# lan496/torch-m3gnet

Measured on AMD Instinct MI355X. Metric: atom-steps/sec (energy+forces) on 10k-atom PBC batch, 1/2/4/8 MI355X, higher is better.
Workload: dtype f32; 1 GPU; single 10000-atom fcc Cu PBC supercell per GPU (10x10x25 cells, a=3.61 A, jitter 0.025 A), r_cut 5 A / 3-body 4 A, default M3GNet (l_max=n_max=3, D=64, 3 blocks), energy+forces+stress; precision=fp32, atoms_per_gpu=10000, edges_per_gpu=420000, triplets_per_gpu=3060000

## Files before the change

### torch-m3gnet_amd/csrc/m3g_api.hip

```cpp
#include <climits>
#include <cmath>
#include <cstdarg>
#include <cstdio>
#include <cstdlib>
#include <cstring>
#include <utility>

#include "m3g_internal.h"

namespace m3g {

static thread_local char g_err[512] = "";
void set_error(const char* fmt, ...) {
  va_list ap;
  va_start(ap, fmt);
  vsnprintf(g_err, sizeof(g_err), fmt, ap);
  va_end(ap);
}

static void layout_mlp(MlpW& m, size_t& off) {
  auto take = [&](size_t n) { size_t r = off; off += (n + 63) / 64 * 64; return r; };
  m.w1a_t = take(kDP * 2 * kDP); m.w1b_t = take(kDP * 2 * kDP); m.w1c_t = take(kDP * 2 * kDP);
  m.b1 = take(2 * kDP);
  m.w2d_t = take(kDP * kDP); m.w2g_t = take(kDP * kDP);
// ... 75 lines not shown
    for (int k = 0; k < cols; ++k) blob[off + (size_t)k * ldo + col_off + o] = in[(size_t)o * ldi + k0 + k];
}
static void put_n(std::vector<float>& blob, size_t off, int ldo, const float* in, int rows, int ldi, int k0, int cols,
                  int row_off = 0) {
  for (int o = 0; o < rows; ++o)
    for (int k = 0; k < cols; ++k) blob[off + (size_t)(row_off + o) * ldo + k] = in[(size_t)o * ldi + k0 + k];
}

static void pack_mlp(std::vector<float>& blob, const MlpW& m, const m3g_plan& p, const std::string& pre,
                     const std::string& lin, int D, int R) {
  const float* wd1 = p.params.at(pre + ".dense.0.weight").data();
  const float* wg1 = p.params.at(pre + ".gate.0.weight").data();
  const size_t parts_t[3] = {m.w1a_t, m.w1b_t, m.w1c_t};
  const size_t parts_n[3] = {m.w1a, m.w1b, m.w1c};
  for (int part = 0; part < 3; ++part) {
    put_t(blob, parts_t[part], 2 * kDP, wd1, D, 3 * D, part * D, D, 0);
    put_t(blob, parts_t[part], 2 * kDP, wg1, D, 3 * D, part * D, D, kDP);
    put_n(blob, parts_n[part], kDP, wd1, D, 3 * D, part * D, D, 0);
    put_n(blob, parts_n[part], kDP, wg1, D, 3 * D, part * D, D, kDP);
  }
  const float* bd1 = p.params.at(pre + ".dense.0.bias").data();
  const float* bg1 = p.params.at(pre + ".gate.0.bias").data();
  for (int o = 0; o < D; ++o) { blob[m.b1 + o] = bd1[o]; blob[m.b1 + kDP + o] = bg1[o]; }
  const float* wd2 = p.params.at(pre + ".dense.2.weight").data();
  const float* wg2 = p.params.at(pre + ".gate.2.weight").data();
  put_t(blob, m.w2d_t, kDP, wd2, D, D, 0, D); put_t(blob, m.w2g_t, kDP, wg2, D, D, 0, D);
  put_n(blob, m.w2d, kDP, wd2, D, D, 0, D); put_n(blob, m.w2g, kDP, wg2, D, D, 0, D);
  const float* bd2 = p.params.at(pre + ".dense.2.bias").data();
  const float* bg2 = p.params.at(pre + ".gate.2.bias").data();
  for (int o = 0; o < D; ++o) { blob[m.b2d + o] = bd2[o]; blob[m.b2g + o] = bg2[o]; }
  const float* wl = p.params.at(lin).data();
  put_t(blob, m.wl_t, kDP, wl, D, R, 0, R);
  put_n(blob, m.wl, kRP, wl, D, R, 0, R);
}

Work work_carve(int B, const StepPath& path, int64_t N, int64_t E, int64_t S, void* base) {
  Work w{};
  Carve c{(char*)base};
  auto take = [&](size_t n_floats) { return (float*)c.take(n_floats * sizeof(float)); };
  size_t e = (size_t)E, n = (size_t)N;
  w.u = take(e * 3); w.d = take(e); w.h = take(e * kRP); w.hp = take(e * kRP);
  w.q = take(e * kCP); w.qp = take(e * kCP); w.fc3 = take(e); w.fc3p = take(e);
  for (int b = 0; b <= B; ++b) w.x[b] = take(n * kDP);
  for (int b = 0; b < B; ++b) w.v[b] = take(n * kCP);
  for (int b = 0; b < B; ++b) w.m[b] = take(e * kCP);
  w.dx = take(n * kDP); w.dx2 = take(n * kDP);
  w.dm = take(e * kCP); w.g = take(e * kCP); w.dg = take(e * kCP);
  w.dh = take(e * kRP); w.dd = take(e); w.du = take(e * 3); w.dp1 = take(e * 4 * kDP); w.dr = take(e * 3);
  const size_t tiles16 = (e + 15) / 16;
  if (path.pipeline == kPipeMfma) {
    for (int b = 0; b <= B; ++b) w.e_blk[b] = take(tiles16 * 1024);
    if (path.saved_acts >= 1) for (int b = 0; b < B; ++b) w.p1_blk[b] = take(tiles16 * 2 * 2048);
    if (path.saved_acts >= 2) for (int b = 0; b < B; ++b) w.p2_blk[b] = take(tiles16 * 2 * 2048);
    for (int b = 0; b < B; ++b) { w.TAb[b] = take(n * 4 * kDP); w.TBb[b] = take(n * 4 * kDP); }
    w.de_soa = take(tiles16 * 1024);
    w.dcn = take(tiles16 * 1024);
    w.dh_parts = take((size_t)(2 * B + 1) * e * kRP);
    w.seg_head = take((tiles16 + 1) * 4 * kDP);
    w.seg_first = take((n + 1) * 4 * kDP);
  } else {
    w.TA = take(n * 4 * kDP); w.TB = take(n * 4 * kDP);
    w.e = take(e * kDP);
    w.de = take(e * kDP);
    for (int b = 0; b < B; ++b) w.act[b] = take(e * 8 * kDP);
  }
  static_assert(kSyncWords <= 64, "the tail scratch reserves 64 words");
  w.tail = take(n + (size_t)S * 2 + 64);
  w.sync = w.tail ? (int32_t*)(w.tail + n + (size_t)S * 2) : nullptr;
  w.total_bytes = c.off;
  return w;
}

}

using namespace m3g;

static void drop_graphs(const m3g_plan* plan);

enum StageId { ST_GEOM = 0, ST_EMBED, ST_NODE_PRE, ST_THREEBODY, ST_EDGE_FWD, ST_NODE_SUM, ST_READOUT, ST_OUTPUTS, ST_EDGE_REV_NODE,
               ST_EDGE_REV, ST_THREEBODY_REV, ST_NODE_REV, ST_EMBED_REV, ST_GEOM_REV, ST_EDGE_REV_FUSED, ST_COUNT };
static const char* kStageNames[ST_COUNT] = {"geometry_basis", "embed", "node_pre", "threebody_fwd", "edge_block_fwd", "node_sum",
                                            "readout", "optional_outputs", "edge_rev_node_mlp", "edge_rev_edge_mlp", "threebody_rev",
                                            "node_rev", "embed_rev", "geometry_rev_forces", "edge_rev_fused"};
struct StageTimer {
  const m3g_plan* p;
  hipStream_t s;
  size_t pair = (size_t)-1;
  StageTimer(const m3g_plan* plan, bool profile, int stage, hipStream_t stream) : p(plan), s(stream) {
    if (!profile) return;
    if (p->ev_used * 2 + 2 > p->ev_pool.size()) {
      hipEvent_t a, b;
      if (hipEventCreate(&a) != hipSuccess || hipEventCreate(&b) != hipSuccess) return;
      p->ev_pool.push_back(a);
      p->ev_pool.push_back(b);
      p->ev_stage.push_back(stage);
    }
    pair = p->ev_used++;
    p->ev_stage[pair] = stage;
    (void)hipEventRecord(p->ev_pool[2 * pair], s);
  }
  ~StageTimer() {
    if (pair != (size_t)-1) (void)hipEventRecord(p->ev_pool[2 * pair + 1], s);
  }
};
#define M3G_STAGE(id) StageTimer _st_##id(plan, mode.profile, id, s)

extern "C" int m3g_profile_enable(m3g_plan* plan, int32_t enable) {
// ... 92 lines not shown
extern "C" int m3g_plan_set_param(m3g_plan* plan, const char* key, const float* host_data, int64_t numel) {
  if (!plan || !key || !host_data) { set_error("m3g_plan_set_param: null argument"); return M3G_ERR_VALUE; }
  auto exp = expected_params(plan->cfg);
  auto it = exp.find(key);
  if (it == exp.end()) { set_error("unknown parameter key '%s'", key); return M3G_ERR_VALUE; }
  if (it->second != numel) { set_error("parameter '%s': expected %lld values, got %lld", key, (long long)it->second, (long long)numel); return M3G_ERR_VALUE; }
  plan->params[key].assign(host_data, host_data + numel);
  plan->committed = false;
  return M3G_OK;
}

extern "C" int m3g_plan_set_const(m3g_plan* plan, const char* name, const float* host_data, int64_t numel) {
  if (!plan || !name || !host_data) { set_error("m3g_plan_set_const: null argument"); return M3G_ERR_VALUE; }
  auto exp = expected_consts(plan->cfg);
  auto it = exp.find(name);
  if (it == exp.end()) { set_error("unknown constant '%s'", name); return M3G_ERR_VALUE; }
  if (it->second != numel) { set_error("constant '%s': expected %lld values, got %lld", name, (long long)it->second, (long long)numel); return M3G_ERR_VALUE; }
  plan->cvals[name].assign(host_data, host_data + numel);
  plan->committed = false;
  return M3G_OK;
}

static int hook_stamps(m3g_plan* plan, int32_t* value) {
  if (*value && !plan->d_stamps) {
    M3G_HIP_CHECK(hipMalloc((void**)&plan->d_stamps, 256 * 16 * 12 * sizeof(unsigned long long)));
    M3G_HIP_CHECK(hipMemset(plan->d_stamps, 0, 256 * 16 * 12 * sizeof(unsigned long long)));
  } else if (!*value && plan->d_stamps) {
    (void)hipFree(plan->d_stamps);
    plan->d_stamps = nullptr;
  }
  *value = *value == 0 ? 0 : *value == 3 ? 3 : *value == 2 ? 2 : 1;
  return M3G_OK;
}
struct OptionRow {
  const char* name;
  int Options::*member;
  int lo, hi;
  const char* error;
  int (*hook)(m3g_plan*, int32_t* value);
};
#define M3G_HOOK(...) [](m3g_plan* plan, int32_t* value) -> int { __VA_ARGS__; return M3G_OK; }
static const OptionRow kOptions[] = {
    {"edge_kernel", &Options::edge_kernel, 0, 2, "edge_kernel must be 0 (VALU baseline), 1 (MFMA) or 2 (any-size path)",
     M3G_HOOK(if (plan->generic && *value != 2) { set_error("this model size only runs on the any-size path (edge_kernel = 2)"); return M3G_ERR_UNSUPPORTED; })},
    {"precision", &Options::precision, 0, 2,
     "precision must be 0 (fp32: exact fp32 MFMA products), 1 (bf16x3 split products) or 2 (f16x3: scaled fp16 split products)", nullptr},
    {"save_p1", &Options::save_p1, 0, 1, nullptr, nullptr},
    {"save_p2", &Options::save_p2, 0, 1, nullptr, nullptr},
    {"rev_kernel", &Options::rev_kernel, 0, 1, "rev_kernel must be 0 (node-MLP + edge-MLP kernel pair) or 1 (fused)", nullptr},
    {"small_tiles", &Options::small_tiles, 0, INT_MAX, "small_tiles must be >= 0", M3G_HOOK(plan->opt.small_tiles_fwd = *value)},
    {"small_tiles_fwd", &Options::small_tiles_fwd, 0, INT_MAX, "small_tiles_fwd must be >= 0", nullptr},
    {"dp1_by_dst", &Options::dp1_by_dst, 0, 1, nullptr, nullptr},
    {"split_node_tiles", &Options::split_node_tiles, 0, INT_MAX, "split_node_tiles must be >= 0", nullptr},
    {"species_tables", &Options::species_tables, 0, 1, nullptr, nullptr},
    {"fuse_node_tb", &Options::fuse_node_tb, 0, 1, nullptr, nullptr},
    {"debug_node_tb_polls", &Options::debug_node_tb_polls, INT_MIN, INT_MAX, nullptr, nullptr},
    {"split_tail", &Options::split_tail, 0, 2, "split_tail must be 0 (never), 1 (a single left-over tile) or 2 (one or two)", nullptr},
    {"small_launches", &Options::small_launches, 0, 1, nullptr, nullptr},
    {"graph_replay", &Options::graph_replay, 0, 1, nullptr, M3G_HOOK(if (!*value) drop_graphs(plan))},
    {"overlap", &Options::overlap, 0, 1, nullptr, nullptr},
    {"threebody_moments", &Options::tb_moments, 0, 1, nullptr, nullptr},
    {"legendre_backward", &Options::legendre_ref, 0, 1, "legendre_backward: 0 (exact derivative) or 1 (the reference's backward)", nullptr},
    {"readout_f16", &Options::readout_f16, 0, 1, nullptr, nullptr},
    {"stress_mode", &Options::stress_mode, 0, 1, "stress_mode must be 0 (reference: sum pos (x) F / V) or 1 (pair virial)", nullptr},
    {"debug_force_move", nullptr, INT_MIN, INT_MAX, nullptr, M3G_HOOK(plan->debug_force_move = *value != 0; plan->committed = false)},
    {"stamps", &Options::stamp_target, INT_MIN, INT_MAX, nullptr, hook_stamps},
};
#undef M3G_HOOK

extern "C" int m3g_plan_set_option(m3g_plan* plan, const char* name, int32_t value) {
  if (!plan || !name) { set_error("m3g_plan_set_option: null argument"); return M3G_ERR_VALUE; }
  for (const OptionRow& row : kOptions) {
    if (strcmp(name, row.name) != 0) continue;
    if (value < row.lo || value > row.hi) {
      if (row.error) { set_error("%s", row.error); return M3G_ERR_VALUE; }
      value = 1;
    }
    if (row.hook) { int rc = row.hook(plan, &value); if (rc) return rc; }
    if (row.member) plan->opt.*row.member = value;
    return M3G_OK;
  }
  set_error("unknown option '%s'", name);
  return M3G_ERR_VALUE;
}

extern "C" int m3g_debug_read_stamps(m3g_plan* plan, uint64_t* host_out ) {
  if (!plan || !host_out || !plan->d_stamps) { set_error("stamps not enabled"); return M3G_ERR_STATE; }
  M3G_HIP_CHECK(hipMemcpy(host_out, plan->d_stamps, 256 * 16 * 12 * sizeof(unsigned long long), hipMemcpyDeviceToHost));
  return M3G_OK;
}

extern "C" int m3g_plan_commit(m3g_plan* plan) {
  if (!plan) { set_error("m3g_plan_commit: null plan"); return M3G_ERR_VALUE; }
  drop_graphs(plan);
  const m3g_config& cfg = plan->cfg;
  for (auto& kv : expected_params(cfg))
    if (!plan->params.count(kv.first)) { set_error("parameter '%s' was never set", kv.first.c_str()); return M3G_ERR_STATE; }
  for (auto& kv : expected_consts(cfg))
    if (!plan->cvals.count(kv.first)) { set_error("constant '%s' was never set", kv.first.c_str()); return M3G_ERR_STATE; }
  const int D = cfg.embedding_dim, R = cfg.n_max, L = cfg.l_max, C = L * R, B = cfg.num_blocks;
  {
    int dev = 0;
    M3G_HIP_CHECK(hipGetDevice(&dev));
    if (plan->device >= 0 && (plan->device != dev || plan->debug_force_move)) {
      M3G_HIP_CHECK(hipSetDevice(plan->device));
      M3G_HIP_CHECK(hipDeviceSynchronize());
// ... 23 lines not shown
  c.inv_len = 1.f / c.length_scale;
  const double rc = cfg.cutoff / cfg.length_scale, rc3 = cfg.threebody_cutoff / cfg.length_scale;
  fill_radial_consts(c, R, rc, plan->cvals.at("coeff").data(), plan->cvals.at("em").data(), plan->cvals.at("dm").data());
  fill_angular_consts(c, L, R, rc, rc3, plan->cvals.at("bessel_zeros").data(), plan->cvals.at("factors").data());

  const WeightLayout& wl = plan->wl;
  std::vector<float> blob(wl.total, 0.f);
  put_t(blob, wl.emb, kDP, plan->params.at("model.3.linear.weight").data(), D, cfg.num_types, 0, cfg.num_types);
  put_t(blob, wl.adj_t, kDP, plan->params.at("model.5.linear.weight").data(), D, R, 0, R);
  put_n(blob, wl.adj, kRP, plan->params.at("model.5.linear.weight").data(), D, R, 0, R);
  for (int t = 0; t < cfg.num_types; ++t) blob[wl.elemental + t] = plan->cvals.at("elemental_energies")[t];
  char buf[128];
  for (int b = 0; b < B; ++b) {
    const BlockW& bw = wl.blk[b];
    std::string tb = "model." + std::to_string(6 + 2 * b), cv = "model." + std::to_string(7 + 2 * b);
    const float* w1 = plan->params.at(tb + ".linear_sigmoid1.weight").data();
    put_t(blob, bw.tb_w1_t, kCP, w1, C, D, 0, D);
    put_n(blob, bw.tb_w1, kDP, w1, C, D, 0, D);
    for (int cc = 0; cc < C; ++cc) blob[bw.tb_b1 + cc] = plan->params.at(tb + ".linear_sigmoid1.bias")[cc];
    const float* wd = plan->params.at(tb + ".gated_mlp.dense.0.weight").data();
    const float* wg = plan->params.at(tb + ".gated_mlp.gate.0.weight").data();
    put_t(blob, bw.tb_wd_t, kDP, wd, D, C, 0, C); put_t(blob, bw.tb_wg_t, kDP, wg, D, C, 0, C);
    put_n(blob, bw.tb_wd, kCP, wd, D, C, 0, C); put_n(blob, bw.tb_wg, kCP, wg, D, C, 0, C);
    pack_mlp(blob, bw.e, *plan, cv + ".concat_edge_update", cv + ".edge_linear.weight", D, R);
    pack_mlp(blob, bw.n, *plan, cv + ".concat_node_update", cv + ".node_linear.weight", D, R);
  }
  {
    const ReadoutW& r = wl.ro;
    snprintf(buf, sizeof buf, "model.%d.gated", 6 + 2 * B);
    std::string ro = buf;
    const float* wd0 = plan->params.at(ro + ".dense.0.weight").data();
    const float* wg0 = plan->params.at(ro + ".gate.0.weight").data();
    const float* wd2 = plan->params.at(ro + ".dense.2.weight").data();
    const float* wg2 = plan->params.at(ro + ".gate.2.weight").data();
    put_t(blob, r.w1d_t, kDP, wd0, D, D, 0, D); put_t(blob, r.w1g_t, kDP, wg0, D, D, 0, D);
    put_t(blob, r.w2d_t, kDP, wd2, D, D, 0, D); put_t(blob, r.w2g_t, kDP, wg2, D, D, 0, D);
    put_n(blob, r.w1d, kDP, wd0, D, D, 0, D); put_n(blob, r.w1g, kDP, wg0, D, D, 0, D);
    put_n(blob, r.w2d, kDP, wd2, D, D, 0, D); put_n(blob, r.w2g, kDP, wg2, D, D, 0, D);
    for (int o = 0; o < D; ++o) {
      blob[r.b1d + o] = plan->params.at(ro + ".dense.0.bias")[o];
      blob[r.b1g + o] = plan->params.at(ro + ".gate.0.bias")[o];
      blob[r.b2d + o] = plan->params.at(ro + ".dense.2.bias")[o];
      blob[r.b2g + o] = plan->params.at(ro + ".gate.2.bias")[o];
      blob[r.w3d + o] = plan->params.at(ro + ".dense.4.weight")[o];
      blob[r.w3g + o] = plan->params.at(ro + ".gate.4.weight")[o];
    }
    blob[r.b3] = plan->params.at(ro + ".dense.4.bias")[0];
    blob[r.b3 + 1] = plan->params.at(ro + ".gate.4.bias")[0];
  }
  if (!plan->d_weights) M3G_HIP_CHECK(hipMalloc((void**)&plan->d_weights, wl.total * sizeof(float)));
  M3G_HIP_CHECK(hipMemcpy(plan->d_weights, blob.data(), wl.total * sizeof(float), hipMemcpyHostToDevice));
  { int rc = pack_mfma_images(plan); if (rc) return rc; }
  { int rc = build_species_tables(plan); if (rc) return rc; }
  plan->committed = true;
  return M3G_OK;
}

static StepPath plan_step_path(const m3g_plan* plan, int64_t N, int64_t E, int64_t T, int64_t S, int topo_hints, bool forces, bool stresses, bool profile) {
  const m3g_config& cfg = plan->cfg;
  return resolve_step_path(plan->opt, ModelDims{cfg.l_max, cfg.n_max, cfg.l_max * cfg.n_max, cfg.num_blocks}, N, E, T, S, topo_hints, forces, stresses, profile);
}

extern "C" int m3g_workspace_bytes(const m3g_plan* plan, int64_t N, int64_t E, int64_t T, int64_t S, size_t* bytes) {
  if (!plan || !bytes || N < 0 || E < 0 || T < 0 || S < 0) { set_error("m3g_workspace_bytes: bad argument"); return M3G_ERR_VALUE; }
  const StepPath p = plan_step_path(plan, N, E, T, S, 0, true, true, false);
  *bytes = p.pipeline == kPipeAnySize ? generic_workspace_bytes(plan, N, E, T, S) : work_carve(plan->cfg.num_blocks, p, N, E, S, nullptr).total_bytes;
  return M3G_OK;
}

static bool ensure_side_stream(const m3g_plan* plan) {
  if (plan->side_stream) return true;
  if (hipStreamCreateWithFlags(&plan->side_stream, hipStreamNonBlocking) != hipSuccess) { plan->side_stream = nullptr; return false; }
  if (hipEventCreateWithFlags(&plan->ev_fork, hipEventDisableTiming) != hipSuccess ||
      hipEventCreateWithFlags(&plan->ev_join, hipEventDisableTiming) != hipSuccess)
    return false;
  return true;
}

static void drop_graphs(const m3g_plan* plan) {
  for (auto& g : plan->graphs) {
    if (g.exec) (void)hipGraphExecDestroy(g.exec);
    if (g.graph) (void)hipGraphDestroy(g.graph);
  }
  plan->graphs.clear();
}

struct RunMode { bool profile; };

struct Step {
  const m3g_plan* plan;
  const m3g_io* io;
  const StepPath p;
  const bool mfma;
  const Consts& c;
  const WeightLayout& wl;
  const float* W;
  hipStream_t s;
  RunMode mode;
  Topo t;
  Work w;
  float *ea, *st;
  int enqueue_forward() const, enqueue_optional_outputs() const, enqueue_reverse() const;
};

static int check_call(const m3g_plan* plan, const m3g_io* io) {
  if (!plan || !io) { set_error("m3g_energy_forces: null argument"); return M3G_ERR_VALUE; }
  if (!plan->committed) { set_error("m3g_energy_forces: plan parameters not committed"); return M3G_ERR_STATE; }
  int dev = -1;
  M3G_HIP_CHECK(hipGetDevice(&dev));
  if (dev == plan->device) return M3G_OK;
  set_error("m3g_energy_forces: the plan was committed on device %d but the current device is %d (commit again on this device)", plan->device, dev);
  return M3G_ERR_STATE;
}

int Step::enqueue_forward() const {
  const bool want_f = io->forces != nullptr;
  {
    M3G_STAGE(ST_GEOM);
    if (p.block0 == kBlock0ExpandBesideGeom) launch_geometry_species(plan, c, t, w, io->pos, io->lattice, io->edge_cell_shift, io->atom_types, s);
    else if (p.block0 == kBlock0Kernel && p.geom_with_node_pre) launch_geometry_node_pre(plan, c, t, w, io->pos, io->lattice, io->edge_cell_shift, io->atom_types, W + wl.emb, s);
    else launch_geometry(c, t, io->pos, io->lattice, io->edge_cell_shift, w, s);
  }
  {
    M3G_STAGE(ST_EMBED);
    if (mfma) {
      if (c.B == 0) launch_embed_nodes_only(c, W, wl, t, io->atom_types, w, s);
      if (!p.fused_rev || c.B == 0) launch_embed_edges_soa(c, W + wl.adj_t, w.h, w.e_blk[0], t.E, s);
    } else {
      launch_embed(c, W, wl, t, io->atom_types, w, s);
    }
  }
  for (int b = 0; b < c.B; ++b) {
    {
      M3G_STAGE(ST_NODE_PRE);
      if (mfma && b == 0 && p.block0 == kBlock0ExpandBesideGeom) {  }
      else if (mfma && b == 0 && p.block0 == kBlock0ExpandAlone) launch_species_expand(plan, c, t, w, io->atom_types, s);
      else if (mfma && b == 0 && p.geom_with_node_pre) {  }
      else if (mfma) launch_node_pre_mfma(plan, p.node_split, c, t, w, b, b > 0 ? w.x[b - 1] : nullptr, w.x[b], w.v[b], w.TAb[b], w.TBb[b],
                                          b == 0 ? io->atom_types : nullptr, W + wl.emb, s);
      else launch_node_pre(c, W, wl.blk[b], t, w, nullptr, w.x[b], w.v[b], w.TA, w.TB, s);
    }
    { M3G_STAGE(ST_THREEBODY); launch_threebody(p, c, t, w, w.v[b], w.m[b], s); }
    M3G_STAGE(ST_EDGE_FWD);
    if (mfma) {
      if (p.fwd_split) launch_edge_fwd_split(plan, p, c, t, w, b, s);
      else launch_edge_block_mfma(plan, p, c, t, w, b, s, b + 1 < c.B || io->edge_attr != nullptr);
      (void)ST_NODE_SUM;
    } else {
      launch_edge_block(c, W, wl.blk[b], t, w, b, w.x[b], w.x[b + 1], s);
    }
  }
  M3G_STAGE(ST_READOUT);
  if (mfma) launch_readout_mfma(plan, p, c, wl, t, io->atom_types, c.B > 0 ? w.x[c.B - 1] : nullptr, w.x[c.B], w, ea, st, io->total_energy, want_f, s);
  else launch_readout(c, W, wl, t, io->atom_types, nullptr, w.x[c.B], w, ea, st, io->total_energy, want_f, s);
  return M3G_OK;
}

int Step::enqueue_optional_outputs() const {
  M3G_STAGE(ST_OUTPUTS);
  if (io->node_features) launch_copy_strided(w.x[c.B], kDP, io->node_features, c.D, c.D, t.N, s);
  if (io->edge_attr) {
    if (mfma) launch_soa_to_rows(w.e_blk[c.B], io->edge_attr, c.D, c.D, t.E, s);
    else launch_copy_strided(w.e, kDP, io->edge_attr, c.D, c.D, t.E, s);
  }
  if (io->edge_distances && t.E > 0) M3G_HIP_CHECK(hipMemcpyAsync(io->edge_distances, w.d, sizeof(float) * t.E, hipMemcpyDeviceToDevice, s));
  if (io->edge_weights) launch_copy_strided(w.h, kRP, io->edge_weights, c.R, c.R, t.E, s);
  if (io->triplet_angles) launch_triplet_angles(t, io->triplet_edge_index, w.u, io->triplet_angles, s);
  if (io->mid_edge_features)
    for (int b = 0; b < c.B; ++b)
      launch_copy_expand_rows(t.act_id, w.m[b], kCP, io->mid_edge_features + (size_t)b * t.E * c.C, c.C, c.C, t.E, s);
  return M3G_OK;
}

int Step::enqueue_reverse() const {
  float *dx_cur = w.dx, *dx_alt = w.dx2;
  bool dr_done = false;
  if (!mfma && c.B > 0 && t.E > 0) {
    M3G_HIP_CHECK(hipMemsetAsync(w.de, 0, sizeof(float) * t.E * kDP, s));
    M3G_HIP_CHECK(hipMemsetAsync(w.dh, 0, sizeof(float) * t.E * kRP, s));
  }
  for (int b = c.B - 1; b >= 0; --b) {
    const bool first = b == c.B - 1;
    switch (p.rev_edge) {
      case kRevSplit: { M3G_STAGE(ST_EDGE_REV_FUSED); launch_edge_rev_split(plan, p, c, t, w, b, dx_cur, first, s); } break;
      case kRevF32: { M3G_STAGE(ST_EDGE_REV_FUSED); launch_edge_rev_f32(plan, p, c, t, w, b, dx_cur, first, s); } break;
      case kRevFused: { M3G_STAGE(ST_EDGE_REV_FUSED); launch_edge_rev_fused(plan, c, t, w, b, dx_cur, first, s); } break;
      case kRevPair: {
        { M3G_STAGE(ST_EDGE_REV_NODE); launch_edge_rev_node_mlp(plan, p, c, t, w, b, dx_cur, s); }
        M3G_STAGE(ST_EDGE_REV);
        launch_edge_rev_edge_mlp(plan, p, c, t, w, b, dx_cur, first, s);
      } break;
      default: { M3G_STAGE(ST_EDGE_REV); launch_edge_block_reverse(c, W, wl.blk[b], t, w, b, dx_cur, s); }
    }
    bool node_done = false;
    if (p.tail[b] == kTailOverlap) {
      if (!ensure_side_stream(plan)) { set_error("overlap: could not create the internal stream"); return M3G_ERR_HIP; }
      M3G_HIP_CHECK(hipEventRecord(plan->ev_fork, s));
      M3G_HIP_CHECK(hipStreamWaitEvent(plan->side_stream, plan->ev_fork, 0));
      launch_threebody_reverse(p, c, t, w, w.v[b], first, plan->side_stream, plan->opt.legendre_ref);
      M3G_HIP_CHECK(hipEventRecord(plan->ev_join, plan->side_stream));
      launch_node_reverse(c, W, wl.blk[b], t, w, w.v[b], dx_cur, dx_alt, true, p.dp1, false, s);
      M3G_HIP_CHECK(hipStreamWaitEvent(s, plan->ev_join, 0));
      launch_node_reverse_v_term(c, W, wl.blk[b], t, w, w.v[b], dx_alt, s);
      node_done = true;
    } else if (p.tail[b] == kTailNodeTb) {
      node_done = launch_node_tb_reverse(c, W, wl.blk[b], t, w, w.v[b], first, dx_cur, dx_alt, p.dp1, b, s, p.tb_hints, plan->opt.debug_node_tb_polls);
    } else if (p.tail[b] == kTailFinalTb) {
      launch_threebody_reverse_final(c, t, w, w.v[b], first, w.dh_parts, c.B, s, p.tb_hints);
      dr_done = true;
    }
    if (!node_done && p.tail[b] != kTailFinalTb) {
      { M3G_STAGE(ST_THREEBODY_REV); launch_threebody_reverse(p, c, t, w, w.v[b], first, s, plan->opt.legendre_ref); }
      if (b > 0) {
        M3G_STAGE(ST_NODE_REV);
        launch_node_reverse(c, W, wl.blk[b], t, w, w.v[b], dx_cur, dx_alt, p.fused_rev, p.dp1, true, s, p.node_rev_small);
        node_done = true;
      }
    }
    if (node_done) std::swap(dx_cur, dx_alt);
  }
  {
    M3G_STAGE(ST_EMBED_REV);
    if (p.fused_rev) {  }
    else if (mfma) launch_embed_edges_reverse_soa(W + wl.adj, w.h, w.de_soa, w.dh_parts + (size_t)2 * c.B * t.E * kRP, t.E, s);
    else launch_embed_reverse(c, W, wl, t, w, s);
  }
  M3G_STAGE(ST_GEOM_REV);
  if (mfma) launch_geometry_reverse(c, t, w, w.dh_parts, p.fused_rev ? c.B : 2 * c.B + 1, io->forces, io->stresses, s, p.gather_virial, io->pos, io->lattice, dr_done);
  else launch_geometry_reverse(c, t, w, w.dh, 1, io->forces, io->stresses, s);
  if (p.stress == kStressPair) launch_stress_pair(t, w, io->lattice, io->stresses, s);
  else if (p.stress == kStressRef) launch_stress(c, t, io->pos, io->lattice, io->forces, io->stresses, s, p.energy_deferred ? ea : nullptr, st, io->total_energy);
  return M3G_OK;
}

static int enqueue_step(const m3g_plan* plan, const m3g_io* io, void* workspace, size_t workspace_bytes, hipStream_t s, RunMode mode) {
  const int64_t N = io->n_atoms, E = io->n_edges, T = io->n_triplets, S = io->n_structs;
  if (N < 0 || E < 0 || T < 0 || S < 0) { set_error("negative size"); return M3G_ERR_VALUE; }
  if (!io->total_energy || !io->topo || (N > 0 && (!io->pos || !io->atom_types)) || (S > 0 && !io->lattice) || (E > 0 && !io->edge_cell_shift)) {
    set_error("m3g_energy_forces: missing required pointer");
// ... 150 lines not shown
```

### torch-m3gnet_amd/csrc/m3g_edge_common.h

```cpp
#pragma once
#include <utility>

#include "m3g_device.h"
#include "m3g_internal.h"
#include "m3g_dual_chain.h"
#include "m3g_dual_f32.h"
#include "m3g_mfma_common.h"

namespace m3g {

constexpr int kFwdLdsFloats = 8 * kTbSteps * 64 + 2 * (8 * 4 * 4 * 64 + 2 * (4 * 4 * 4 * 64) + 2 * 4 * 64 + 4 * 64) + 4 * 64;
constexpr int kRevMlpFloats = 8 * 4 * 4 * 64 + 4 * (4 * 4 * 4 * 64) + 2 * 4 * 64 + 4 * 8 * 4 * 64 + 64 * 4;
constexpr int kRevEdgeFloats = kRevMlpFloats + 8 * kTbSteps * 64 + 8 * 4 * 64;
constexpr int kWaves = 16;
constexpr int kWavesFwdH = 12;
constexpr int kWavesFwdBf = 12;
template <int PREC>
constexpr int fwd_waves() { return PREC == kPrecF16x3 ? kWavesFwdH : PREC == kPrecBf16x3 ? kWavesFwdBf : kWaves; }
constexpr int kWavesRevFused = 8;
constexpr int kWavesRev = 12;
constexpr int kTileEdges = 16;
constexpr int kTileFloats = 4 * 64 * 4;
constexpr int kP1TileFloats = 8 * 64 * 4;

// ... 178 lines not shown
  for (int base = 0; base < n_vec; base += nt * kBatch) {
    f32x4 t[kBatch];
    static_for<kBatch>([&]<int j>() {
      const int i = base + j * nt + (int)threadIdx.x;
      t[j] = i < n_vec ? *(const f32x4*)(src + 4 * i) : zero4();
    });
    static_for<kBatch>([&]<int j>() {
      const int i = base + j * nt + (int)threadIdx.x;
      if (i < n_vec) *(f32x4*)(lds + 4 * i) = t[j];
    });
  }
  if (threadIdx.x == 0) *lds_head = 0;
  __syncthreads();
}

__device__ __forceinline__ unsigned long long stamp_now() {
  unsigned long long t;
  __builtin_amdgcn_sched_barrier(0);
  asm volatile("s_memtime %0\n\ts_waitcnt lgkmcnt(0)" : "=s"(t)::"memory");
  __builtin_amdgcn_sched_barrier(0);
  return t;
}
template <bool ON>
struct Stamps {
  unsigned long long last = 0, sum[12] = {0, 0, 0, 0, 0, 0, 0, 0, 0, 0, 0, 0};
  __device__ __forceinline__ void start() { if (ON) last = stamp_now(); }
  template <int I>
  __device__ __forceinline__ void mark() {
    if (ON) { unsigned long long t = stamp_now(); sum[I] += t - last; last = t; }
  }
  template <bool ACCUMULATE>
  __device__ __forceinline__ void store(unsigned long long* stamps, int lane) const {
    if (ON && lane == 0) {
      const int wave = threadIdx.x >> 6;
      unsigned long long* dst = stamps + ((size_t)blockIdx.x * 16 + wave) * 12;
      for (int i = 0; i < 12; ++i) dst[i] = ACCUMULATE ? dst[i] + sum[i] : sum[i];
    }
  }
};

struct FwdArgs {
  int64_t E, tiles;
  const float* img;
  const int32_t *src, *dst;
  const float *h, *m, *TA, *TB;
  const int32_t* act_id;
  const float* e_in;
  float* e_out;
  float *seg_head, *seg_first;
  unsigned long long* stamps;
  float* p1_out;
  float* p2_out;
  float w_inv;
};

template <int TBS>
__device__ __forceinline__ void tb_preact(const float* tbimg, const float (&mb)[TBS], f32x4 (&p)[8], int lane) {
  zero(p);
  static_for<TBS>([&]<int s>() {
    const float b = mb[s];
    static_for<8>([&]<int ob>() { p[ob] = mfma16(tbimg[(ob * kTbSteps + s) * 64 + lane], b, p[ob]); });
  });
}

template <int PREC, int TBS>
struct TbIn { float mb[TBS]; };
template <int TBS>
struct TbIn<kPrecF16x3, TBS> { f16x8 hi, lo; float inv; };

template <int PREC, int TBS>
__device__ __forceinline__ TbIn<PREC, TBS> tb_load(const float* __restrict__ m, int arow, int q, float w_inv) {
  TbIn<PREC, TBS> r;
  if constexpr (PREC == kPrecF16x3) {
    f32x4 v[2] = {zero4(), zero4()};
    if (arow >= 0 && q < 2) {
      const float* row = m + (int64_t)arow * kCP + 8 * q;
      v[0] = *(const f32x4*)row;
      v[1] = *(const f32x4*)(row + 4);
    }
    const EdgeScale sc = edge_scale<2>(v);
    split8h(v[0], v[1], sc.s, r.hi, r.lo);
    r.inv = sc.inv * w_inv;
  } else {
    static_for<TBS>([&]<int s>() { r.mb[s] = arow >= 0 ? m[(int64_t)arow * kCP + 4 * s + q] : 0.f; });
  }
  return r;
}
template <int PREC, int TBS>
__device__ __forceinline__ void tb_preact_p(const float* tbimg, const TbIn<PREC, TBS>& in, f32x4 (&p)[8], int lane) {
  if constexpr (PREC == kPrecF16x3) {
    const f16x8* hi = reinterpret_cast<const f16x8*>(tbimg) + (lane & 31);
    const f16x8* lo = hi + 8 * 32;
    f16x8 ah = hi[0], al = lo[0];
    static_for<8>([&]<int ob>() {
      f16x8 nh = ah, nl = al;
      if constexpr (ob + 1 < 8) { nh = hi[(ob + 1) * 32]; nl = lo[(ob + 1) * 32]; }
      sched_fence();
      f32x4 t = zero4();
      t = mfma_f16(ah, in.hi, t);
      t = mfma_f16(ah, in.lo, t);
      t = mfma_f16(al, in.hi, t);
      p[ob] = t * in.inv;
      sched_fence();
      ah = nh; al = nl;
    });
  } else {
    tb_preact<TBS>(tbimg, in.mb, p, lane);
  }
}

__device__ __forceinline__ void gather_tables(const float* __restrict__ TA, const float* __restrict__ TB, int mlp, int64_t ci,
                                              int64_t cj, int qd, f32x4 (&p1)[8]) {
  const float* ta = TA + ci * (4 * kDP) + mlp * (2 * kDP) + 4 * qd;
  const float* tb = TB + cj * (4 * kDP) + mlp * (2 * kDP) + 4 * qd;
  static_for<8>([&]<int ob>() { p1[ob] = *(const f32x4*)(ta + ob * 16) + *(const f32x4*)(tb + ob * 16); });
}

__device__ __forceinline__ void gated_out_reverse(f32x4& d2d, f32x4& d2g, const f32x4& d_upd, const f32x4& sl, const float* wl4, f32x4& dhv) {
  static_for<2>([&]<int k>() {
    const f32x2 p2d = {d2d[2 * k], d2d[2 * k + 1]}, p2g = {d2g[2 * k], d2g[2 * k + 1]};
    const f32x2 du = {d_upd[2 * k], d_upd[2 * k + 1]}, s_lin = {sl[2 * k], sl[2 * k + 1]};
    f32x2 sd, dsd;
    silu_pair(p2d, sd, dsd);
    const f32x2 sg = sigmoid_pair(p2g);
    const f32x2 a_g = du * sg;
    const f32x2 d_s = a_g * sd;
    const f32x2 d_o = a_g * s_lin;
    const f32x2 dd = d_o * dsd;
    const f32x2 dgt = (d_s * s_lin) * (1.f - sg);
    const f32x4 w0 = *(const f32x4*)(wl4 + (2 * k) * 4), w1 = *(const f32x4*)(wl4 + (2 * k + 1) * 4);
    f32x2 h01 = {dhv[0], dhv[1]}, h23 = {dhv[2], dhv[3]};
    h01 += f32x2{w0[0], w0[1]} * d_s[0]; h23 += f32x2{w0[2], w0[3]} * d_s[0];
    h01 += f32x2{w1[0], w1[1]} * d_s[1]; h23 += f32x2{w1[2], w1[3]} * d_s[1];
    dhv[0] = h01[0]; dhv[1] = h01[1]; dhv[2] = h23[0]; dhv[3] = h23[1];
    d2d[2 * k] = dd[0]; d2d[2 * k + 1] = dd[1];
    d2g[2 * k] = dgt[0]; d2g[2 * k + 1] = dgt[1];
  });
}

__device__ __forceinline__ void load_dmsg(const float* __restrict__ dx_new, int64_t ci, int qd, f32x4 (&dmsg)[4]) {
  const float* xrow = dx_new + ci * kDP + 4 * qd;
  static_for<4>([&]<int blk>() { dmsg[blk] = *(const f32x4*)(xrow + blk * 16); });
}
__device__ __forceinline__ void de2_from(bool de_is_zero, const float* de_tile, const f32x4 (&contrib)[4], f32x4 (&de)[4]) {
  if (de_is_zero) {
    static_for<4>([&]<int blk>() { de[blk] = contrib[blk]; });
  } else {
    static_for<4>([&]<int blk>() { de[blk] = load_tile4(de_tile + blk * 256) + contrib[blk]; });
  }
}
template <bool STORE>
__device__ __forceinline__ void de1_from(float* de_tile, const f32x4 (&contrib)[4], f32x4 (&de)[4]) {
  static_for<4>([&]<int blk>() {
    de[blk] += contrib[blk];
    if (STORE) *(f32x4*)(de_tile + blk * 256) = de[blk];
  });
}

struct RevArgs {
  int64_t E, tiles;
  const float* img;
  const int32_t *src, *dst;
  const float *h, *m, *dx_new;
  const int32_t* act_id;
  const float *TA, *TB;
  const float* e_tile;
  const float* e2_tile;
  float* de_soa;
  float* dcn;
  int de_is_zero;
  float* dm;
  float* dh;
  float* dp1;
  unsigned long long* stamps;
  float *seg_head, *seg_first;
  const float* p1;
  const float* p2;
  float w_inv;
  float* dp1_scale;
  const int32_t* in_pos;
  int split_tail;
};

__device__ __forceinline__ float sum_lane_quarters(float x) {
  const unsigned u = __builtin_bit_cast(unsigned, x);
  auto r16 = __builtin_amdgcn_permlane16_swap(u, u, false, false);
  const float y = __builtin_bit_cast(float, (unsigned)r16[0]) + __builtin_bit_cast(float, (unsigned)r16[1]);
  const unsigned v = __builtin_bit_cast(unsigned, y);
  auto r32 = __builtin_amdgcn_permlane32_swap(v, v, false, false);
  return __builtin_bit_cast(float, (unsigned)r32[0]) + __builtin_bit_cast(float, (unsigned)r32[1]);
}

__device__ __forceinline__ void store_dh(float* dh, int64_t edge, int64_t E, f32x4 dhv, int qd) {
  static_for<4>([&]<int rr>() { dhv[rr] = sum_lane_quarters(dhv[rr]); });
  if (qd == 0 && edge < E) *(f32x4*)(dh + edge * kRP) = dhv;
}

inline int grid_for_tiles(int64_t tiles, int  = kWaves) {
  int64_t wgs = tiles;
  wgs = (wgs + 7) / 8 * 8;
  if (wgs < 8) wgs = 8;
  if (wgs > 256) wgs = 256;
  return (int)wgs;
}

inline int tb_steps_for(int C) { return (C + 3) / 4; }
inline int64_t tiles_for(int64_t E) { return (E + kTileEdges - 1) / kTileEdges; }

inline FwdArgs fwd_args(const Topo& t, const Work& w, int b, const float* img) {
  FwdArgs a{};
  a.E = t.E; a.tiles = tiles_for(t.E); a.img = img;
  a.src = t.src; a.dst = t.dst; a.h = w.h; a.m = w.m[b]; a.TA = w.TAb[b]; a.TB = w.TBb[b]; a.act_id = t.act_id;
  a.e_in = w.e_blk[b]; a.e_out = w.e_blk[b + 1]; a.seg_head = w.seg_head; a.seg_first = w.seg_first; a.w_inv = 1.f;
  return a;
}
inline RevArgs rev_args(const Topo& t, const Work& w, int b, const float* img, const float* dx_new, bool de_is_zero, int dh_slice) {
  RevArgs a{};
  a.E = t.E; a.tiles = tiles_for(t.E); a.img = img;
  a.src = t.src; a.dst = t.dst; a.h = w.h; a.m = w.m[b]; a.dx_new = dx_new; a.act_id = t.act_id;
  a.de_soa = w.de_soa; a.de_is_zero = de_is_zero ? 1 : 0; a.dm = w.dm; a.dh = w.dh_parts + (size_t)dh_slice * t.E * kRP; a.dp1 = w.dp1;
  a.w_inv = 1.f;
  return a;
}

#define M3G_TBS_SWITCH(C_, CALL)                     \
  switch (tb_steps_for(C_)) {                        \
    case 1: { constexpr int TBS = 1; CALL; } break;  \
    case 2: { constexpr int TBS = 2; CALL; } break;  \
    case 3: { constexpr int TBS = 3; CALL; } break;  \
    default: { constexpr int TBS = 4; CALL; } break; \
  }

#define M3G_PREC_SWITCH(P_, CALL)                                            \
  if ((P_) == kPrecF32) { constexpr int PREC = kPrecF32; CALL; }             \
  else if ((P_) == kPrecF16x3) { constexpr int PREC = kPrecF16x3; CALL; }    \
  else { constexpr int PREC = kPrecBf16x3; CALL; }

}
```

### torch-m3gnet_amd/csrc/m3g_edge_mfma.hip

```cpp
#include "m3g_edge_common.h"

namespace m3g {

__device__ __forceinline__ void save_store(float* ptr, const f32x4& val) { __builtin_nontemporal_store(val, (f32x4*)ptr); }
template <bool KEEP_P1, int PREC, int SAVE = 0>
__device__ __forceinline__ void mlp_preacts(const float* lds, int w1c, int w2d, int w2g, int b2, const f32x4 (&x)[4], f32x4 (&p1)[8],
                                            f32x4 (&p2)[8], int lane, float* p1_out = nullptr, float* p2_out = nullptr, float w_inv = 1.f) {
  chain_p<PREC, 8, 2>(lds + w1c, x, p1, lane, w_inv);
  if constexpr (SAVE == 1) static_for<8>([&]<int ob>() { *(f32x4*)(p1_out + ob * 256) = p1[ob]; });
  bias_step<4, 0>(lds + b2, p2, lane);
  bias_step<4, 4>(lds + b2 + 4 * 64, p2, lane);
  if constexpr (!KEEP_P1 && SAVE == 2) {
    static_for<8>([&]<int ob>() {
      f32x4 ds;
      static_for<2>([&]<int k>() {
        f32x2 act, der;
        silu_pair(f32x2{p1[ob][2 * k], p1[ob][2 * k + 1]}, act, der);
        p1[ob][2 * k] = act[0]; p1[ob][2 * k + 1] = act[1];
        ds[2 * k] = der[0]; ds[2 * k + 1] = der[1];
      });
      save_store(p1_out + ob * 256, ds);
    });
    chain_p<PREC, 4, 2, 0, 0>(lds + w2d, p1, p2, lane, w_inv);
    chain_p<PREC, 4, 2, 4, 4>(lds + w2g, p1, p2, lane, w_inv);
    static_for<8>([&]<int ob>() { save_store(p2_out + ob * 256, p2[ob]); });
    return;
  }
  if (KEEP_P1) {
    f32x4 hid[8];
    static_for<8>([&]<int ob>() { silu_keep_derivative(p1[ob], hid[ob]); });
    chain_p<PREC, 4, 2, 0, 0>(lds + w2d, hid, p2, lane, w_inv);
    chain_p<PREC, 4, 2, 4, 4>(lds + w2g, hid, p2, lane, w_inv);
  } else {
    if constexpr (PREC == kPrecF16x3) {
      static_for<8>([&]<int ob>() {
        static_for<2>([&]<int k>() {
          const f32x2 v = silu_pair(f32x2{p1[ob][2 * k], p1[ob][2 * k + 1]});
          p1[ob][2 * k] = v[0]; p1[ob][2 * k + 1] = v[1];
        });
      });
    } else {
      static_for<8>([&]<int ob>() { static_for<4>([&]<int r>() { p1[ob][r] = fsilu(p1[ob][r]); }); });
    }
    chain_p<PREC, 4, 2, 0, 0>(lds + w2d, p1, p2, lane, w_inv);
    chain_p<PREC, 4, 2, 4, 4>(lds + w2g, p1, p2, lane, w_inv);
  }
}

template <bool ST, int S0, int PREC, int SAVE>
__device__ __forceinline__ void mlp_forward_mfma(const float* lds, const MfmaMlpFwd& L, int mlp, const FwdArgs& a, int64_t ci,
                                                 int64_t cj, float hb, const f32x4 (&x)[4], f32x4 (&out)[4], int lane,
                                                 Stamps<ST>& st, float* p1_out, float* p2_out) {
  f32x4 p1[8], p2[8];
  gather_tables(a.TA, a.TB, mlp, ci, cj, lane >> 4, p1);
  st.template mark<S0>();
  mlp_preacts<false, PREC, SAVE>(lds, L.w1c, L.w2d, L.w2g, L.b2, x, p1, p2, lane, p1_out, p2_out, a.w_inv);
  st.template mark<S0 + 1>();
  static_for<4>([&]<int ob>() {
    out[ob] = mfma16(lds[L.wl + ob * 64 + lane], hb, zero4());
    mul_gated<PREC == kPrecF16x3 || PREC == kPrecF32>(out[ob], p2[ob], p2[4 + ob]);
  });
  st.template mark<S0 + 3>();
}

template <int TBS, bool ST = false, bool FIRST = false, int PREC = kPrecBf16x3, int SAVE = 0, bool STORE_E = true>
__global__ void __launch_bounds__(64 * fwd_waves<PREC>()) k_edge_block_mfma(FwdArgs a, MfmaFwdLayout L) {
  __shared__ __attribute__((aligned(16))) float lds[kFwdLdsFloats + 4];
  int* q_head = reinterpret_cast<int*>(lds + kFwdLdsFloats);
  load_image(lds, a.img, kFwdLdsFloats, q_head);
  const int lane = threadIdx.x & 63, qd = lane >> 4;
  TileQueue queue(a.tiles, q_head);
  Stamps<ST> st;
  int ticket = queue.fetch(lane);
  if (ticket >= queue.count) return;
  int ci_i, cj_i;
  load_ends(a.src, a.dst, queue.base + ticket, a.E, lane, ci_i, cj_i);
  int arow_i = load_arow(a.act_id, queue.base + ticket, a.E, lane);
  for (;;) {
    const int64_t tile = queue.base + ticket;
    ticket = queue.fetch(lane);
    const bool has_next = ticket < queue.count;
    int nci = 0, ncj = 0, narow = -1;
    if (has_next) {
      load_ends(a.src, a.dst, queue.base + ticket, a.E, lane, nci, ncj);
      narow = load_arow(a.act_id, queue.base + ticket, a.E, lane);
    }
    int lv = lane;
    asm volatile("" : "+v"(lv));
    st.start();
    const int64_t edge = tile * kTileEdges + (lane & 15);
    const int64_t ec = edge < a.E ? edge : a.E - 1;
    const int64_t ci = ci_i, cj = cj_i;
    const int qv = lv >> 4;
    const int tl_out = FIRST ? lv : lane;
    const float* e_tile = a.e_in + tile * kTileFloats + lane * 4;
    float* e_otile = a.e_out + tile * kTileFloats + tl_out * 4;
    f32x4 x[4];
    if (!FIRST) static_for<4>([&]<int blk>() { x[blk] = load_tile4(e_tile + blk * 256); });
    const int arow = arow_i;
    const TbIn<PREC, TBS> tbin = tb_load<PREC, TBS>(a.m, arow, qv, a.w_inv);
    const float hb = a.h[ec * kRP + qv];
    if (FIRST) {
      static_for<4>([&]<int blk>() {
        x[blk] = mfma16(lds[L.adj + blk * 64 + lv], hb, zero4());
        static_for<4>([&]<int r>() { x[blk][r] = fsilu(x[blk][r]); });
      });
    }
    st.template mark<0>();
    {
      f32x4 p[8];
      tb_preact_p<PREC, TBS>(lds + L.tb, tbin, p, lv);
      static_for<4>([&]<int blk>() { add_gated<PREC == kPrecF16x3 || PREC == kPrecF32>(x[blk], p[blk], p[4 + blk]); });
    }
    st.template mark<1>();
    f32x4 out[4];
    float* p1_tile = SAVE >= 1 ? a.p1_out + tile * (2 * kP1TileFloats) + lane * 4 : nullptr;
    float* p2_tile = SAVE >= 2 ? a.p2_out + tile * (2 * kP1TileFloats) + lane * 4 : nullptr;
    mlp_forward_mfma<ST, 2, PREC, SAVE>(lds, L.mlp[0], 0, a, ci, cj, hb, x, out, lv, st, p1_tile, p2_tile);
    static_for<4>([&]<int blk>() {
      x[blk] += out[blk];
      if constexpr (STORE_E) *(f32x4*)(e_otile + blk * 256) = x[blk];
    });
    st.template mark<6>();
    mlp_forward_mfma<ST, 7, PREC, SAVE>(lds, L.mlp[1], 1, a, ci, cj, hb, x, out, lv, st, SAVE >= 1 ? p1_tile + kP1TileFloats : nullptr,
                                        SAVE >= 2 ? p2_tile + kP1TileFloats : nullptr);
    {
      if (edge >= a.E) static_for<4>([&]<int blk>() { out[blk] = zero4(); });
      const SegMasks sk = seg_masks((int)ci, lane);
      seg_scan(out, sk);
      seg_store(out, sk, a.seg_head, a.seg_first, tile, ci, qd, 0);
    }
    st.template mark<11>();
    if (!has_next) break;
    ci_i = nci;
    cj_i = ncj;
    arow_i = narow;
  }
  st.template store<false>(a.stamps, lane);
}

template <bool ST, int PREC, bool SAVED>
__device__ __forceinline__ void mlp_reverse_mfma(const float* lds, const MfmaMlpRev& L, int mlp, const RevArgs& a, int64_t edge, int64_t tile,
                                                 int64_t ci, int64_t cj, const f32x4& hv, const f32x4 (&x)[4],
                                                 const f32x4 (&d_upd)[4], f32x4 (&contrib)[4], f32x4& dhv, int lane,
                                                 Stamps<ST>& st) {
  const int qd = lane >> 4;
  f32x4 p1[8], d2[8];
  if constexpr (SAVED) {
    const float* src = a.p1 + tile * (2 * kP1TileFloats) + mlp * kP1TileFloats + (threadIdx.x & 63) * 4;
    static_for<8>([&]<int ob>() { p1[ob] = load_tile4(src + ob * 256); });
    st.template mark<2>();
    bias_step<4, 0>(lds + L.b2, d2, lane);
    bias_step<4, 4>(lds + L.b2 + 4 * 64, d2, lane);
    f32x4 hid[8];
    static_for<8>([&]<int ob>() { silu_keep_derivative(p1[ob], hid[ob]); });
    chain_p<PREC, 4, 2, 0, 0>(lds + L.w2d, hid, d2, lane, a.w_inv);
    chain_p<PREC, 4, 2, 4, 4>(lds + L.w2g, hid, d2, lane, a.w_inv);
  } else {
    gather_tables(a.TA, a.TB, mlp, ci, cj, qd, p1);
    st.template mark<2>();
    mlp_preacts<true, PREC>(lds, L.w1c, L.w2d, L.w2g, L.b2, x, p1, d2, lane, nullptr, nullptr, a.w_inv);
  }
  st.template mark<3>();
  static_for<4>([&]<int ob>() {
    static_for<4>([&]<int r>() {
      const float p2d = d2[ob][r], p2g = d2[4 + ob][r];
      const f32x4 w = *(const f32x4*)(lds + L.wl + (ob * 16 + 4 * qd + r) * 4);
      const float s_lin = w[0] * hv[0] + w[1] * hv[1] + w[2] * hv[2] + w[3] * hv[3];
      const float sg = fsigmoid(p2g), sgd = fsigmoid(p2d), sd = p2d * sgd;
      const float du = d_upd[ob][r];
      const float d_out = du * s_lin, d_s = du * sd * sg;
      dhv[0] += d_s * w[0]; dhv[1] += d_s * w[1]; dhv[2] += d_s * w[2]; dhv[3] += d_s * w[3];
      d2[ob][r] = d_out * sg * (sgd * (1.f + p2d * (1.f - sgd)));
      d2[4 + ob][r] = d_out * sd * sg * (1.f - sg);
    });
    asm volatile("" : "+v"(dhv[0]), "+v"(dhv[1]), "+v"(dhv[2]), "+v"(dhv[3]));
  });
  st.template mark<4>();
  f32x4 dp1[8];
  zero(dp1);
  chain_p<PREC, 4, 2, 0, 0>(lds + L.w2dT, d2, dp1, lane, a.w_inv);
  chain_p<PREC, 4, 2, 4, 4>(lds + L.w2gT, d2, dp1, lane, a.w_inv);
  static_for<8>([&]<int ob>() { dp1[ob] *= p1[ob]; });
  st.template mark<5>();
  if (edge < a.E) {
    float* row = a.dp1 + edge * (4 * kDP) + mlp * (2 * kDP) + 4 * qd;
    static_for<8>([&]<int ob>() { *(f32x4*)(row + ob * 16) = dp1[ob]; });
  }
  zero(contrib);
  chain_p<PREC, 4, 4>(lds + L.w1cT, dp1, contrib, lane, a.w_inv);
  st.template mark<6>();
}

template <int PREC, bool SAVED = false>
__global__ void __launch_bounds__(64 * kWavesRev) k_edge_rev_node_mlp(RevArgs a, MfmaRevLayout L) {
  __shared__ __attribute__((aligned(16))) float lds[kRevMlpFloats + 4];
  int* q_head = reinterpret_cast<int*>(lds + kRevMlpFloats);
  load_image(lds, a.img, kRevMlpFloats, q_head);
  const int lane = threadIdx.x & 63, qd = lane >> 4;
  TileQueue queue(a.tiles, q_head);
  int ticket = queue.fetch(lane);
  if (ticket >= queue.count) return;
  int ci_i, cj_i;
  load_ends(a.src, a.dst, queue.base + ticket, a.E, lane, ci_i, cj_i);
  for (;;) {
    const int64_t tile = queue.base + ticket;
    ticket = queue.fetch(lane);
    const bool has_next = ticket < queue.count;
    int nci = 0, ncj = 0;
    if (has_next) load_ends(a.src, a.dst, queue.base + ticket, a.E, lane, nci, ncj);
    int lv = lane;
    asm volatile("" : "+v"(lv));
    const int64_t edge = tile * kTileEdges + (lane & 15);
    const int64_t ec = edge < a.E ? edge : a.E - 1;
    const int64_t ci = ci_i, cj = cj_i;
    float* dcn_tile = a.dcn + tile * kTileFloats + lane * 4;
    const float* e_tile = a.e_tile + tile * kTileFloats + lane * 4;
    const f32x4 hv = *(const f32x4*)(a.h + ec * kRP);
    f32x4 dhv = zero4();
    f32x4 contrib[4];
    {
      f32x4 dmsg[4], x[4];
      load_dmsg(a.dx_new, ci, qd, dmsg);
      if (!SAVED) static_for<4>([&]<int blk>() { x[blk] = *(const f32x4*)(e_tile + blk * 256); });
      Stamps<false> st0;
      mlp_reverse_mfma<false, PREC, SAVED>(lds, L.mlp, 1, a, edge, tile, ci, cj, hv, x, dmsg, contrib, dhv, lv, st0);
    }
    static_for<4>([&]<int blk>() { *(f32x4*)(dcn_tile + blk * 256) = contrib[blk]; });
    store_dh(a.dh, edge, a.E, dhv, qd);
    if (!has_next) break;
    ci_i = nci;
    cj_i = ncj;
  }
}

template <int TBS, bool ST = false, int PREC = kPrecBf16x3, bool SAVED = false>
__global__ void __launch_bounds__(64 * kWavesRev) k_edge_rev_edge_mlp(RevArgs a, MfmaRevLayout L) {
  Stamps<ST> st;
  __shared__ __attribute__((aligned(16))) float lds[kRevEdgeFloats + 4];
  int* q_head = reinterpret_cast<int*>(lds + kRevEdgeFloats);
  load_image(lds, a.img, kRevEdgeFloats, q_head);
  const int lane = threadIdx.x & 63, qd = lane >> 4;
  TileQueue queue(a.tiles, q_head);
  int ticket = queue.fetch(lane);
  if (ticket >= queue.count) return;
  int ci_i, cj_i;
  load_ends(a.src, a.dst, queue.base + ticket, a.E, lane, ci_i, cj_i);
  for (;;) {
    const int64_t tile = queue.base + ticket;
    ticket = queue.fetch(lane);
    const bool has_next = ticket < queue.count;
    int nci = 0, ncj = 0;
    if (has_next) load_ends(a.src, a.dst, queue.base + ticket, a.E, lane, nci, ncj);
    int lv = lane;
    asm volatile("" : "+v"(lv));
    st.start();
    const int64_t edge = tile * kTileEdges + (lane & 15);
    const int64_t ec = edge < a.E ? edge : a.E - 1;
    const int64_t ci = ci_i, cj = cj_i;
    float* de_tile = a.de_soa + tile * kTileFloats + lane * 4;
    const float* e_tile = a.e_tile + tile * kTileFloats + lane * 4;
    const f32x4 hv = *(const f32x4*)(a.h + ec * kRP);
    f32x4 dhv = zero4();
    float mb[TBS];
    const int arow = a.act_id[ec];
    static_for<TBS>([&]<int s>() { mb[s] = arow >= 0 ? a.m[(int64_t)arow * kCP + 4 * s + qd] : 0.f; });
    f32x4 de[4], contrib[4];
    {
      f32x4 x[4];
      if constexpr (!SAVED) {
        f32x4 p[8];
        static_for<4>([&]<int blk>() { x[blk] = *(const f32x4*)(e_tile + blk * 256); });
        tb_preact<TBS>(lds + L.tb, mb, p, lv);
        static_for<4>([&]<int blk>() { add_gated<false>(x[blk], p[blk], p[4 + blk]); });
      }
      st.template mark<1>();
      const float* dcn_tile = a.dcn + tile * kTileFloats + lane * 4;
      if (a.de_is_zero) {
        static_for<4>([&]<int blk>() { de[blk] = *(const f32x4*)(dcn_tile + blk * 256); });
      } else {
        static_for<4>([&]<int blk>() { de[blk] = *(const f32x4*)(de_tile + blk * 256) + *(const f32x4*)(dcn_tile + blk * 256); });
      }
      mlp_reverse_mfma<ST, PREC, SAVED>(lds, L.mlp, 0, a, edge, tile, ci, cj, hv, x, de, contrib, dhv, lv, st);
    }
    static_for<4>([&]<int blk>() {
      de[blk] += contrib[blk];
      *(f32x4*)(de_tile + blk * 256) = de[blk];
    });
    f32x4 d8[8];
    tb_preact<TBS>(lds + L.tb, mb, d8, lv);
    static_for<4>([&]<int blk>() {
      static_for<4>([&]<int r>() {
        const float p = d8[blk][r], sgd = fsigmoid(p), sg = fsigmoid(d8[4 + blk][r]);
        d8[blk][r] = de[blk][r] * sg * (sgd * (1.f + p * (1.f - sgd)));
        d8[4 + blk][r] = de[blk][r] * (p * sgd) * sg * (1.f - sg);
      });
    });
    f32x4 dmv[1];
    zero(dmv);
    chain_p<PREC, 1, 4>(lds + L.tbT, d8, dmv, lv, a.w_inv);
    store_dh(a.dh, edge, a.E, dhv, qd);
    if (edge < a.E && arow >= 0) *(f32x4*)(a.dm + (int64_t)arow * kCP + 4 * qd) = dmv[0];
    st.template mark<7>();
    if (!has_next) break;
    ci_i = nci;
    cj_i = ncj;
  }
  st.template store<false>(a.stamps, lane);
}

constexpr int kRevFusedFloats = 8 * kTbSteps * 64 + 8 * 4 * 64 + 2 * (128 * 64 + 2 * 64 * 64 + 2 * 4 * 64 + 64 * 4 + 4 * 64) + 4 * 64 + 64 * 4;

template <int PREC, int OB, int KS, int ROWS, int XOFF = 0, int AOFF = 0, int RB0 = 0, int NX, int NA>
__device__ __forceinline__ void cdual(const float* img, const f32x4 (&x)[NX], f32x4 (&acc)[NA], int lane, float w_inv) {
  if constexpr (PREC == kPrecF16x3) chain_dual_h<OB, KS, ROWS, XOFF, AOFF, RB0>(img, x, acc, lane, w_inv);
  else chain_dual<OB, KS, ROWS, XOFF, AOFF, RB0>(img, x, acc, lane);
}
template <int PREC, int OB, int KS, int ROWS, int DOFF = 0, int AOFF = 0, int KB0 = 0, int ND, int NA>
__device__ __forceinline__ void cdual_t(const float* img, const f32x4 (&d)[ND], f32x4 (&acc)[NA], int lane, float w_inv) {
  if constexpr (PREC == kPrecF16x3) chain_dual_t_h<OB, KS, ROWS, DOFF, AOFF, KB0>(img, d, acc, lane, w_inv);
  else chain_dual_t<OB, KS, ROWS, DOFF, AOFF, KB0>(img, d, acc, lane);
}

template <bool KEEP_P1>
__device__ __forceinline__ void mlp_preacts_dual(const float* lds, const MfmaMlpFused& L, const f32x4 (&x)[4], f32x4 (&p1)[8],
                                                 f32x4 (&p2)[8], int lane) {
  chain_dual<8, 2, 128>(lds + L.w1c, x, p1, lane);
  bias_step<4, 0>(lds + L.b2, p2, lane);
  bias_step<4, 4>(lds + L.b2 + 4 * 64, p2, lane);
  if (KEEP_P1) {
    f32x4 hid[8];
    static_for<8>([&]<int ob>() { silu_keep_derivative(p1[ob], hid[ob]); });
    chain_dual<4, 2, 64, 0, 0>(lds + L.w2d, hid, p2, lane);
    chain_dual<4, 2, 64, 4, 4>(lds + L.w2g, hid, p2, lane);
  } else {
    static_for<8>([&]<int ob>() { static_for<4>([&]<int r>() { p1[ob][r] = fsilu(p1[ob][r]); }); });
    chain_dual<4, 2, 64, 0, 0>(lds + L.w2d, p1, p2, lane);
    chain_dual<4, 2, 64, 4, 4>(lds + L.w2g, p1, p2, lane);
  }
}


template <bool NEED_DP1, int MLP, int PREC, bool ST = false, int S0 = 0>
__device__ __forceinline__ void mlp_reverse_dual(const float* lds, const MfmaMlpFused& L, const RevArgs& a, int64_t edge, int64_t tile,
                                                 int64_t ci, int64_t cj, const SegMasks& sk, const f32x4& hv, const f32x4 (&x)[4],
                                                 const f32x4 (&d_upd)[4], f32x4 (&contrib)[4], f32x4& dhv, int lane, Stamps<ST>& st,
                                                 f32x4& dp1_inv) {
  constexpr int mlp = MLP;
  const int qd = lane >> 4;
  f32x4 p1[8], d2[8];
  gather_tables(a.TA, a.TB, mlp, ci, cj, qd, p1);
  cdual<PREC, 8, 2, 128>(lds + L.w1c, x, p1, lane, a.w_inv);
  sched_fence();
  st.template mark<S0>();
  bias_step<4, 0>(lds + L.b2, d2, lane);
  bias_step<4, 4>(lds + L.b2 + 4 * 64, d2, lane);
  static_for<2>([&]<int half>() {
    f32x4 hid[4];
    static_for<4>([&]<int ob>() {
      static_for<2>([&]<int k>() {
        f32x4& pv = p1[4 * half + ob];
        f32x2 act, der;
        silu_pair(f32x2{pv[2 * k], pv[2 * k + 1]}, act, der);
        hid[ob][2 * k] = act[0]; hid[ob][2 * k + 1] = act[1];
        pv[2 * k] = der[0]; pv[2 * k + 1] = der[1];
      });
    });
    cdual<PREC, 4, 2, 64, 0, 4 * half>(lds + (half == 0 ? L.w2d : L.w2g), hid, d2, lane, a.w_inv);
    sched_fence();
  });
  st.template mark<S0 + 1>();
  const float hb_sel = qd == 0 ? hv[0] : qd == 1 ? hv[1] : qd == 2 ? hv[2] : hv[3];
  static_for<4>([&]<int ob>() {
    const f32x4 sl = mfma16(lds[L.wld + ob * 64 + lane], hb_sel, zero4());
    gated_out_reverse(d2[ob], d2[4 + ob], d_upd[ob], sl, lds + L.wl + (ob * 16 + 4 * qd) * 4, dhv);
    asm volatile("" : "+v"(dhv[0]), "+v"(dhv[1]), "+v"(dhv[2]), "+v"(dhv[3]));
  });
  zero(contrib);
  sched_fence();
  st.template mark<S0 + 2>();
  static_for<2>([&]<int half>() {
    f32x4 dp1[4];
    zero(dp1);
    cdual_t<PREC, 4, 2, 64, 4 * half, 0>(lds + (half == 0 ? L.w2d : L.w2g), d2, dp1, lane, a.w_inv);
    static_for<4>([&]<int ob>() { dp1[ob] *= p1[4 * half + ob]; });
    if (NEED_DP1 && edge < a.E) {
      if constexpr (PREC == kPrecBf16x3) {
        unsigned* row = reinterpret_cast<unsigned*>(a.dp1) + edge * kDp1PackedDwords + 3 * (mlp * 32 + half * 16 + qd);
        static_for<4>([&]<int ob>() { *(u32x3_a4*)(row + 12 * ob) = pack24(dp1[ob]); });
      }
    }
    if constexpr (PREC == kPrecF16x3) {
      EdgeScale scd;
      chain_dual_t_h<4, 2, 128, 0, 0, 4 * half>(lds + L.w1c, dp1, contrib, lane, a.w_inv, &scd);
      if (NEED_DP1 && edge < a.E) {
        unsigned* row = reinterpret_cast<unsigned*>(a.dp1) + edge * kDp1PackedDwords + 3 * (mlp * 32 + half * 16 + qd);
        const float s9 = scd.s * 512.f;
        static_for<4>([&]<int ob>() { *(u32x3_a4*)(row + 12 * ob) = pack24_fixed(dp1[ob], s9); });
      }
      dp1_inv[mlp * 2 + half] = scd.inv * (1.f / 512.f);
    } else {
      cdual_t<PREC, 4, 2, 128, 0, 0, 4 * half>(lds + L.w1c, dp1, contrib, lane, a.w_inv);
    }
    if (NEED_DP1) {
      if (edge >= a.E) zero(dp1);
      seg_scan(dp1, sk);
      seg_store(dp1, sk, a.seg_head, a.seg_first, tile, ci, qd, MLP * 8 + 4 * half);
    }
    sched_fence();
    st.template mark<S0 + 3 + half>();
  });
}

template <int TBS, bool NEED_DP1, int WAVES, int PREC = kPrecBf16x3, bool ST = false>
__global__ void __launch_bounds__(64 * WAVES) k_edge_rev_fused(RevArgs a, MfmaRevFusedLayout L) {
  Stamps<ST> st;
  __shared__ __attribute__((aligned(16))) float lds[kRevFusedFloats + 4];
  int* q_head = reinterpret_cast<int*>(lds + kRevFusedFloats);
  load_image(lds, a.img, kRevFusedFloats, q_head);
  const int lane = threadIdx.x & 63, qd = lane >> 4;
  TileQueue queue(a.tiles, q_head);
  int ticket = queue.fetch(lane);
  if (ticket >= queue.count) return;
  int ci_i, cj_i;
  load_ends(a.src, a.dst, queue.base + ticket, a.E, lane, ci_i, cj_i);
  int arow_i = load_arow(a.act_id, queue.base + ticket, a.E, lane);
  for (;;) {
    const int64_t tile = queue.base + ticket;
    ticket = queue.fetch(lane);
    const bool has_next = ticket < queue.count;
    int nci = 0, ncj = 0, narow = -1;
    if (has_next) {
      load_ends(a.src, a.dst, queue.base + ticket, a.E, lane, nci, ncj);
      narow = load_arow(a.act_id, queue.base + ticket, a.E, lane);
    }
    int lv = lane;
    asm volatile("" : "+v"(lv));
    st.start();
    const int64_t edge = tile * kTileEdges + (lane & 15);
    const int64_t ec = edge < a.E ? edge : a.E - 1;
    const int64_t ci = ci_i, cj = cj_i;
    const SegMasks sk = seg_masks((int)ci, lane);
    float* de_tile = a.de_soa + tile * kTileFloats + lane * 4;
    const float* e_tile = a.e_tile + tile * kTileFloats + lane * 4;
    const f32x4 hv = *(const f32x4*)(a.h + ec * kRP);
    f32x4 dhv = zero4(), dp1_inv = zero4();
    const int arow = arow_i;
    const TbIn<PREC, TBS> tbin = tb_load<PREC, TBS>(a.m, arow, qd, a.w_inv);
    f32x4 x[4], de[4], contrib[4];
    constexpr bool FIRST = !NEED_DP1;
    {
      f32x4 x2[4];
      const float* e2_tile = a.e2_tile + tile * kTileFloats + lane * 4;
      static_for<4>([&]<int blk>() { x2[blk] = load_tile4(e2_tile + blk * 256); });
      f32x4 dmsg[4];
      load_dmsg(a.dx_new, ci, qd, dmsg);
      mlp_reverse_dual<NEED_DP1, 1, PREC, ST, 0>(lds, L.mlp[1], a, edge, tile, ci, cj, sk, hv, x2, dmsg, contrib, dhv, lv, st, dp1_inv);
    }
    de2_from(a.de_is_zero, de_tile, contrib, de);
    asm volatile("" : "+v"(lv));
    sched_fence();
    if (FIRST) {
      const float hb = a.h[ec * kRP + qd];
      static_for<4>([&]<int blk>() {
        x[blk] = mfma16(lds[L.adj + blk * 64 + lv], hb, zero4());
        static_for<4>([&]<int r>() { x[blk][r] = fsilu(x[blk][r]); });
      });
    } else {
      static_for<4>([&]<int blk>() { x[blk] = load_tile4(e_tile + blk * 256); });
    }
    {
      f32x4 p[8];
      tb_preact_p<PREC, TBS>(lds + L.tb, tbin, p, lv);
      static_for<4>([&]<int blk>() { add_gated<true>(x[blk], p[blk], p[4 + blk]); });
    }
    st.template mark<5>();
    mlp_reverse_dual<NEED_DP1, 0, PREC, ST, 6>(lds, L.mlp[0], a, edge, tile, ci, cj, sk, hv, x, de, contrib, dhv, lv, st, dp1_inv);
    if (NEED_DP1 && PREC == kPrecF16x3 && qd == 0 && edge < a.E) *(f32x4*)(a.dp1_scale + edge * 4) = dp1_inv;
    de1_from<!FIRST>(de_tile, contrib, de);
    if (FIRST) {
      const float hb = a.h[ec * kRP + qd];
      static_for<4>([&]<int blk>() {
        const f32x4 pe = mfma16(lds[L.adj + blk * 64 + lv], hb, zero4());
        static_for<4>([&]<int r>() {
          const f32x4 w = *(const f32x4*)(lds + L.adjp + (blk * 16 + 4 * qd + r) * 4);
          const float t = de[blk][r] * fdsilu(pe[r]);
          dhv[0] += t * w[0]; dhv[1] += t * w[1]; dhv[2] += t * w[2]; dhv[3] += t * w[3];
        });
        asm volatile("" : "+v"(dhv[0]), "+v"(dhv[1]), "+v"(dhv[2]), "+v"(dhv[3]));
      });
    }
    f32x4 d8[8];
    tb_preact_p<PREC, TBS>(lds + L.tb, tbin, d8, lv);
    static_for<4>([&]<int blk>() { gated_reverse(d8[blk], d8[4 + blk], de[blk]); });
    f32x4 dmv[1];
    zero(dmv);
    chain_p<PREC, 1, 4>(lds + L.tbT, d8, dmv, lv, a.w_inv);
    store_dh(a.dh, edge, a.E, dhv, qd);
    if (edge < a.E && arow >= 0) *(f32x4*)(a.dm + (int64_t)arow * kCP + 4 * qd) = dmv[0];
    st.template mark<11>();
    if (!has_next) break;
    ci_i = nci;
    cj_i = ncj;
    arow_i = narow;
  }
  st.template store<true>(a.stamps, lane);
}

__device__ __forceinline__ int64_t soa_index(int64_t edge, int o) {
  return (edge >> 4) * kTileFloats + (o >> 4) * 256 + (((o >> 2) & 3) * 16 + (int)(edge & 15)) * 4 + (o & 3);
}

__global__ void __launch_bounds__(256) k_soa_to_rows(int64_t E, int width, int row_stride, const float* __restrict__ soa,
                                                     float* __restrict__ rows) {
  int64_t idx = blockIdx.x * (int64_t)blockDim.x + threadIdx.x;
  if (idx >= E * kDP) return;
  int64_t edge = idx >> 6;
  int o = (int)(idx & 63);
  if (o < width) rows[edge * row_stride + o] = soa[soa_index(edge, o)];
}
__global__ void __launch_bounds__(256) k_rows_to_soa(int64_t E, int64_t tiles, const float* __restrict__ rows, float* __restrict__ soa) {
  int64_t idx = blockIdx.x * (int64_t)blockDim.x + threadIdx.x;
  if (idx >= tiles * kTileFloats) return;
  int64_t tile = idx / kTileFloats;
  int rem = (int)(idx % kTileFloats), blk = rem >> 8, lane = (rem >> 2) & 63, reg = rem & 3;
  int64_t edge = tile * kTileEdges + (lane & 15);
  int o = blk * 16 + 4 * (lane >> 4) + reg;
  soa[idx] = edge < E ? rows[edge * kDP + o] : 0.f;
}

// ... 25 lines not shown
  int64_t ec = edge < E ? edge : E - 1;
  const f32x4 hv = *(const f32x4*)(h + ec * kRP);
  const float* src = de_soa + tile * kTileFloats + lane * 4;
  float d0 = 0.f, d1 = 0.f, d2 = 0.f, d3 = 0.f;
#pragma unroll
  for (int blk = 0; blk < 4; ++blk) {
    const f32x4 dv = *(const f32x4*)(src + blk * 256);
#pragma unroll
    for (int reg = 0; reg < 4; ++reg) {
      int o = blk * 16 + 4 * qd + reg;
      const f32x4 w = *(const f32x4*)(adj + o * kRP);
      float pe = w[0] * hv[0] + w[1] * hv[1] + w[2] * hv[2] + w[3] * hv[3];
      float t = dv[reg] * dsilu_f(pe);
      d0 += t * w[0]; d1 += t * w[1]; d2 += t * w[2]; d3 += t * w[3];
    }
  }
  d0 += __shfl_xor(d0, 16); d1 += __shfl_xor(d1, 16); d2 += __shfl_xor(d2, 16); d3 += __shfl_xor(d3, 16);
  d0 += __shfl_xor(d0, 32); d1 += __shfl_xor(d1, 32); d2 += __shfl_xor(d2, 32); d3 += __shfl_xor(d3, 32);
  if (qd == 0 && edge < E) *(f32x4*)(dh + edge * kRP) = f32x4{d0, d1, d2, d3};
}

void launch_rows_to_soa(const float* rows, float* soa, int64_t E, hipStream_t s) {
  int64_t tiles = tiles_for(E);
  if (tiles > 0)
    hipLaunchKernelGGL(k_rows_to_soa, dim3((unsigned)((tiles * kTileFloats + 255) / 256)), dim3(256), 0, s, E, tiles, rows, soa);
}
void launch_soa_to_rows(const float* soa, float* rows, int row_stride, int width, int64_t E, hipStream_t s) {
  if (E > 0) hipLaunchKernelGGL(k_soa_to_rows, dim3((unsigned)((E * kDP + 255) / 256)), dim3(256), 0, s, E, width, row_stride, soa, rows);
}
void launch_embed_edges_soa(const Consts& c, const float* adj_t, const float* h, float* soa, int64_t E, hipStream_t s) {
  int64_t tiles = tiles_for(E);
  if (tiles > 0)
    hipLaunchKernelGGL(k_embed_edges_soa, dim3((unsigned)((tiles * kTileFloats + 255) / 256)), dim3(256), 0, s, c.R, E, tiles, adj_t, h, soa);
}
void launch_embed_edges_reverse_soa(const float* adj, const float* h, const float* de_soa, float* dh, int64_t E, hipStream_t s) {
  int64_t tiles = tiles_for(E);
  if (tiles > 0)
    hipLaunchKernelGGL(k_embed_edges_reverse_soa, dim3((unsigned)((tiles * 64 + 255) / 256)), dim3(256), 0, s, E, tiles, adj, h, de_soa, dh);
}

void launch_edge_block_mfma(const m3g_plan* plan, const StepPath& p, const Consts& c, const Topo& t, const Work& w, int b, hipStream_t s,
                            bool e_out_read) {
  const int64_t tiles = tiles_for(t.E);
  const MfmaFwdLayout L = mfma_fwd_layout();
  const int prec = plan->opt.precision;
  if (tiles > 0) {
    FwdArgs a = fwd_args(t, w, b, plan->d_mfma_fwd[prec] + (size_t)b * L.total);
    a.stamps = plan->d_stamps;
    if (p.saved_acts >= 1) a.p1_out = w.p1_blk[b];
    if (p.saved_acts == 2) a.p2_out = w.p2_blk[b];
    if (prec == kPrecF16x3) a.w_inv = plan->w_scale_inv;
    dim3 grid(grid_for_tiles(tiles));
    const bool first = b == 0 && p.fused_rev;
    const int save = p.fwd_save;
#define M3G_FWD_LAUNCH(ST_, FIRST_, PREC_, SAVE_) hipLaunchKernelGGL((k_edge_block_mfma<TBS, ST_, FIRST_, PREC_, SAVE_>), grid, dim3(64 * fwd_waves<PREC_>()), 0, s, a, L)
#define M3G_FWD_BY_MODE(ST_, FIRST_)                                                               \
  if (prec == kPrecBf16x3) { M3G_FWD_LAUNCH(ST_, FIRST_, kPrecBf16x3, 0); }                        \
  else if (prec == kPrecF16x3) { M3G_FWD_LAUNCH(ST_, FIRST_, kPrecF16x3, 0); }                     \
  else if (save == 2 && !ST_ && !e_out_read) { hipLaunchKernelGGL((k_edge_block_mfma<TBS, false, FIRST_, kPrecF32, 2, false>), grid, dim3(64 * fwd_waves<kPrecF32>()), 0, s, a, L); } \
  else if (save == 2) { M3G_FWD_LAUNCH(ST_, FIRST_, kPrecF32, 2); }                                \
  else if (save == 1) { M3G_FWD_LAUNCH(ST_, FIRST_, kPrecF32, 1); }                                \
  else { M3G_FWD_LAUNCH(ST_, FIRST_, kPrecF32, 0); }
    if (plan->d_stamps && plan->opt.stamp_target == 1 && tb_steps_for(c.C) == 3) {
      constexpr int TBS = 3;
      if (first) { M3G_FWD_BY_MODE(true, true); } else { M3G_FWD_BY_MODE(true, false); }
    } else if (first) {
      M3G_TBS_SWITCH(c.C, M3G_FWD_BY_MODE(false, true));
    } else {
      M3G_TBS_SWITCH(c.C, M3G_FWD_BY_MODE(false, false));
    }
#undef M3G_FWD_BY_MODE
#undef M3G_FWD_LAUNCH
  }
}

void launch_edge_rev_node_mlp(const m3g_plan* plan, const StepPath& p, const Consts& c, const Topo& t, const Work& w, int b, const float* dx_new,
                              hipStream_t s) {
  (void)c;
  const int64_t tiles = tiles_for(t.E);
  if (tiles == 0) return;
  const MfmaRevLayout L = mfma_rev_layout();
  const int prec = plan->opt.precision;
  const float* img_n = plan->d_mfma_rev[prec] + (size_t)b * L.per_block + L.total_e;
  const bool saved = p.saved_acts >= 1;
  RevArgs an = rev_args(t, w, b, img_n, dx_new, false, 2 * b + 1);
  an.TA = w.TAb[b]; an.TB = w.TBb[b]; an.e_tile = w.e_blk[b + 1]; an.dcn = w.dcn;
  if (saved) an.p1 = w.p1_blk[b];
  if (prec == kPrecF16x3) an.w_inv = plan->w_scale_inv;
  if (saved) { M3G_PREC_SWITCH(prec, hipLaunchKernelGGL((k_edge_rev_node_mlp<PREC, true>), dim3(grid_for_tiles(tiles)), dim3(64 * kWavesRev), 0, s, an, L)); }
  else { M3G_PREC_SWITCH(prec, hipLaunchKernelGGL((k_edge_rev_node_mlp<PREC, false>), dim3(grid_for_tiles(tiles)), dim3(64 * kWavesRev), 0, s, an, L)); }
}

void launch_edge_rev_edge_mlp(const m3g_plan* plan, const StepPath& p, const Consts& c, const Topo& t, const Work& w, int b, const float* dx_new,
                              bool de_is_zero, hipStream_t s) {
  const int64_t tiles = tiles_for(t.E);
  if (tiles == 0) return;
  const MfmaRevLayout L = mfma_rev_layout();
  const int prec = plan->opt.precision;
  const bool saved = p.saved_acts >= 1;
  const float* img_e = plan->d_mfma_rev[prec] + (size_t)b * L.per_block;
  RevArgs ae = rev_args(t, w, b, img_e, dx_new, de_is_zero, 2 * b);
  ae.TA = w.TAb[b]; ae.TB = w.TBb[b]; ae.e_tile = w.e_blk[b]; ae.dcn = w.dcn; ae.stamps = plan->d_stamps;
  if (saved) ae.p1 = w.p1_blk[b];
  if (prec == kPrecF16x3) ae.w_inv = plan->w_scale_inv;
  dim3 grid(grid_for_tiles(tiles)), block(64 * kWavesRev);
  if (plan->d_stamps && plan->opt.stamp_target == 2 && tb_steps_for(c.C) == 3 && prec == kPrecBf16x3) {
    hipLaunchKernelGGL((k_edge_rev_edge_mlp<3, true>), grid, block, 0, s, ae, L);
    return;
  }
  if (saved) { M3G_PREC_SWITCH(prec, M3G_TBS_SWITCH(c.C, hipLaunchKernelGGL((k_edge_rev_edge_mlp<TBS, false, PREC, true>), grid, block, 0, s, ae, L))); }
  else { M3G_PREC_SWITCH(prec, M3G_TBS_SWITCH(c.C, hipLaunchKernelGGL((k_edge_rev_edge_mlp<TBS, false, PREC, false>), grid, block, 0, s, ae, L))); }
}

void launch_edge_rev_fused(const m3g_plan* plan, const Consts& c, const Topo& t, const Work& w, int b, const float* dx_new,
                           bool de_is_zero, hipStream_t s) {
  const int64_t tiles = tiles_for(t.E);
  if (tiles == 0) return;
  const MfmaRevFusedLayout L = mfma_rev_fused_layout();
  const bool f16 = plan->opt.precision == kPrecF16x3;
  const float* img = (f16 ? plan->d_mfma_revf_h : plan->d_mfma_revf) + (size_t)b * L.total;
  RevArgs ar = rev_args(t, w, b, img, dx_new, de_is_zero, b);
  ar.TA = w.TAb[b]; ar.TB = w.TBb[b]; ar.e_tile = w.e_blk[b]; ar.e2_tile = w.e_blk[b + 1]; ar.stamps = plan->d_stamps;
  ar.seg_head = w.seg_head; ar.seg_first = w.seg_first; ar.dp1_scale = dp1_scale_of(w.dp1, t.E);
  if (f16) ar.w_inv = plan->w_scale_inv;
  constexpr int WV = kWavesRevFused;
  dim3 grid(grid_for_tiles(tiles)), block(64 * WV);
  if (plan->d_stamps && plan->opt.stamp_target == 3 && f16 && tb_steps_for(c.C) == 3) {
    if (b > 0) hipLaunchKernelGGL((k_edge_rev_fused<3, true, WV, kPrecF16x3, true>), grid, block, 0, s, ar, L);
    else hipLaunchKernelGGL((k_edge_rev_fused<3, false, WV, kPrecF16x3, true>), grid, block, 0, s, ar, L);
    return;
  }
#define M3G_REVF_LAUNCH(NEED_) \
  if (f16) { M3G_TBS_SWITCH(c.C, hipLaunchKernelGGL((k_edge_rev_fused<TBS, NEED_, WV, kPrecF16x3>), grid, block, 0, s, ar, L)); } \
  else { M3G_TBS_SWITCH(c.C, hipLaunchKernelGGL((k_edge_rev_fused<TBS, NEED_, WV, kPrecBf16x3>), grid, block, 0, s, ar, L)); }
  if (b > 0) { M3G_REVF_LAUNCH(true); }
  else { M3G_REVF_LAUNCH(false); }
#undef M3G_REVF_LAUNCH
}

}
```

### torch-m3gnet_amd/csrc/m3g_edge_small.hip

```cpp
#include "m3g_edge_common.h"
#include "m3g_edge_split_rev.h"

namespace m3g {

namespace {

inline int grid_for_split(int64_t tiles) {
  int64_t wgs = tiles < 512 ? tiles : 512;
  return (int)(wgs < 1 ? 1 : wgs);
}

struct FwdMlpA {
  float w1[2][16], w2[2][16];
  f32x4 b2[2];
  float wl;
};
__device__ __forceinline__ void load_fwd_mlp(const float* __restrict__ img, const MfmaMlpFwd& L, int w, int lane, FwdMlpA& A) {
  static_for<2>([&]<int hf>() {
    static_for<16>([&]<int k>() {
      A.w1[hf][k] = img[L.w1c + ((hf * 4 + w) * 16 + k) * 64 + lane];
      A.w2[hf][k] = img[(hf == 0 ? L.w2d : L.w2g) + (w * 16 + k) * 64 + lane];
    });
    A.b2[hf] = *(const f32x4*)(img + L.b2 + hf * 4 * 64 + w * 64 + 4 * (lane >> 4));
  });
  A.wl = img[L.wl + w * 64 + lane];
}

template <int SAVE>
__device__ __forceinline__ f32x4 mlp_forward_split(const FwdMlpA& A, const f32x4 (&t1)[2], const f32x4 (&x)[4], float hb, float* hs, int w,
                                                   int lane, float* p1_out, float* p2_out) {
  f32x4 p1d = t1[0], p1g = t1[1];
  __builtin_amdgcn_s_setprio(1);
  static_for<4>([&]<int blk>() {
    static_for<4>([&]<int r>() {
      const float b = x[blk][r];
      p1d = mfma16(A.w1[0][blk * 4 + r], b, p1d);
      p1g = mfma16(A.w1[1][blk * 4 + r], b, p1g);
    });
  });
  __builtin_amdgcn_s_setprio(0);
  if constexpr (SAVE == 2) {
    f32x4 dsd, dsg;
    static_for<2>([&]<int k>() {
      f32x2 act, der;
      silu_pair(f32x2{p1d[2 * k], p1d[2 * k + 1]}, act, der);
      p1d[2 * k] = act[0]; p1d[2 * k + 1] = act[1];
      dsd[2 * k] = der[0]; dsd[2 * k + 1] = der[1];
      silu_pair(f32x2{p1g[2 * k], p1g[2 * k + 1]}, act, der);
      p1g[2 * k] = act[0]; p1g[2 * k + 1] = act[1];
      dsg[2 * k] = der[0]; dsg[2 * k + 1] = der[1];
    });
    __builtin_nontemporal_store(dsd, (f32x4*)(p1_out + w * 256));
    __builtin_nontemporal_store(dsg, (f32x4*)(p1_out + (4 + w) * 256));
  } else {
    static_for<4>([&]<int r>() { p1d[r] = fsilu(p1d[r]); p1g[r] = fsilu(p1g[r]); });
  }
  split_publish(hs, w, lane, p1d, p1g);
  f32x4 hid[8];
  split_collect(hs, lane, hid);
  f32x4 p2d = A.b2[0], p2g = A.b2[1];
  __builtin_amdgcn_s_setprio(1);
  chain_reg16<0>(A.w2[0], hid, p2d);
  chain_reg16<4>(A.w2[1], hid, p2g);
  __builtin_amdgcn_s_setprio(0);
  if constexpr (SAVE == 2) {
    __builtin_nontemporal_store(p2d, (f32x4*)(p2_out + w * 256));
    __builtin_nontemporal_store(p2g, (f32x4*)(p2_out + (4 + w) * 256));
  }
  f32x4 out = mfma16(A.wl, hb, zero4());
  mul_gated<true>(out, p2d, p2g);
  return out;
}

template <int TBS, bool FIRST, int SAVE>
__global__ void __launch_bounds__(64 * kSplitWaves) k_edge_fwd_split(FwdArgs a, MfmaFwdLayout L) {
  __shared__ __attribute__((aligned(16))) float xs[4 * 256];
  __shared__ __attribute__((aligned(16))) float hs[8 * 256];
  const int lane = threadIdx.x & 63, qd = lane >> 4;
  const int w = __builtin_amdgcn_readfirstlane((int)(threadIdx.x >> 6));
  if ((int64_t)blockIdx.x >= a.tiles) return;
  float a_tb[2][TBS];
  static_for<2>([&]<int hf>() { static_for<TBS>([&]<int s>() { a_tb[hf][s] = a.img[L.tb + ((hf * 4 + w) * kTbSteps + s) * 64 + lane]; }); });
  FwdMlpA A0, A1;
  load_fwd_mlp(a.img, L.mlp[0], w, lane, A0);
  load_fwd_mlp(a.img, L.mlp[1], w, lane, A1);
  float a_adj = 0.f;
  if (FIRST) a_adj = a.img[L.adj + w * 64 + lane];
  for (int64_t tile = blockIdx.x; tile < a.tiles; tile += gridDim.x) {
    const int64_t edge = tile * kTileEdges + (lane & 15);
    const int64_t ec = edge < a.E ? edge : a.E - 1;
    const int64_t ci = a.src[ec], cj = a.dst[ec];
    const int arow = a.act_id[ec];
    const float hb = a.h[ec * kRP + qd];
    float mb[TBS];
    static_for<TBS>([&]<int s>() { mb[s] = arow >= 0 ? a.m[(int64_t)arow * kCP + 4 * s + qd] : 0.f; });
    f32x4 t1[2][2];
    static_for<2>([&]<int mlp>() {
      static_for<2>([&]<int hf>() {
        const int off = mlp * (2 * kDP) + 4 * qd + (hf * 4 + w) * 16;
        t1[mlp][hf] = *(const f32x4*)(a.TA + ci * (4 * kDP) + off) + *(const f32x4*)(a.TB + cj * (4 * kDP) + off);
      });
    });
    f32x4 xw;
    if (FIRST) {
      xw = mfma16(a_adj, hb, zero4());
      static_for<4>([&]<int r>() { xw[r] = fsilu(xw[r]); });
    } else {
      xw = load_tile4(a.e_in + tile * kTileFloats + w * 256 + lane * 4);
    }
    {
      f32x4 pd = zero4(), pg = zero4();
      static_for<TBS>([&]<int s>() {
        pd = mfma16(a_tb[0][s], mb[s], pd);
        pg = mfma16(a_tb[1][s], mb[s], pg);
      });
      add_gated<true>(xw, pd, pg);
    }
    f32x4 x[4];
    *(f32x4*)(xs + w * 256 + lane * 4) = xw;
    __syncthreads();
    static_for<4>([&]<int blk>() { x[blk] = *(const f32x4*)(xs + blk * 256 + lane * 4); });
    float* p1_tile = SAVE == 2 ? a.p1_out + tile * (2 * kP1TileFloats) + lane * 4 : nullptr;
    float* p2_tile = SAVE == 2 ? a.p2_out + tile * (2 * kP1TileFloats) + lane * 4 : nullptr;
    f32x4 out = mlp_forward_split<SAVE>(A0, t1[0], x, hb, hs, w, lane, p1_tile, p2_tile);
    xw += out;
    *(f32x4*)(a.e_out + tile * kTileFloats + w * 256 + lane * 4) = xw;
    *(f32x4*)(xs + w * 256 + lane * 4) = xw;
    __syncthreads();
    static_for<4>([&]<int blk>() { x[blk] = *(const f32x4*)(xs + blk * 256 + lane * 4); });
    out = mlp_forward_split<SAVE>(A1, t1[1], x, hb, hs, w, lane, SAVE == 2 ? p1_tile + kP1TileFloats : nullptr,
                                  SAVE == 2 ? p2_tile + kP1TileFloats : nullptr);
    f32x4 msg[1] = {edge < a.E ? out : zero4()};
    const SegMasks sk = seg_masks((int)ci, lane);
    seg_scan(msg, sk);
    seg_store(msg, sk, a.seg_head, a.seg_first, tile, ci, qd, w);
  }
}

template <int TBS, bool NEED_DP1>
__global__ void __launch_bounds__(64 * kSplitWaves) __attribute__((amdgpu_waves_per_eu(2, 2))) k_edge_rev_split(RevArgs a, MfmaRevF32Layout L) {
  __shared__ __attribute__((aligned(16))) float scratch[kRevSplitGroupFloats + kRevSplitTabFloats];
  if ((int64_t)blockIdx.x >= a.tiles) return;
  const int lane = threadIdx.x & 63;
  const int w = __builtin_amdgcn_readfirstlane((int)(threadIdx.x >> 6));
  rev_split_run<TBS, NEED_DP1>(a, L, a.img, scratch, 1, 0, w, lane, (int64_t)blockIdx.x, a.tiles, (int64_t)gridDim.x);
}

}

void launch_edge_fwd_split(const m3g_plan* plan, const StepPath& p, const Consts& c, const Topo& t, const Work& w, int b, hipStream_t s) {
  const int64_t tiles = tiles_for(t.E);
  if (tiles == 0) return;
  const int save = p.fwd_save;
  const MfmaFwdLayout L = mfma_fwd_layout();
  FwdArgs a = fwd_args(t, w, b, plan->d_mfma_fwd[kPrecF32] + (size_t)b * L.total);
  if (save == 2) { a.p1_out = w.p1_blk[b]; a.p2_out = w.p2_blk[b]; }
  const dim3 grid(grid_for_split(tiles)), block(64 * kSplitWaves);
  const bool first = b == 0 && p.fused_rev;
#define M3G_FWDS(FIRST_) \
  if (save == 2) { M3G_TBS_SWITCH(c.C, hipLaunchKernelGGL((k_edge_fwd_split<TBS, FIRST_, 2>), grid, block, 0, s, a, L)); } \
  else { M3G_TBS_SWITCH(c.C, hipLaunchKernelGGL((k_edge_fwd_split<TBS, FIRST_, 0>), grid, block, 0, s, a, L)); }
  if (first) { M3G_FWDS(true); } else { M3G_FWDS(false); }
#undef M3G_FWDS
}

void launch_edge_rev_split(const m3g_plan* plan, const StepPath& p, const Consts& c, const Topo& t, const Work& w, int b, const float* dx_new, bool de_is_zero,
                           hipStream_t s) {
  const int64_t tiles = tiles_for(t.E);
  if (tiles == 0) return;
  const MfmaRevF32Layout L = mfma_rev_f32_layout();
  RevArgs ar = rev_args(t, w, b, plan->d_mfma_revf32 + (size_t)b * L.total, dx_new, de_is_zero, b);
  ar.seg_head = w.seg_head; ar.seg_first = w.seg_first; ar.p1 = w.p1_blk[b]; ar.p2 = w.p2_blk[b];
  if (p.dp1_by_dst) ar.in_pos = t.in_pos;
  const dim3 grid(grid_for_split(tiles)), block(64 * kSplitWaves);
  if (b > 0) { M3G_TBS_SWITCH(c.C, hipLaunchKernelGGL((k_edge_rev_split<TBS, true>), grid, block, 0, s, ar, L)); }
  else { M3G_TBS_SWITCH(c.C, hipLaunchKernelGGL((k_edge_rev_split<TBS, false>), grid, block, 0, s, ar, L)); }
}

}
```

### torch-m3gnet_amd/csrc/m3g_geometry.hip

```cpp
#include "m3g_internal.h"
#include "m3g_struct_sum.h"
#include "m3g_geometry_body.h"

namespace m3g {

template <bool FULL, int L, int R>
__global__ void __launch_bounds__(256) k_geometry(Consts c, GeomArgs a) {
  geometry_body<FULL, L, R>(c, a, blockIdx.x);
}

__global__ void __launch_bounds__(256) k_geometry_reverse(GeomRev a, float* __restrict__ dr) {
  int64_t e = blockIdx.x * (int64_t)blockDim.x + threadIdx.x;
  if (e >= a.E) return;
  float rx, ry, rz;
  edge_dr(a, e, rx, ry, rz);
  dr[e * 3 + 0] = rx;
  dr[e * 3 + 1] = ry;
  dr[e * 3 + 2] = rz;
}

__device__ __forceinline__ float inv_volume(const float* __restrict__ L) {
  const float cx = L[4] * L[8] - L[5] * L[7], cy = L[5] * L[6] - L[3] * L[8], cz = L[3] * L[7] - L[4] * L[6];
  return 1.f / fabsf(L[0] * cx + L[1] * cy + L[2] * cz);
}
// ... 82 lines not shown
                                                            const float* __restrict__ dr, float* __restrict__ stresses) {
  __shared__ float part[kStructThreads * 6];
  float tot[6];
  struct_reduce<6, kStructThreads>(blockIdx.x, struct_ptr, flags, n_atoms, batch, tot, part, [&](int a, int s, float* v) {
    const float inv = -inv_volume(lattice + (int64_t)s * 9);
#pragma unroll
    for (int k = 0; k < 6; ++k) v[k] = 0.f;
    for (int e = row_ptr[a]; e < row_ptr[a + 1]; ++e) {
      const float d = dist[e];
      const float rx = d * u[e * 3], ry = d * u[e * 3 + 1], rz = d * u[e * 3 + 2];
      const float gx = dr[e * 3], gy = dr[e * 3 + 1], gz = dr[e * 3 + 2];
      v[0] += rx * gx; v[1] += ry * gy; v[2] += rz * gz;
      v[3] += 0.5f * (ry * gz + rz * gy); v[4] += 0.5f * (rz * gx + rx * gz); v[5] += 0.5f * (rx * gy + ry * gx);
    }
#pragma unroll
    for (int k = 0; k < 6; ++k) v[k] *= inv;
  });
  if (threadIdx.x < 6) stresses[(int64_t)blockIdx.x * 6 + threadIdx.x] = tot[threadIdx.x];
}

__global__ void __launch_bounds__(kStructThreads) k_struct_energy(const int32_t* __restrict__ struct_ptr, const int32_t* __restrict__ flags,
                                                       int64_t n_atoms, const int32_t* __restrict__ batch, const float* __restrict__ ea,
                                                       float energy_scale, float* __restrict__ scaled_total, float* __restrict__ total) {
  __shared__ float part[kStructThreads];
  struct_energy<kStructThreads>(blockIdx.x, struct_ptr, flags, n_atoms, batch, ea, energy_scale, scaled_total, total, part);
}
void launch_energy_sums(const Consts& c, const Topo& t, const float* ea, float* scaled_total, float* total, hipStream_t s) {
  if (t.S > 0)
    hipLaunchKernelGGL(k_struct_energy, dim3((unsigned)t.S), dim3(kStructThreads), 0, s, t.struct_ptr, t.flags, t.N, t.batch, ea, c.energy_scale,
                       scaled_total, total);
}


__global__ void __launch_bounds__(256) k_triplet_angles(int64_t T, const int64_t* __restrict__ tei, const float* __restrict__ u,
                                                        float* __restrict__ out) {
  int64_t t = blockIdx.x * (int64_t)blockDim.x + threadIdx.x;
  if (t >= T) return;
  int64_t e1 = tei[t], e2 = tei[T + t];
  float c = u[e1 * 3] * u[e2 * 3] + u[e1 * 3 + 1] * u[e2 * 3 + 1] + u[e1 * 3 + 2] * u[e2 * 3 + 2];
  c = fminf(1.f, fmaxf(-1.f, c));
  if (fabsf(c) > 1.f - 2.4e-7f) c = copysignf(1.f, c);
  out[t] = c;
}

__global__ void __launch_bounds__(256) k_edge_featurizer(Consts c, int64_t E, const float* __restrict__ d, float* __restrict__ out,
                                                         int out_stride) {
  int64_t e = blockIdx.x * (int64_t)blockDim.x + threadIdx.x;
  if (e >= E) return;
  float h[kRCap], hp[kRCap];
  radial_basis(c, d[e], h, hp);
  for (int m = 0; m < c.R; ++m) out[e * out_stride + m] = h[m];
}

void launch_geometry(const Consts& c, const Topo& t, const float* pos, const float* lattice, const int32_t* shift,
                     const Work& w, hipStream_t s) {
  if (t.E == 0) {
    if (w.sync) (void)hipMemsetAsync(w.sync, 0, sizeof(int32_t) * kSyncWords, s);
    return;
  }
  const GeomArgs a = geometry_args(t, pos, lattice, shift, w);
  M3G_DISPATCH_LR(c.L, c.R, hipLaunchKernelGGL((k_geometry<true, L, R>), grid_for(t.E), dim3(256), 0, s, c, a));
}

void launch_distance_only(float length_scale, const Topo& t, const float* pos, const float* lattice, const int32_t* shift,
                          float* u, float* d, hipStream_t s) {
  if (t.E == 0) return;
  Consts c{};
  c.length_scale = length_scale;
  const GeomArgs a{t.E, t.src, t.dst, t.batch, pos, lattice, shift, u, d, nullptr, nullptr, nullptr, nullptr, nullptr, nullptr, nullptr, nullptr};
  hipLaunchKernelGGL((k_geometry<false, 1, 1>), grid_for(t.E), dim3(256), 0, s, c, a);
}

void launch_geometry_reverse(const Consts& c, const Topo& t, const Work& w, const float* dh, int dh_parts, float* forces,
                             float* stresses, hipStream_t s, bool gather_virial, const float* pos, const float* lattice, bool dr_done) {
  const GeomRev g{t.E, w.u, w.d, w.hp, dh, dh_parts, w.dd, w.du, (t.T > 0 && c.B > 0) ? t.act_id : nullptr};
  if (t.E > 0 && !dr_done) hipLaunchKernelGGL(k_geometry_reverse, grid_for(t.E), dim3(256), 0, s, g, w.dr);
  if (t.N > 0) {
    StressTail st{t.S, t.struct_ptr, t.flags, t.batch, pos, lattice, stresses, gather_virial ? w.sync + kSyncForceTail : nullptr};
    hipLaunchKernelGGL(k_force_gather, grid_for(t.N * 16), dim3(256), 0, s, c.length_scale, t.N, t.row_ptr, t.in_ptr, t.in_edge,
                       w.dr, forces, stresses, (stresses && !gather_virial) ? 6 * t.S : 0, st);
  } else if (stresses) {
    (void)hipMemsetAsync(stresses, 0, sizeof(float) * 6 * t.S, s);
  }
}

void launch_force_gather(float length_scale, const Topo& t, const float* dr, float* forces, float* stresses, hipStream_t s) {
  if (t.N > 0)
    hipLaunchKernelGGL(k_force_gather, grid_for(t.N * 16), dim3(256), 0, s, length_scale, t.N, t.row_ptr, t.in_ptr, t.in_edge, dr, forces,
                       stresses, stresses ? 6 * t.S : 0, StressTail{});
  else if (stresses)
    (void)hipMemsetAsync(stresses, 0, sizeof(float) * 6 * t.S, s);
}

void launch_stress(const Consts& c, const Topo& t, const float* pos, const float* lattice, const float* forces,
                   float* stresses, hipStream_t s, const float* ea, float* scaled_total, float* total) {
  if (t.S > 0)
    hipLaunchKernelGGL(k_struct_stress, dim3((unsigned)t.S), dim3(kStructThreads), 0, s, t.struct_ptr, t.flags, t.N, t.batch, pos, lattice, forces,
                       stresses, ea, c.energy_scale, scaled_total, total);
}

void launch_stress_pair(const Topo& t, const Work& w, const float* lattice, float* stresses, hipStream_t s) {
  if (t.S > 0)
    hipLaunchKernelGGL(k_struct_stress_pair, dim3((unsigned)t.S), dim3(kStructThreads), 0, s, t.struct_ptr, t.flags, t.N, t.batch, t.row_ptr, lattice,
                       w.u, w.d, w.dr, stresses);
}

void launch_triplet_angles(const Topo& t, const int64_t* tei, const float* u, float* out, hipStream_t s) {
  if (t.T > 0) hipLaunchKernelGGL(k_triplet_angles, grid_for(t.T), dim3(256), 0, s, t.T, tei, u, out);
}

void launch_edge_featurizer(const Consts& c, int64_t E, const float* d, float* out, int out_stride, hipStream_t s) {
  if (E > 0) hipLaunchKernelGGL(k_edge_featurizer, grid_for(E), dim3(256), 0, s, c, E, d, out, out_stride);
}

}
```

### torch-m3gnet_amd/csrc/m3g_geometry_body.h

```cpp
#pragma once
#include "m3g_internal.h"
#include "m3g_basis.h"

namespace m3g {

__device__ __forceinline__ void radial_basis(const Consts& c, float d, float* h, float* hp) {
  float f = 0.f, df = 0.f;
#pragma unroll
  for (int m = 0; m < kRCap; ++m) {
    if (m < c.R) {
      if (m > 0) { f = h[m - 1]; df = hp[m - 1]; }
      radial_term(c, m, d, f, df);
      h[m] = f;
      hp[m] = df;
    } else {
      h[m] = 0.f;
      hp[m] = 0.f;
    }
  }
}

struct GeomArgs {
  int64_t E;
  const int32_t *src, *dst, *batch;
  const float *pos, *lattice;
  const int32_t* shift;
  float *u, *dist, *h, *hp, *q, *qp, *fc3, *fc3p;
  const int32_t* act_id;
  int32_t* sync;
};
template <bool FULL, int L, int R>
__device__ __forceinline__ void geometry_body(const Consts& c, const GeomArgs& a, int64_t vblock) {
  const int64_t E = a.E;
  const int32_t* __restrict__ src = a.src;
  const int32_t* __restrict__ dst = a.dst;
  const int32_t* __restrict__ batch = a.batch;
  const float* __restrict__ pos = a.pos;
  const float* __restrict__ lattice = a.lattice;
  const int32_t* __restrict__ shift = a.shift;
  float* __restrict__ u = a.u;
  float* __restrict__ dist = a.dist;
  float* __restrict__ h = a.h;
  float* __restrict__ hp = a.hp;
  float* __restrict__ q = a.q;
  float* __restrict__ qp = a.qp;
  float* __restrict__ fc3 = a.fc3;
  float* __restrict__ fc3p = a.fc3p;
  const int32_t* __restrict__ act_id = a.act_id;
  int32_t* __restrict__ sync = a.sync;
  int64_t e = vblock * (int64_t)blockDim.x + threadIdx.x;
  if (sync && vblock == 0 && threadIdx.x < kSyncWords) sync[threadIdx.x] = 0;
  if (e >= E) return;
  int i = src[e], j = dst[e], s = batch[i];
  float ls = c.length_scale;
  float r[3];
  float sh0 = (float)shift[e * 3 + 0], sh1 = (float)shift[e * 3 + 1], sh2 = (float)shift[e * 3 + 2];
#pragma unroll
  for (int a = 0; a < 3; ++a) {
    float l0 = lattice[s * 9 + 0 + a] / ls, l1 = lattice[s * 9 + 3 + a] / ls, l2 = lattice[s * 9 + 6 + a] / ls;
    float sv = (sh0 * l0 + sh1 * l1) + sh2 * l2;
    r[a] = (pos[(int64_t)j * 3 + a] / ls + sv) - pos[(int64_t)i * 3 + a] / ls;
  }
  float d = sqrtf(r[0] * r[0] + r[1] * r[1] + r[2] * r[2]);
  dist[e] = d;
  u[e * 3 + 0] = r[0] / d;
  u[e * 3 + 1] = r[1] / d;
  u[e * 3 + 2] = r[2] / d;
  if (!FULL) return;
  float hh[kRCap], hd[kRCap];
  radial_basis(c, d, hh, hd);
  *(float4*)(h + e * kRP) = float4{hh[0], hh[1], hh[2], hh[3]};
  *(float4*)(hp + e * kRP) = float4{hd[0], hd[1], hd[2], hd[3]};
  const Envelope env = envelope(d, c.rc3);
  const float f = env.f, fp = env.fp;
  fc3[e] = f;
  fc3p[e] = fp;
  const int ar = act_id[e];
  if (ar < 0) return;
  float qr[kCP], qpr[kCP];
#pragma unroll
  for (int cc = 0; cc < kCP; ++cc) { qr[cc] = 0.f; qpr[cc] = 0.f; }
#pragma unroll
  for (int n = 0; n < R; ++n) {
#pragma unroll
    for (int l = 0; l < L; ++l) {
      float jl[kLCap], djl[kLCap];
      float x = c.zeros[l][n] * d / c.rc;
      sph_bessel<kLCap, true>(kLCap, x, jl, djl);
      float chi = jl[l] / c.factors[l][n];
      float dchi = djl[l] * (c.zeros[l][n] / c.rc) / c.factors[l][n];
      qr[l * R + n] = chi * f;
      qpr[l * R + n] = dchi * f + chi * fp;
    }
  }
#pragma unroll
  for (int cc = 0; cc < kCP; cc += 4) {
    *(float4*)(q + (int64_t)ar * kCP + cc) = float4{qr[cc], qr[cc + 1], qr[cc + 2], qr[cc + 3]};
    *(float4*)(qp + (int64_t)ar * kCP + cc) = float4{qpr[cc], qpr[cc + 1], qpr[cc + 2], qpr[cc + 3]};
  }
}


struct GeomRev {
  int64_t E;
  const float *u, *dist, *hp, *dh;
  int dh_parts;
  const float *dd, *du;
  const int32_t* act_id;
};
__device__ __forceinline__ void edge_dr(const GeomRev& a, int64_t e, float& rx, float& ry, float& rz) {
#pragma clang fp contract(off)
  const int ar = a.act_id ? a.act_id[e] : -1;
  float g = ar >= 0 ? a.dd[ar] : 0.f;
  float dhs[kRP] = {0.f, 0.f, 0.f, 0.f};
  for (int p = 0; p < a.dh_parts; ++p) {
    const float4 t = *(const float4*)(a.dh + ((int64_t)p * a.E + e) * kRP);
    dhs[0] += t.x; dhs[1] += t.y; dhs[2] += t.z; dhs[3] += t.w;
  }
  {
    const float4 t = *(const float4*)(a.hp + e * kRP);
    float dot = dhs[1] * t.y;
    dot = __builtin_fmaf(dhs[0], t.x, dot);
    dot = __builtin_fmaf(dhs[2], t.z, dot);
    dot = __builtin_fmaf(dhs[3], t.w, dot);
    g = g + dot;
  }
  const float ux = a.u[e * 3], uy = a.u[e * 3 + 1], uz = a.u[e * 3 + 2];
  float ax = 0.f, ay = 0.f, az = 0.f;
  if (ar >= 0) { ax = a.du[(int64_t)ar * 3]; ay = a.du[(int64_t)ar * 3 + 1]; az = a.du[(int64_t)ar * 3 + 2]; }
  const float proj = __builtin_fmaf(ax, ux, ay * uy) + az * uz;
  const float inv = 1.f / a.dist[e];
  rx = __builtin_fmaf(g, ux, __builtin_fmaf(-proj, ux, ax) * inv);
  ry = __builtin_fmaf(g, uy, __builtin_fmaf(-proj, uy, ay) * inv);
  rz = __builtin_fmaf(g, uz, __builtin_fmaf(-proj, uz, az) * inv);
}

inline GeomArgs geometry_args(const Topo& t, const float* pos, const float* lattice, const int32_t* shift, const Work& w) {
  return GeomArgs{t.E, t.src, t.dst, t.batch, pos, lattice, shift, w.u, w.d, w.h, w.hp, w.q, w.qp, w.fc3, w.fc3p, t.act_id, w.sync};
}

}
```

### torch-m3gnet_amd/csrc/m3g_internal.h

```cpp
#pragma once
#include <hip/hip_runtime.h>

#include <cmath>
#include <cstddef>
#include <cstdint>
#include <map>
#include <string>
#include <vector>

#include "../../include/m3gnet_hip.h"
#include "m3g_step_path.h"

namespace m3g {

constexpr int kDP = 64;
constexpr int kLCap = 4;
constexpr int kRCap = 4;
constexpr int kRAnyCap = 10;
constexpr int kCP = 16;
constexpr int kRP = 4;

void set_error(const char* fmt, ...);
#define M3G_HIP_CHECK(expr)                                                               \
  do {                                                                                    \
// ... 70 lines not shown
  int w1c;
  int w2d, w2g, b2;
  int w2dT;
  int w2gT;
  int w1cT;
  int wl;
  int total;
};
struct MfmaRevLayout {
  MfmaMlpRev mlp;
  int tb;
  int tbT;
  int total_n;
  int total_e;
  int per_block;
};
struct MfmaMlpFused {
  int w1c;
  int w2d, w2g;
  int b2;
  int wl;
  int wld;
};
struct MfmaRevFusedLayout {
  int tb;
  int tbT;
  MfmaMlpFused mlp[2];
  int adj;
  int adjp;
  int total;
};
struct MfmaMlpRevF32 {
  int w2d, w2g;
  int w1cT;
  int b2;
  int wl;
  int wld;
};
struct MfmaRevF32Layout {
  int tb;
  int tbT;
  MfmaMlpRevF32 mlp[2];
  int adj;
  int adjp;
  int total;
};
MfmaRevF32Layout mfma_rev_f32_layout();
constexpr int kNodeRowBlocks = 33;
constexpr int kNodeImgFloats = kNodeRowBlocks * 16 * 64 + kNodeRowBlocks * 16;
constexpr int kSpeciesRowFloats = kDP + kCP + 2 * 4 * kDP;
constexpr size_t species_tab_v(int num_types) { return (size_t)num_types * kDP; }
constexpr size_t species_tab_ta(int num_types) { return (size_t)num_types * (kDP + kCP); }
constexpr size_t species_tab_tb(int num_types) { return (size_t)num_types * (kDP + kCP + 4 * kDP); }
struct ReadoutImg {
  static constexpr int w1 = 0;
  static constexpr int w2d = w1 + 8 * 2 * 512;
  static constexpr int w2g = w2d + 4 * 2 * 512;
  static constexpr int w2dT = w2g + 4 * 2 * 512;
  static constexpr int w2gT = w2dT + 4 * 2 * 512;
  static constexpr int w1T = w2gT + 4 * 2 * 512;
  static constexpr int b1 = w1T + 4 * 4 * 512;
  static constexpr int b2 = b1 + 128;
  static constexpr int w3 = b2 + 128;
  static constexpr int b3 = w3 + 128;
  static constexpr int total = b3 + 4;
};
MfmaFwdLayout mfma_fwd_layout();
MfmaRevLayout mfma_rev_layout();
MfmaRevFusedLayout mfma_rev_fused_layout();

}

struct m3g_plan {
  m3g_config cfg;
  m3g::Consts consts;
  m3g::WeightLayout wl;
  std::map<std::string, std::vector<float>> params;
  std::map<std::string, std::vector<float>> cvals;
  float* d_weights = nullptr;
  float* d_mfma_fwd[m3g::kNumPrec] = {nullptr, nullptr, nullptr};
  float* d_mfma_rev[m3g::kNumPrec] = {nullptr, nullptr, nullptr};
  float* d_mfma_revf = nullptr;
  float* d_mfma_revf_h = nullptr;
  float* d_mfma_revf32 = nullptr;
  float* d_node_img[m3g::kNumPrec] = {nullptr, nullptr, nullptr};
  float* d_species_tab[m3g::kNumPrec] = {nullptr, nullptr, nullptr};
  m3g::Options opt;
  float w_scale_inv = 1.f;
  int device = -1;
  bool generic = false;
  float* d_generic = nullptr;
  std::map<std::string, size_t> generic_off;
  float* d_readout_img = nullptr;
  float* d_readout_img_h = nullptr;
  float ro_w_scale_inv = 1.f;
  unsigned long long* d_stamps = nullptr;
  bool committed = false;
  bool debug_force_move = false;
  mutable hipStream_t side_stream = nullptr;
  mutable hipEvent_t ev_fork = nullptr, ev_join = nullptr;
  struct GraphEntry { std::vector<unsigned char> key; hipGraph_t graph = nullptr; hipGraphExec_t exec = nullptr; };
  mutable std::vector<GraphEntry> graphs;
  bool profile = false;
  mutable std::vector<hipEvent_t> ev_pool;
  mutable std::vector<int> ev_stage;
  mutable size_t ev_used = 0;
};

namespace m3g {

inline size_t align_up(size_t x, size_t a = 256) { return (x + a - 1) / a * a; }
inline dim3 grid_for(int64_t n, int per = 256) { return dim3((unsigned)((n + per - 1) / per)); }
struct Carve {
  uintptr_t base;
  size_t off = 0;
  explicit Carve(const void* b) : base((uintptr_t)b) {}
  template <class T> T* take(size_t count) { T* r = (T*)(base + off); off += align_up(sizeof(T) * count); return r; }
  void* take(size_t bytes) { return take<char>(bytes); }
};
inline size_t carve_offset(const void* p) { return (size_t)(uintptr_t)p; }

template <class C>
inline void fill_radial_consts(C& c, int R, double rc, const float* coeff, const float* em, const float* dm) {
  const float pi_f = (float)M_PI;
  for (int m = 0; m < R; ++m) {
    c.a1[m] = ((float)(m + 1) * pi_f) / (float)rc;
    c.a2[m] = ((float)(m + 2) * pi_f) / (float)rc;
    c.coeff[m] = coeff[m];
    c.rec_mul[m] = m > 0 ? sqrtf(em[m] / dm[m - 1]) : 0.f;
    c.rec_div[m] = sqrtf(dm[m]);
  }
}
template <class C>
inline void fill_angular_consts(C& c, int L, int R, double rc, double rc3, const float* zeros, const float* factors) {
  c.rc = (float)rc;
  c.rc3 = (float)rc3;
  for (int l = 0; l < L; ++l) {
    c.ynorm[l] = (float)std::sqrt((2 * l + 1) / (4.0 * M_PI));
    for (int n = 0; n < R; ++n) {
// ... 41 lines not shown
  int32_t* in_edge;
  int32_t* in_pos;
  int32_t* in_pair;
  int32_t* t1_ptr;
  int32_t* t1_e2;
  int32_t* t2_ptr;
  int32_t* t2_e1;
  int32_t* act_list;
  int32_t* act_scan;
  int32_t* act_id;
  int32_t* arow_ptr;
  int32_t* t1_e2c;
  int32_t* t2_e1c;
  uint8_t* t1_b;
  uint8_t* t2_b;
  int32_t* act_dst;
  int32_t* tb_win;
  int32_t* tb_fast;
  int32_t* n_act;
  int32_t* batch;
  int32_t* struct_ptr;
  int32_t* flags;
  void* sort_tmp;
  size_t sort_tmp_bytes;
  size_t total_bytes;
};
Topo topo_carve(int64_t N, int64_t E, int64_t T, int64_t S, void* base);
size_t topo_sort_tmp_bytes(int64_t E, int64_t T);

inline float* dp1_scale_of(float* dp1, int64_t E) { return dp1 ? dp1 + (size_t)E * 192 : nullptr; }
struct Work {
  float *u, *d, *h, *hp, *q, *qp, *fc3, *fc3p;
  float* x[kMaxBlocks + 1];
  float* v[kMaxBlocks];
  float *TA, *TB;
  float* e;
  float* m[kMaxBlocks];
  float* act[kMaxBlocks];
  float *dx, *dx2;
  float* de;
  float* dm;
  float* g;
  float* dg;
  float* dh;
  float* dd;
  float* du;
  float* dp1;
  float* dr;
  float* e_blk[kMaxBlocks + 1];
  float* p2_blk[kMaxBlocks];
  float* p1_blk[kMaxBlocks];
  float* TAb[kMaxBlocks];
  float* TBb[kMaxBlocks];
  float* de_soa;
  float* dcn;
  float* dh_parts;
  float* seg_head;
  float* seg_first;
  float* tail;
  int32_t* sync;
  size_t total_bytes;
};
Work work_carve(int B, const StepPath& path , int64_t N, int64_t E, int64_t S, void* base);

void launch_geometry(const Consts& c, const Topo& t, const float* pos, const float* lattice, const int32_t* shift,
                     const Work& w, hipStream_t s);
void launch_geometry_reverse(const Consts& c, const Topo& t, const Work& w, const float* dh, int dh_parts, float* forces,
                             float* stresses, hipStream_t s, bool gather_virial = false, const float* pos = nullptr, const float* lattice = nullptr,
                             bool dr_done = false);
void launch_stress(const Consts& c, const Topo& t, const float* pos, const float* lattice, const float* forces,
                   float* stresses, hipStream_t s, const float* ea = nullptr, float* scaled_total = nullptr, float* total = nullptr);
void launch_stress_pair(const Topo& t, const Work& w, const float* lattice, float* stresses, hipStream_t s);
void launch_force_gather(float length_scale, const Topo& t, const float* dr, float* forces, float* stresses, hipStream_t s);
size_t generic_workspace_bytes(const m3g_plan* plan, int64_t N, int64_t E, int64_t T, int64_t S);
int generic_commit(m3g_plan* plan);
void generic_free(m3g_plan* plan);
int generic_energy_forces(const m3g_plan* plan, const m3g_io* io, void* workspace, size_t workspace_bytes, hipStream_t s);
void generic_edge_featurizer(int n_max, double rc, const float* coeff, const float* em, const float* dm, int64_t E, const float* d, float* out,
                             hipStream_t s);
void launch_triplet_angles(const Topo& t, const int64_t* tei, const float* u, float* out, hipStream_t s);
void launch_distance_only(float length_scale, const Topo& t, const float* pos, const float* lattice,
                          const int32_t* shift, float* u, float* d, hipStream_t s);
void launch_edge_featurizer(const Consts& c, int64_t E, const float* d, float* out, int out_stride, hipStream_t s);
void launch_embed(const Consts& c, const float* W, const WeightLayout& wl, const Topo& t, const int64_t* types,
                  const Work& w, hipStream_t s);
void launch_embed_reverse(const Consts& c, const float* W, const WeightLayout& wl, const Topo& t, const Work& w,
                          hipStream_t s);
void launch_node_pre(const Consts& c, const float* W, const BlockW& bw, const Topo& t, const Work& w, const float* x_prev, float* x,
                     float* v, float* TA, float* TB, hipStream_t s);
void launch_node_pre_mfma(const m3g_plan* plan, bool split, const Consts& c, const Topo& t, const Work& w, int b, const float* x_prev, float* x,
                          float* v, float* TA, float* TB, const int64_t* types, const float* emb, hipStream_t s);
void launch_geometry_node_pre(const m3g_plan* plan, const Consts& c, const Topo& t, const Work& w, const float* pos, const float* lattice,
                              const int32_t* shift, const int64_t* types, const float* emb, hipStream_t s);
void launch_species_expand(const m3g_plan* plan, const Consts& c, const Topo& t, const Work& w, const int64_t* types, hipStream_t s);
void launch_geometry_species(const m3g_plan* plan, const Consts& c, const Topo& t, const Work& w, const float* pos, const float* lattice,
                             const int32_t* shift, const int64_t* types, hipStream_t s);
int build_species_tables(m3g_plan* plan);
void launch_energy_sums(const Consts& c, const Topo& t, const float* scaled_atomic, float* scaled_total, float* total, hipStream_t s);
void launch_readout_mfma(const m3g_plan* plan, const StepPath& p, const Consts& c, const WeightLayout& wl, const Topo& t, const int64_t* types,
                         const float* x_prev, float* x, const Work& w, float* scaled_atomic, float* scaled_total, float* total,
                         bool want_grad, hipStream_t s);
void launch_node_reverse(const Consts& c, const float* W, const BlockW& bw, const Topo& t, const Work& w,
                         const float* v, const float* dx_new, float* dx_out, bool row_sums_in_seg, int dp1_packed, bool with_v_term,
                         hipStream_t s, bool small = false);
void launch_node_reverse_v_term(const Consts& c, const float* W, const BlockW& bw, const Topo& t, const Work& w, const float* v,
                                float* dx_out, hipStream_t s);
void launch_readout(const Consts& c, const float* W, const WeightLayout& wl, const Topo& t, const int64_t* types,
                    const float* x_prev, float* x, const Work& w, float* scaled_atomic, float* scaled_total, float* total,
                    bool want_grad, hipStream_t s);
void launch_gather_rows(const float* table, int64_t n, int width, int table_stride, int table_rows, bool transposed,
                        const int64_t* idx, float* out, hipStream_t s);
void launch_copy_expand_rows(const int32_t* row_id, const float* in, int in_stride, float* out, int out_stride, int width, int64_t n,
                             hipStream_t s);
void launch_copy_strided(const float* in, int in_stride, float* out, int out_stride, int width, int64_t rows,
                         hipStream_t s);
void launch_threebody(const StepPath& p, const Consts& c, const Topo& t, const Work& w, const float* v, float* m, hipStream_t s);
void launch_threebody_reverse(const StepPath& p, const Consts& c, const Topo& t, const Work& w, const float* v, bool first, hipStream_t s,
                              bool ref_legendre = false);
void launch_threebody_reverse_final(const Consts& c, const Topo& t, const Work& w, const float* v, bool first, const float* dh, int dh_parts,
                                    hipStream_t s, int topo_hints);
bool launch_node_tb_reverse(const Consts& c, const float* W, const BlockW& bw, const Topo& t, const Work& w, const float* v, bool first,
                            const float* dx_new, float* dx_out, int dp1_packed, int block, hipStream_t s, int topo_hints, int debug_polls = 0);
int pack_mfma_images(m3g_plan* plan);
void free_mfma_images(m3g_plan* plan);
void launch_edge_block_mfma(const m3g_plan* plan, const StepPath& p, const Consts& c, const Topo& t, const Work& w, int b, hipStream_t s,
                            bool e_out_read = true);
void launch_edge_rev_node_mlp(const m3g_plan* plan, const StepPath& p, const Consts& c, const Topo& t, const Work& w, int b, const float* dx_new,
                              hipStream_t s);
void launch_edge_rev_edge_mlp(const m3g_plan* plan, const StepPath& p, const Consts& c, const Topo& t, const Work& w, int b, const float* dx_new,
                              bool de_is_zero, hipStream_t s);
void launch_edge_rev_fused(const m3g_plan* plan, const Consts& c, const Topo& t, const Work& w, int b, const float* dx_new,
                           bool de_is_zero, hipStream_t s);
void launch_edge_rev_f32(const m3g_plan* plan, const StepPath& p, const Consts& c, const Topo& t, const Work& w, int b, const float* dx_new,
                         bool de_is_zero, hipStream_t s);
void launch_edge_fwd_split(const m3g_plan* plan, const StepPath& p, const Consts& c, const Topo& t, const Work& w, int b, hipStream_t s);
void launch_edge_rev_split(const m3g_plan* plan, const StepPath& p, const Consts& c, const Topo& t, const Work& w, int b, const float* dx_new, bool de_is_zero,
                           hipStream_t s);
void launch_embed_edges_soa(const Consts& c, const float* adj_t, const float* h, float* soa, int64_t E, hipStream_t s);
void launch_embed_edges_reverse_soa(const float* adj, const float* h, const float* de_soa, float* dh_slice, int64_t E, hipStream_t s);
void launch_embed_nodes_only(const Consts& c, const float* W, const WeightLayout& wl, const Topo& t, const int64_t* types,
                             const Work& w, hipStream_t s);
void launch_rows_to_soa(const float* rows, float* soa, int64_t E, hipStream_t s);
void launch_soa_to_rows(const float* soa, float* rows, int row_stride, int width, int64_t E, hipStream_t s);
void launch_edge_block(const Consts& c, const float* W, const BlockW& bw, const Topo& t, const Work& w, int b,
                       const float* x_old, float* x_new, hipStream_t s);
void launch_edge_block_reverse(const Consts& c, const float* W, const BlockW& bw, const Topo& t, const Work& w, int b,
                               const float* dx_new, hipStream_t s);

}
```

### torch-m3gnet_amd/csrc/m3g_node_mfma.hip

```cpp
#include "m3g_edge_common.h"
#include "m3g_struct_sum.h"
#include "m3g_geometry_body.h"

namespace m3g {


constexpr int kNodeXPitch = 68;
__device__ __forceinline__ void add_message_sums(f32x4 (&xr)[4], int64_t atom, int q, const float* __restrict__ seg_head,
                                                 const float* __restrict__ seg_first, const int32_t* __restrict__ row_ptr) {
  const int r0 = row_ptr[atom], r1 = row_ptr[atom + 1];
  if (r1 > r0) {
    if (r0 & 15) static_for<4>([&]<int j>() { xr[j] += *(const f32x4*)(seg_first + atom * (4 * kDP) + 16 * q + 4 * j); });
    for (int t = (r0 + 15) >> 4; t <= (r1 - 1) >> 4; ++t)
      static_for<4>([&]<int j>() { xr[j] += *(const f32x4*)(seg_head + (int64_t)t * (4 * kDP) + 16 * q + 4 * j); });
  }
}
__device__ __forceinline__ void store_x_row(float* __restrict__ x, int64_t atom, int q, const f32x4 (&xr)[4]) {
  static_for<4>([&]<int j>() { *(f32x4*)(x + atom * kDP + 16 * q + 4 * j) = xr[j]; });
}
__device__ __forceinline__ void x_rows_to_blocks(float* xs, int m, int q, const f32x4 (&xr)[4], f32x4 (&xb)[4]) {
  static_for<4>([&]<int j>() { *(f32x4*)(xs + m * kNodeXPitch + 16 * q + 4 * j) = xr[j]; });
  static_for<4>([&]<int blk>() { xb[blk] = *(const f32x4*)(xs + m * kNodeXPitch + blk * 16 + 4 * q); });
}
__device__ __forceinline__ void store_node_block(int ob, const f32x4& acc, int64_t atom, int q, int C, float* __restrict__ TA, float* __restrict__ TB,
// ... 106 lines not shown
    const int j = w + 4 * jj;
    const int ob = 11 * g + (j < 11 ? j : 0);
    static_for<16>([&]<int k>() { a[jj][k] = img[(ob * 16 + k) * 64 + lane]; });
    acc[jj] = *(const f32x4*)(img + kNodeRowBlocks * 16 * 64 + ob * 16 + 4 * q);
  });
  const int64_t atom = tile * 16 + m;
  const bool live = atom < N;
  f32x4 xr[4];
  static_for<4>([&]<int j>() { xr[j] = zero4(); });
  if (live) {
    const float* src = (x_prev ? x_prev : x) + atom * kDP + 16 * q;
    if (types) {
      int64_t ty = types[atom];
      ty = ty < 0 ? 0 : (ty >= num_types ? num_types - 1 : ty);
      src = emb + ty * kDP + 16 * q;
    }
    static_for<4>([&]<int j>() { xr[j] = *(const f32x4*)(src + 4 * j); });
    if (types && g == 0 && w == 0) store_x_row(x, atom, q, xr);
    if (x_prev) {
      add_message_sums(xr, atom, q, seg_head, seg_first, row_ptr);
      if (g == 0 && w == 0) store_x_row(x, atom, q, xr);
    }
  }
  f32x4 xb[4];
  x_rows_to_blocks(xs, m, q, xr, xb);
  static_for<4>([&]<int blk>() {
    static_for<4>([&]<int r>() {
      const float b = xb[blk][r];
      static_for<3>([&]<int jj>() { acc[jj] = mfma16(a[jj][blk * 4 + r], b, acc[jj]); });
    });
  });
  if (!live) return;
  static_for<3>([&]<int jj>() {
    const int j = w + 4 * jj;
    if (j >= 11) return;
    store_node_block(11 * g + j, acc[jj], atom, q, C, TA, TB, v);
  });
}

__global__ void __launch_bounds__(256) k_node_pre_split(NodePreArgs a) { node_pre_split_body(a, blockIdx.x); }
template <int L, int R>
__global__ void __launch_bounds__(256) k_geometry_node_pre(Consts c, GeomArgs ga, int n_geo, NodePreArgs na) {
  if ((int)blockIdx.x < n_geo) geometry_body<true, L, R>(c, ga, blockIdx.x);
  else node_pre_split_body(na, (int64_t)blockIdx.x - n_geo);
}

struct SpeciesArgs {
  int64_t N;
  const int64_t* types;
  int num_types;
  const float* tab;
  float *x, *v, *TA, *TB;
};
constexpr int kSpeciesRowVecs = kSpeciesRowFloats / 4, kSpeciesVecsPerThread = 4;
__device__ __forceinline__ void species_expand_body(const SpeciesArgs& a, int64_t vblock) {
  const int64_t total = a.N * kSpeciesRowVecs;
  const int64_t first = vblock * (256 * kSpeciesVecsPerThread) + threadIdx.x;
  const float* __restrict__ tab = a.tab;
  const int64_t* __restrict__ types = a.types;
  const int nt = a.num_types;
  f32x4 t[kSpeciesVecsPerThread];
  float* dst[kSpeciesVecsPerThread];
  static_for<kSpeciesVecsPerThread>([&]<int j>() {
    const int64_t i = first + j * 256;
    dst[j] = nullptr;
    if (i >= total) return;
    const int64_t atom = i / kSpeciesRowVecs;
    const int piece = (int)(i - atom * kSpeciesRowVecs);
    bool bad;
    const int64_t ty = species_index(types[atom], nt, bad);
    const float* src;
    if (piece < 16) {
      src = tab + ty * kDP + 4 * piece;
      dst[j] = a.x + atom * kDP + 4 * piece;
    } else if (piece < 20) {
      src = tab + species_tab_v(nt) + ty * kCP + 4 * (piece - 16);
      dst[j] = a.v + atom * kCP + 4 * (piece - 16);
    } else if (piece < 84) {
      src = tab + species_tab_ta(nt) + ty * (4 * kDP) + 4 * (piece - 20);
      dst[j] = a.TA + atom * (4 * kDP) + 4 * (piece - 20);
    } else {
      src = tab + species_tab_tb(nt) + ty * (4 * kDP) + 4 * (piece - 84);
      dst[j] = a.TB + atom * (4 * kDP) + 4 * (piece - 84);
    }
    t[j] = *(const f32x4*)src;
  });
  static_for<kSpeciesVecsPerThread>([&]<int j>() {
    if (dst[j]) *(f32x4*)dst[j] = t[j];
  });
}
static_assert(kSpeciesRowVecs == 16 + 4 + 64 + 64, "species_expand_body: the pieces of a row");

__global__ void __launch_bounds__(256) k_species_expand(SpeciesArgs a) { species_expand_body(a, blockIdx.x); }
template <int L, int R>
__global__ void __launch_bounds__(256) k_geometry_species(Consts c, GeomArgs ga, int n_geo, SpeciesArgs sa) {
  if ((int)blockIdx.x < n_geo) geometry_body<true, L, R>(c, ga, blockIdx.x);
  else species_expand_body(sa, (int64_t)blockIdx.x - n_geo);
}

struct ReadoutSums {
  const int32_t *struct_ptr, *flags, *batch;
  float* total;
  int32_t* counter;
};
template <int PREC>
__global__ void __launch_bounds__(256) k_readout_mfma(Consts c, int64_t N, const float* __restrict__ img, float w_inv, const float* __restrict__ elemental,
                                                      const int64_t* __restrict__ types, const float* __restrict__ x_prev,
                                                      const float* __restrict__ seg_head, const float* __restrict__ seg_first,
                                                      const int32_t* __restrict__ row_ptr, float* __restrict__ x,
                                                      float* scaled_atomic, float* __restrict__ dx,
                                                      float* __restrict__ scaled_total, int64_t S, ReadoutSums rs) {
  __shared__ __attribute__((aligned(16))) float lds[ReadoutImg::total + 4 * 16 * kNodeXPitch];
  if (blockIdx.x == 0) for (int64_t i = threadIdx.x; i < S; i += blockDim.x) scaled_total[i] = 0.f;
  {
    constexpr int kVec = ReadoutImg::total / 4, kBatch = 16;
    for (int base = 0; base < kVec; base += 256 * kBatch) {
      f32x4 t[kBatch];
      static_for<kBatch>([&]<int j>() {
        const int i = base + j * 256 + (int)threadIdx.x;
        t[j] = i < kVec ? *(const f32x4*)(img + 4 * i) : zero4();
      });
      static_for<kBatch>([&]<int j>() {
        const int i = base + j * 256 + (int)threadIdx.x;
        if (i < kVec) *(f32x4*)(lds + 4 * i) = t[j];
      });
    }
  }
  __syncthreads();
  const int lane = threadIdx.x & 63, wave = threadIdx.x >> 6, m = lane & 15, q = lane >> 4;
  float* xs = lds + ReadoutImg::total + wave * 16 * kNodeXPitch;
  const int64_t tiles = (N + 15) / 16;
  for (int64_t tile = (int64_t)blockIdx.x * 4 + wave; tile < tiles; tile += (int64_t)gridDim.x * 4) {
    const int64_t atom = tile * 16 + m;
    const bool live = atom < N;
    f32x4 xr[4];
    static_for<4>([&]<int j>() { xr[j] = zero4(); });
    if (live) {
      const float* src = (x_prev ? x_prev : x) + atom * kDP + 16 * q;
      static_for<4>([&]<int j>() { xr[j] = *(const f32x4*)(src + 4 * j); });
      if (x_prev) {
        add_message_sums(xr, atom, q, seg_head, seg_first, row_ptr);
        static_for<4>([&]<int j>() { *(f32x4*)(x + atom * kDP + 16 * q + 4 * j) = xr[j]; });
      }
    }
    f32x4 xb[4];
    x_rows_to_blocks(xs, m, q, xr, xb);
    int lv = lane;
    asm volatile("" : "+v"(lv));
    f32x4 p1[8], hid[8];
    static_for<8>([&]<int ob>() { p1[ob] = *(const f32x4*)(lds + ReadoutImg::b1 + ob * 16 + 4 * q); });
// ... 176 lines not shown
  if (!rs.counter) return;
  if (!last_workgroup(rs.counter)) return;
  for (int sidx = 0; sidx < (int)S; ++sidx)
    struct_energy<256>(sidx, rs.struct_ptr, rs.flags, N, rs.batch, scaled_atomic, c.energy_scale, scaled_total, rs.total, xs);
}

void launch_readout_mfma(const m3g_plan* plan, const StepPath& p, const Consts& c, const WeightLayout& wl, const Topo& t, const int64_t* types,
                         const float* x_prev, float* x, const Work& w, float* scaled_atomic, float* scaled_total, float* total,
                         bool want_grad, hipStream_t s) {
  if (t.N == 0) (void)hipMemsetAsync(scaled_total, 0, sizeof(float) * t.S, s);
  if (t.N > 0) {
    const int64_t tiles = (t.N + 15) / 16;
    const int wgs = (int)std::min<int64_t>((tiles + 3) / 4, 256);
    const ReadoutSums rs{t.struct_ptr, t.flags, t.batch, total, p.readout_sums ? w.sync + kSyncReadout : nullptr};
    auto launch = [&](auto kernel, unsigned grid, const float* img, auto... w_inv) {
      hipLaunchKernelGGL(kernel, dim3(grid), dim3(256), 0, s, c, t.N, img, w_inv..., plan->d_weights + wl.elemental, types, x_prev, w.seg_head,
                         w.seg_first, t.row_ptr, x, scaled_atomic, want_grad ? w.dx : nullptr, scaled_total, t.S, rs);
    };
    if (p.readout == kReadoutSplit) {
      if (want_grad) launch(k_readout_split<true>, (unsigned)tiles, plan->d_readout_img);
      else launch(k_readout_split<false>, (unsigned)tiles, plan->d_readout_img);
    } else if (p.readout == kReadoutF16) {
      launch(k_readout_mfma<kPrecF16x3>, (unsigned)wgs, plan->d_readout_img_h, plan->ro_w_scale_inv);
    } else {
      launch(k_readout_mfma<kPrecF32>, (unsigned)wgs, plan->d_readout_img, 1.f);
    }
  }
  if (!p.readout_sums && !p.energy_deferred) launch_energy_sums(c, t, scaled_atomic, scaled_total, total, s);
}

void launch_node_pre_mfma(const m3g_plan* plan, bool split, const Consts& c, const Topo& t, const Work& w, int b, const float* x_prev, float* x,
                          float* v, float* TA, float* TB, const int64_t* types, const float* emb, hipStream_t s) {
  if (t.N == 0) return;
  const int64_t tiles = (t.N + 15) / 16;
  const int prec = plan->opt.precision;
  if (split) {
    const NodePreArgs a{c.C, t.N, plan->d_node_img[kPrecF32] + (size_t)b * kNodeImgFloats, x_prev, w.seg_head, w.seg_first, t.row_ptr, x, v, TA, TB,
                        types, emb, c.num_types};
    hipLaunchKernelGGL(k_node_pre_split, dim3((unsigned)(3 * tiles)), dim3(256), 0, s, a);
    return;
  }
  const int wgs = 3 * (int)std::min<int64_t>((tiles + 3) / 4, 256);
  M3G_PREC_SWITCH(prec,
                  hipLaunchKernelGGL((k_node_pre_mfma<PREC>), dim3(wgs), dim3(256), 0, s, c.C, t.N,
                                     plan->d_node_img[prec] + (size_t)b * kNodeImgFloats, x_prev, w.seg_head, w.seg_first,
                                     t.row_ptr, x, v, TA, TB, types, emb, c.num_types,
                                     prec == kPrecF16x3 ? plan->w_scale_inv : 1.f));
}

void launch_geometry_node_pre(const m3g_plan* plan, const Consts& c, const Topo& t, const Work& w, const float* pos, const float* lattice,
                              const int32_t* shift, const int64_t* types, const float* emb, hipStream_t s) {
  const int64_t tiles = (t.N + 15) / 16;
  const int n_geo = (int)((t.E + 255) / 256);
  const GeomArgs ga = geometry_args(t, pos, lattice, shift, w);
  const NodePreArgs na{c.C, t.N, plan->d_node_img[kPrecF32], nullptr, w.seg_head, w.seg_first, t.row_ptr, w.x[0], w.v[0], w.TAb[0], w.TBb[0], types, emb,
                       c.num_types};
  M3G_DISPATCH_LR(c.L, c.R, hipLaunchKernelGGL((k_geometry_node_pre<L, R>), dim3((unsigned)(n_geo + 3 * tiles)), dim3(256), 0, s, c, ga, n_geo, na));
}

static SpeciesArgs species_args(const m3g_plan* plan, const Consts& c, const Topo& t, const Work& w, const int64_t* types) {
  return SpeciesArgs{t.N, types, c.num_types, plan->d_species_tab[plan->opt.precision], w.x[0], w.v[0], w.TAb[0], w.TBb[0]};
}
static unsigned species_expand_blocks(int64_t N) {
  constexpr int64_t per = 256 * kSpeciesVecsPerThread;
  return (unsigned)((N * kSpeciesRowVecs + per - 1) / per);
}
void launch_species_expand(const m3g_plan* plan, const Consts& c, const Topo& t, const Work& w, const int64_t* types, hipStream_t s) {
  hipLaunchKernelGGL(k_species_expand, dim3(species_expand_blocks(t.N)), dim3(256), 0, s, species_args(plan, c, t, w, types));
}
void launch_geometry_species(const m3g_plan* plan, const Consts& c, const Topo& t, const Work& w, const float* pos, const float* lattice,
                             const int32_t* shift, const int64_t* types, hipStream_t s) {
  const int n_geo = (int)((t.E + 255) / 256);
  const GeomArgs ga = geometry_args(t, pos, lattice, shift, w);
  const SpeciesArgs sa = species_args(plan, c, t, w, types);
  M3G_DISPATCH_LR(c.L, c.R, hipLaunchKernelGGL((k_geometry_species<L, R>), dim3((unsigned)n_geo + species_expand_blocks(t.N)), dim3(256), 0, s, c, ga, n_geo, sa));
}

int build_species_tables(m3g_plan* plan) {
  const int nt = plan->cfg.num_types;
  if (plan->cfg.num_blocks == 0) return M3G_OK;
  std::vector<int64_t> iota(nt);
  for (int i = 0; i < nt; ++i) iota[i] = i;
  int64_t* d_types = nullptr;
  M3G_HIP_CHECK(hipMalloc((void**)&d_types, sizeof(int64_t) * nt));
  hipError_t e = hipMemcpy(d_types, iota.data(), sizeof(int64_t) * nt, hipMemcpyHostToDevice);
  const int64_t tiles = (nt + 15) / 16;
  const int wgs = 3 * (int)std::min<int64_t>((tiles + 3) / 4, 256);
  for (int prec = 0; prec < kNumPrec && e == hipSuccess; ++prec) {
    float*& tab = plan->d_species_tab[prec];
    if (!tab) e = hipMalloc((void**)&tab, sizeof(float) * (size_t)nt * kSpeciesRowFloats);
    if (e != hipSuccess) break;
    M3G_PREC_SWITCH(prec,
                    hipLaunchKernelGGL((k_node_pre_mfma<PREC>), dim3(wgs), dim3(256), 0, nullptr, plan->consts.C, (int64_t)nt, plan->d_node_img[prec],
                                       nullptr, nullptr, nullptr, nullptr, tab, tab + species_tab_v(nt), tab + species_tab_ta(nt),
                                       tab + species_tab_tb(nt), d_types, plan->d_weights + plan->wl.emb, nt,
                                       prec == kPrecF16x3 ? plan->w_scale_inv : 1.f));
    e = hipGetLastError();
  }
  if (e == hipSuccess) e = hipDeviceSynchronize();
  (void)hipFree(d_types);
  M3G_HIP_CHECK(e);
  return M3G_OK;
}

}
```

### torch-m3gnet_amd/csrc/m3g_pack_mfma.hip

```cpp
#include <cmath>
#include <cstring>

#include "m3g_dual_chain.h"
#include "m3g_dual_f32.h"
#include "m3g_internal.h"

namespace m3g {

MfmaFwdLayout mfma_fwd_layout() {
  MfmaFwdLayout L{};
  int off = 0;
  auto take = [&](int n) { int r = off; off += n; return r; };
  L.tb = take(8 * kTbSteps * 64);
  for (int m = 0; m < 2; ++m) {
    L.mlp[m].w1c = take(8 * 4 * 4 * 64);
    L.mlp[m].w2d = take(4 * 4 * 4 * 64);
    L.mlp[m].w2g = take(4 * 4 * 4 * 64);
    L.mlp[m].b2 = take(2 * 4 * 64);
    L.mlp[m].wl = take(4 * 1 * 64);
  }
  L.adj = take(4 * 64);
  L.total = off;
  return L;
}
// ... 83 lines not shown
static void chain_image_h(float* img, int OB, int KS, float scale, F get) {
  uint16_t* hi = reinterpret_cast<uint16_t*>(img);
  uint16_t* lo = hi + (size_t)OB * KS * 512;
  for (int ob = 0; ob < OB; ++ob)
    for (int s = 0; s < KS; ++s)
      for (int lane = 0; lane < 64; ++lane)
        for (int j = 0; j < 8; ++j) {
          const int feat = (2 * s + (j >> 2)) * 16 + 4 * (lane >> 4) + (j & 3);
          const float w = get(ob * 16 + (lane & 15), feat) * scale;
          const uint16_t h = f16_rne(w);
          const size_t idx = (((size_t)ob * KS + s) * 64 + lane) * 8 + j;
          hi[idx] = h;
          lo[idx] = f16_rne(w - f16_to_float(h));
        }
}
template <class F>
static void tb_image_h(float* img, float scale, F get) {
  uint16_t* hi = reinterpret_cast<uint16_t*>(img);
  uint16_t* lo = hi + 8 * 32 * 8;
  for (int ob = 0; ob < 8; ++ob)
    for (int lane = 0; lane < 32; ++lane)
      for (int j = 0; j < 8; ++j) {
        const float w = get(ob * 16 + (lane & 15), 8 * (lane >> 4) + j) * scale;
        const uint16_t h = f16_rne(w);
        const size_t idx = ((size_t)ob * 32 + lane) * 8 + j;
        hi[idx] = h;
        lo[idx] = f16_rne(w - f16_to_float(h));
      }
}
template <class F>
static void direct_image(float* img, int OB, int S, F get) {
  for (int ob = 0; ob < OB; ++ob)
    for (int s = 0; s < S; ++s)
      for (int lane = 0; lane < 64; ++lane) img[(ob * S + s) * 64 + lane] = get(ob * 16 + (lane & 15), 4 * s + (lane >> 4));
}

template <class F>
static void f32_chain_image(float* img, int OB, int S, F get) {
  for (int ob = 0; ob < OB; ++ob)
    for (int s = 0; s < S; ++s)
      for (int lane = 0; lane < 64; ++lane)
        img[(ob * S + s) * 64 + lane] = get(ob * 16 + (lane & 15), (s >> 2) * 16 + 4 * (lane >> 4) + (s & 3));
}

template <class F>
static void chain_image_p(int prec, float wscale, float* img, int OB, int KS, F get) {
  if (prec == kPrecBf16x3) chain_image(img, OB, KS, get);
  else if (prec == kPrecF16x3) chain_image_h(img, OB, KS, wscale, get);
  else f32_chain_image(img, OB, 8 * KS, get);
}

void free_mfma_images(m3g_plan* plan) {
  auto drop = [](float*& p) { if (p) { (void)hipFree(p); p = nullptr; } };
  for (int prec = 0; prec < kNumPrec; ++prec) { drop(plan->d_mfma_fwd[prec]); drop(plan->d_mfma_rev[prec]); drop(plan->d_node_img[prec]); drop(plan->d_species_tab[prec]); }
  drop(plan->d_mfma_revf);
  drop(plan->d_mfma_revf_h);
  drop(plan->d_mfma_revf32);
  drop(plan->d_readout_img);
  drop(plan->d_readout_img_h);
}

static int upload(float*& dst, const std::vector<float>& host) {
  if (!dst) M3G_HIP_CHECK(hipMalloc((void**)&dst, host.size() * sizeof(float)));
  M3G_HIP_CHECK(hipMemcpy(dst, host.data(), host.size() * sizeof(float), hipMemcpyHostToDevice));
  return M3G_OK;
}

int pack_mfma_images(m3g_plan* plan) {
  const m3g_config& cfg = plan->cfg;
  const int D = cfg.embedding_dim, R = cfg.n_max, C = cfg.l_max * cfg.n_max, B = cfg.num_blocks;
  const MfmaFwdLayout F = mfma_fwd_layout();
  const MfmaRevLayout Rv = mfma_rev_layout();
  const MfmaRevFusedLayout Rf = mfma_rev_fused_layout();
  const MfmaRevF32Layout R32 = mfma_rev_f32_layout();
  std::vector<float> revf((size_t)std::max(B, 1) * Rf.total, 0.f), revf32((size_t)std::max(B, 1) * R32.total, 0.f);
  std::vector<float> revfh((size_t)std::max(B, 1) * Rf.total, 0.f);
  float wscale = 1.f;
  {
    float wmax = 0.f;
    for (const auto& kv : plan->params) {
      const std::string& k = kv.first;
      const bool chain_weight = k.find(".concat_") != std::string::npos || k.find(".gated_mlp.") != std::string::npos ||
                                k.find(".linear_sigmoid1.weight") != std::string::npos;
      if (!chain_weight || k.find(".bias") != std::string::npos) continue;
      for (float v : kv.second) wmax = std::max(wmax, std::fabs(v));
    }
    int e = 0;
    if (wmax > 0.f && std::isfinite(wmax)) (void)std::frexp(wmax, &e);
    wscale = std::ldexp(1.f, 13 - e);
    plan->w_scale_inv = std::ldexp(1.f, e - 13);
  }
  for (int prec = 0; prec < kNumPrec; ++prec) {
  std::vector<float> node((size_t)std::max(B, 1) * kNodeImgFloats, 0.f);
  std::vector<float> fwd((size_t)std::max(B, 1) * F.total, 0.f), rev((size_t)std::max(B, 1) * Rv.per_block, 0.f);
  for (int b = 0; b < B; ++b) {
    float* f = fwd.data() + (size_t)b * F.total;
    float* r = rev.data() + (size_t)b * Rv.per_block;
    const std::string tb = "model." + std::to_string(6 + 2 * b), cv = "model." + std::to_string(7 + 2 * b);
    const float* wd = plan->params.at(tb + ".gated_mlp.dense.0.weight").data();
    const float* wg = plan->params.at(tb + ".gated_mlp.gate.0.weight").data();
    auto tbw = [&](int row, int k) -> float {
      const float* w = row < 64 ? wd : wg;
      int o = row & 63;
      return (o < D && k < C) ? w[(size_t)o * C + k] : 0.f;
    };
    if (prec == kPrecF16x3) tb_image_h(f + F.tb, wscale, tbw);
    else direct_image(f + F.tb, 8, kTbSteps, tbw);
// ... 176 lines not shown
```

### torch-m3gnet_amd/csrc/m3g_step_path.h

```cpp
#pragma once
#include <cstdint>

#include "../../include/m3gnet_hip.h"

namespace m3g {

constexpr int kMaxBlocks = 8;
constexpr int kPrecF32 = 0;
constexpr int kPrecBf16x3 = 1;
constexpr int kPrecF16x3 = 2;
constexpr int kNumPrec = 3;

constexpr int kSyncWords = 16;
constexpr int kSyncForceTail = 0, kSyncReadout = 1, kSyncNodeRev = 2;
constexpr int64_t kForceTailMaxStructs = 8;
constexpr int64_t kFusedSumsMaxAtoms = 1024;
constexpr int64_t kNodeTbFusedMaxAtoms = 128;

constexpr int32_t topo_hints_word(int32_t bad, int32_t rows, int32_t atoms) {
  return (bad == 0 && rows > 0) ? (M3G_TOPO_TB_COMPLETE | ((rows & 0xff) << 8) | ((atoms & 0xff) << 16)) : 0;
}
constexpr int topo_hints_rows(int hints) { return (hints >> 8) & 0xff; }
constexpr int topo_hints_atoms(int hints) { return (hints >> 16) & 0xff; }

struct Options {
  int precision = kPrecF32;
  int save_p1 = 1;
  int save_p2 = 1;
  int small_tiles_fwd = 3072;
  int small_tiles = 1536;
  int dp1_by_dst = 0;
  int split_node_tiles = 128;
  int species_tables = 1;
  int fuse_node_tb = 1;
  int debug_node_tb_polls = 0;
  int split_tail = 1;
  int small_launches = 1;
  int rev_kernel = 1;
  int readout_f16 = 0;
  int legendre_ref = 0;
  int tb_moments = 1;
  int stress_mode = 0;
  int edge_kernel = 1;
  int stamp_target = 0;
  int overlap = 0;
  int graph_replay = 0;
};
static_assert(sizeof(Options) == 21 * sizeof(int), "Options: twenty-one ints, no padding (its bytes are compared as a key)");

enum { kDp1F32 = 0, kDp1Packed = 1, kDp1Fixed = 2, kDp1F32ByDst = 3  };

enum Pipeline { kPipeValu = 0, kPipeMfma = 1, kPipeAnySize = 2 };
enum RevEdge { kRevValu = 0, kRevPair, kRevFused, kRevF32, kRevSplit };
enum Readout { kReadoutValu = 0, kReadoutSplit, kReadoutF32, kReadoutF16 };
enum RevTail {
  kTailSeparate = 0,
  kTailOverlap,
  kTailNodeTb,
  kTailFinalTb,
};
enum Block0Tables {
  kBlock0Kernel = 0,
  kBlock0ExpandBesideGeom,
  kBlock0ExpandAlone,
};
enum StressKernel { kStressNone = 0, kStressInGather , kStressPair, kStressRef };

struct ModelDims { int L, R, C, B; };

struct StepPath {
  int pipeline = kPipeMfma;
  bool fused_rev = false;
  int saved_acts = 0;
  int fwd_save = 0;
  int dp1 = kDp1F32;
  bool dp1_by_dst = false;
  int tb_hints = 0;
  bool moments = false;
  bool long_lists = false;
  bool geom_with_node_pre = false;
  int block0 = kBlock0Kernel;
  bool node_split = false;
  bool fwd_split = false;
  int rev_edge = kRevValu;
  int split_tail = 0;
  int readout = kReadoutValu;
  bool readout_sums = false;
  bool energy_deferred = false;
  int tail[kMaxBlocks] = {};
  bool node_rev_small = false;
  bool gather_virial = false;
  int stress = kStressNone;
};

inline StepPath resolve_step_path(const Options& o, const ModelDims& m, int64_t N, int64_t E, int64_t T, int64_t S, int topo_hints,
                                  bool want_forces, bool want_stresses, bool profile) {
  StepPath p;
  p.pipeline = o.edge_kernel;
  if (o.edge_kernel == 2) return p;
  const bool mfma = o.edge_kernel == 1, f32 = o.precision == kPrecF32, stamps = o.stamp_target != 0;
  const bool saves_p1 = mfma && f32 && o.save_p1 != 0;
  const bool saves_p2 = saves_p1 && o.rev_kernel == 1 && o.save_p2 != 0;
  p.saved_acts = saves_p2 ? 2 : saves_p1 ? 1 : 0;
  p.fwd_save = want_forces ? p.saved_acts : 0;
  p.fused_rev = mfma && o.rev_kernel == 1 && (!f32 || saves_p1);
  p.dp1_by_dst = o.dp1_by_dst && p.fused_rev && f32;
  p.dp1 = !p.fused_rev ? kDp1F32 : p.dp1_by_dst ? kDp1F32ByDst : o.precision == kPrecBf16x3 ? kDp1Packed : o.precision == kPrecF16x3 ? kDp1Fixed : kDp1F32;

  p.tb_hints = o.tb_moments && !o.legendre_ref ? topo_hints : 0;
  p.moments = (p.tb_hints & M3G_TOPO_TB_COMPLETE) && m.L >= 1 && m.L <= 3 && m.R >= 1 && m.R <= 4 && topo_hints_rows(p.tb_hints) > 0 &&
              topo_hints_atoms(p.tb_hints) > 0;
  p.long_lists = T > 24 * E;
  const bool tb_mom = p.moments && E != 0 && T != 0;

  const int64_t etiles = (E + 15) / 16, ntiles = (N + 15) / 16;
  const bool small_nodes = o.small_launches && ntiles <= o.split_node_tiles;
  const bool few = N <= kFusedSumsMaxAtoms && S > 0 && S <= kForceTailMaxStructs;
  if (mfma) {
    p.node_split = f32 && small_nodes;
    p.geom_with_node_pre = !profile && p.node_split && m.B != 0 && E != 0 && N != 0;
    if (o.species_tables && m.B != 0 && N != 0) p.block0 = !profile && E != 0 ? kBlock0ExpandBesideGeom : kBlock0ExpandAlone;
    p.fwd_split = etiles > 0 && etiles <= o.small_tiles_fwd && f32 && p.fwd_save != 1 && !stamps;
    p.rev_edge = !p.fused_rev ? kRevPair : !f32 ? kRevFused : (etiles > 0 && etiles <= o.small_tiles && saves_p2 && !stamps) ? kRevSplit : kRevF32;
    p.split_tail = o.split_tail;
    const bool f16_readout = o.precision == kPrecF16x3 && o.readout_f16;
    p.readout = f16_readout ? kReadoutF16 : small_nodes ? kReadoutSplit : kReadoutF32;
    p.readout_sums = o.small_launches && N > 0 && few;
    p.energy_deferred = o.small_launches && want_forces && want_stresses && o.stress_mode == 0 && !profile && !p.readout_sums && N > 0;
  }
  if (!want_forces) return p;
  for (int b = 0; b < m.B && b < kMaxBlocks; ++b) {
    if (b > 0 && p.fused_rev && o.overlap && !profile) p.tail[b] = kTailOverlap;
    else if (b > 0 && p.fused_rev && o.fuse_node_tb && !profile && N <= kNodeTbFusedMaxAtoms && N != 0 && tb_mom && kSyncNodeRev + b < kSyncWords)
      p.tail[b] = kTailNodeTb;
    else if (b == 0 && p.fused_rev && o.small_launches && !profile && tb_mom) p.tail[b] = kTailFinalTb;
  }
  p.node_rev_small = o.small_launches && N <= kFusedSumsMaxAtoms;
  p.gather_virial = mfma && o.small_launches && o.stress_mode == 0 && want_stresses && N > 0 && few;
  p.stress = !want_stresses ? kStressNone : p.gather_virial ? kStressInGather : o.stress_mode == 1 ? kStressPair : kStressRef;
  return p;
}

}
```

Baseline: 4.328 million atom-steps/s.

## Precompute species-pair rows for block 0 edge MLP first-layer preactivations

In block 0 the per-node tables TA and TB depend only on atom species. This change precomputes a num_types² table of TA[zi]+TB[zj] at commit time, and the geometry kernel writes a per-edge pair row index. The block-0 forward and reverse edge kernels then gather one row instead of two and skip the add. The per-node TAb/TBb expansion for block 0 is also dropped, which saves memory and species-expand work, at the cost of an extra int32-per-edge array and more kernel template variants.

```diff
diff --git a/torch-m3gnet_amd/csrc/m3g_api.hip b/torch-m3gnet_amd/csrc/m3g_api.hip
--- a/torch-m3gnet_amd/csrc/m3g_api.hip
+++ b/torch-m3gnet_amd/csrc/m3g_api.hip
@@ -151,7 +151,8 @@
     for (int b = 0; b <= B; ++b) w.e_blk[b] = take(tiles16 * 1024);
     if (path.saved_acts >= 1) for (int b = 0; b < B; ++b) w.p1_blk[b] = take(tiles16 * 2 * 2048);
     if (path.saved_acts >= 2) for (int b = 0; b < B; ++b) w.p2_blk[b] = take(tiles16 * 2 * 2048);
-    for (int b = 0; b < B; ++b) { w.TAb[b] = take(n * 4 * kDP); w.TBb[b] = take(n * 4 * kDP); }
+    for (int b = path.pair_rows ? 1 : 0; b < B; ++b) { w.TAb[b] = take(n * 4 * kDP); w.TBb[b] = take(n * 4 * kDP); }
+    if (path.pair_rows) w.pair_row = (int32_t*)c.take(e * sizeof(int32_t));
     w.de_soa = take(tiles16 * 1024);
     w.dcn = take(tiles16 * 1024);
     w.dh_parts = take((size_t)(2 * B + 1) * e * kRP);
@@ -350,6 +351,7 @@
     {"small_tiles_fwd", &Options::small_tiles_fwd, 0, INT_MAX, "small_tiles_fwd must be >= 0", nullptr},
     {"dp1_by_dst", &Options::dp1_by_dst, 0, 1, nullptr, nullptr},
     {"split_node_tiles", &Options::split_node_tiles, 0, INT_MAX, "split_node_tiles must be >= 0", nullptr},
+    {"pair_rows", &Options::pair_rows, 0, 1, nullptr, nullptr},
     {"species_tables", &Options::species_tables, 0, 1, nullptr, nullptr},
     {"fuse_node_tb", &Options::fuse_node_tb, 0, 1, nullptr, nullptr},
     {"debug_node_tb_polls", &Options::debug_node_tb_polls, INT_MIN, INT_MAX, nullptr, nullptr},
@@ -479,6 +481,7 @@
   M3G_HIP_CHECK(hipMemcpy(plan->d_weights, blob.data(), wl.total * sizeof(float), hipMemcpyHostToDevice));
   { int rc = pack_mfma_images(plan); if (rc) return rc; }
   { int rc = build_species_tables(plan); if (rc) return rc; }
+  { int rc = build_pair_tables(plan); if (rc) return rc; }
   plan->committed = true;
   return M3G_OK;
 }
@@ -546,7 +549,7 @@
     M3G_STAGE(ST_GEOM);
     if (p.block0 == kBlock0ExpandBesideGeom) launch_geometry_species(plan, c, t, w, io->pos, io->lattice, io->edge_cell_shift, io->atom_types, s);
     else if (p.block0 == kBlock0Kernel && p.geom_with_node_pre) launch_geometry_node_pre(plan, c, t, w, io->pos, io->lattice, io->edge_cell_shift, io->atom_types, W + wl.emb, s);
-    else launch_geometry(c, t, io->pos, io->lattice, io->edge_cell_shift, w, s);
+    else launch_geometry(c, t, io->pos, io->lattice, io->edge_cell_shift, io->atom_types, w, s);
   }
   {
     M3G_STAGE(ST_EMBED);
@@ -611,7 +614,7 @@
     switch (p.rev_edge) {
       case kRevSplit: { M3G_STAGE(ST_EDGE_REV_FUSED); launch_edge_rev_split(plan, p, c, t, w, b, dx_cur, first, s); } break;
       case kRevF32: { M3G_STAGE(ST_EDGE_REV_FUSED); launch_edge_rev_f32(plan, p, c, t, w, b, dx_cur, first, s); } break;
-      case kRevFused: { M3G_STAGE(ST_EDGE_REV_FUSED); launch_edge_rev_fused(plan, c, t, w, b, dx_cur, first, s); } break;
+      case kRevFused: { M3G_STAGE(ST_EDGE_REV_FUSED); launch_edge_rev_fused(plan, p, c, t, w, b, dx_cur, first, s); } break;
       case kRevPair: {
         { M3G_STAGE(ST_EDGE_REV_NODE); launch_edge_rev_node_mlp(plan, p, c, t, w, b, dx_cur, s); }
         M3G_STAGE(ST_EDGE_REV);
diff --git a/torch-m3gnet_amd/csrc/m3g_edge_common.h b/torch-m3gnet_amd/csrc/m3g_edge_common.h
--- a/torch-m3gnet_amd/csrc/m3g_edge_common.h
+++ b/torch-m3gnet_amd/csrc/m3g_edge_common.h
@@ -254,6 +254,8 @@
   float* p1_out;
   float* p2_out;
   float w_inv;
+  const int32_t* pair_row;
+  const float* pair_tab;
 };
 
 template <int TBS>
@@ -316,6 +318,16 @@
   const float* ta = TA + ci * (4 * kDP) + mlp * (2 * kDP) + 4 * qd;
   const float* tb = TB + cj * (4 * kDP) + mlp * (2 * kDP) + 4 * qd;
   static_for<8>([&]<int ob>() { p1[ob] = *(const f32x4*)(ta + ob * 16) + *(const f32x4*)(tb + ob * 16); });
+}
+
+__device__ __forceinline__ void gather_pair_row(const float* __restrict__ S, int mlp, int64_t row, int qd, f32x4 (&p1)[8]) {
+  const float* s = S + row * kPairRowFloats + mlp * (2 * kDP) + 4 * qd;
+  static_for<8>([&]<int ob>() { p1[ob] = *(const f32x4*)(s + ob * 16); });
+}
+template <bool PAIR, class ARGS>
+__device__ __forceinline__ void start_rows(const ARGS& a, int mlp, int64_t ci, int64_t cj, int qd, f32x4 (&p1)[8]) {
+  if constexpr (PAIR) gather_pair_row(a.pair_tab, mlp, cj, qd, p1);
+  else gather_tables(a.TA, a.TB, mlp, ci, cj, qd, p1);
 }
 
 __device__ __forceinline__ void gated_out_reverse(f32x4& d2d, f32x4& d2g, const f32x4& d_upd, const f32x4& sl, const float* wl4, f32x4& dhv) {
@@ -381,6 +393,8 @@
   float w_inv;
   float* dp1_scale;
   const int32_t* in_pos;
+  const int32_t* pair_row;
+  const float* pair_tab;
   int split_tail;
 };
 
@@ -414,6 +428,7 @@
   a.E = t.E; a.tiles = tiles_for(t.E); a.img = img;
   a.src = t.src; a.dst = t.dst; a.h = w.h; a.m = w.m[b]; a.TA = w.TAb[b]; a.TB = w.TBb[b]; a.act_id = t.act_id;
   a.e_in = w.e_blk[b]; a.e_out = w.e_blk[b + 1]; a.seg_head = w.seg_head; a.seg_first = w.seg_first; a.w_inv = 1.f;
+  a.pair_row = w.pair_row;
   return a;
 }
 inline RevArgs rev_args(const Topo& t, const Work& w, int b, const float* img, const float* dx_new, bool de_is_zero, int dh_slice) {
@@ -421,9 +436,13 @@
   a.E = t.E; a.tiles = tiles_for(t.E); a.img = img;
   a.src = t.src; a.dst = t.dst; a.h = w.h; a.m = w.m[b]; a.dx_new = dx_new; a.act_id = t.act_id;
   a.de_soa = w.de_soa; a.de_is_zero = de_is_zero ? 1 : 0; a.dm = w.dm; a.dh = w.dh_parts + (size_t)dh_slice * t.E * kRP; a.dp1 = w.dp1;
-  a.w_inv = 1.f;
+  a.w_inv = 1.f; a.pair_row = w.pair_row;
   return a;
 }
+enum { kFwdLater = 0 , kFwdFirst = 1 ,
+       kFwdFirstPair = 2 , kFwdLaterPair = 3  };
+constexpr bool fwd_forms_e0(int first) { return first == kFwdFirst || first == kFwdFirstPair; }
+constexpr bool fwd_pair(int first) { return first == kFwdFirstPair || first == kFwdLaterPair; }
 
 #define M3G_TBS_SWITCH(C_, CALL)                     \
   switch (tb_steps_for(C_)) {                        \
diff --git a/torch-m3gnet_amd/csrc/m3g_edge_mfma.hip b/torch-m3gnet_amd/csrc/m3g_edge_mfma.hip
--- a/torch-m3gnet_amd/csrc/m3g_edge_mfma.hip
+++ b/torch-m3gnet_amd/csrc/m3g_edge_mfma.hip
@@ -47,12 +47,12 @@
   }
 }
 
-template <bool ST, int S0, int PREC, int SAVE>
+template <bool ST, int S0, int PREC, int SAVE, bool PAIR>
 __device__ __forceinline__ void mlp_forward_mfma(const float* lds, const MfmaMlpFwd& L, int mlp, const FwdArgs& a, int64_t ci,
                                                  int64_t cj, float hb, const f32x4 (&x)[4], f32x4 (&out)[4], int lane,
                                                  Stamps<ST>& st, float* p1_out, float* p2_out) {
   f32x4 p1[8], p2[8];
-  gather_tables(a.TA, a.TB, mlp, ci, cj, lane >> 4, p1);
+  start_rows<PAIR>(a, mlp, ci, cj, lane >> 4, p1);
   st.template mark<S0>();
   mlp_preacts<false, PREC, SAVE>(lds, L.w1c, L.w2d, L.w2g, L.b2, x, p1, p2, lane, p1_out, p2_out, a.w_inv);
   st.template mark<S0 + 1>();
@@ -63,8 +63,10 @@
   st.template mark<S0 + 3>();
 }
 
-template <int TBS, bool ST = false, bool FIRST = false, int PREC = kPrecBf16x3, int SAVE = 0, bool STORE_E = true>
+template <int TBS, bool ST = false, int FIRST = kFwdLater, int PREC = kPrecBf16x3, int SAVE = 0, bool STORE_E = true>
 __global__ void __launch_bounds__(64 * fwd_waves<PREC>()) k_edge_block_mfma(FwdArgs a, MfmaFwdLayout L) {
+  constexpr bool PAIR = fwd_pair(FIRST), E0 = fwd_forms_e0(FIRST);
+  const int32_t* __restrict__ ends_j = PAIR ? a.pair_row : a.dst;
   __shared__ __attribute__((aligned(16))) float lds[kFwdLdsFloats + 4];
   int* q_head = reinterpret_cast<int*>(lds + kFwdLdsFloats);
   load_image(lds, a.img, kFwdLdsFloats, q_head);
@@ -74,7 +76,7 @@
   int ticket = queue.fetch(lane);
   if (ticket >= queue.count) return;
   int ci_i, cj_i;
-  load_ends(a.src, a.dst, queue.base + ticket, a.E, lane, ci_i, cj_i);
+  load_ends(a.src, ends_j, queue.base + ticket, a.E, lane, ci_i, cj_i);
   int arow_i = load_arow(a.act_id, queue.base + ticket, a.E, lane);
   for (;;) {
     const int64_t tile = queue.base + ticket;
@@ -82,7 +84,7 @@
     const bool has_next = ticket < queue.count;
     int nci = 0, ncj = 0, narow = -1;
     if (has_next) {
-      load_ends(a.src, a.dst, queue.base + ticket, a.E, lane, nci, ncj);
+      load_ends(a.src, ends_j, queue.base + ticket, a.E, lane, nci, ncj);
       narow = load_arow(a.act_id, queue.base + ticket, a.E, lane);
     }
     int lv = lane;
@@ -92,15 +94,16 @@
     const int64_t ec = edge < a.E ? edge : a.E - 1;
     const int64_t ci = ci_i, cj = cj_i;
     const int qv = lv >> 4;
-    const int tl_out = FIRST ? lv : lane;
+    const int tl_out = E0 ? lv : lane;
+    const int tl_save = FIRST == kFwdFirstPair ? lv : lane;
     const float* e_tile = a.e_in + tile * kTileFloats + lane * 4;
     float* e_otile = a.e_out + tile * kTileFloats + tl_out * 4;
     f32x4 x[4];
-    if (!FIRST) static_for<4>([&]<int blk>() { x[blk] = load_tile4(e_tile + blk * 256); });
+    if (!E0) static_for<4>([&]<int blk>() { x[blk] = load_tile4(e_tile + blk * 256); });
     const int arow = arow_i;
     const TbIn<PREC, TBS> tbin = tb_load<PREC, TBS>(a.m, arow, qv, a.w_inv);
     const float hb = a.h[ec * kRP + qv];
-    if (FIRST) {
+    if (E0) {
       static_for<4>([&]<int blk>() {
         x[blk] = mfma16(lds[L.adj + blk * 64 + lv], hb, zero4());
         static_for<4>([&]<int r>() { x[blk][r] = fsilu(x[blk][r]); });
@@ -114,15 +117,15 @@
     }
     st.template mark<1>();
     f32x4 out[4];
-    float* p1_tile = SAVE >= 1 ? a.p1_out + tile * (2 * kP1TileFloats) + lane * 4 : nullptr;
-    float* p2_tile = SAVE >= 2 ? a.p2_out + tile * (2 * kP1TileFloats) + lane * 4 : nullptr;
-    mlp_forward_mfma<ST, 2, PREC, SAVE>(lds, L.mlp[0], 0, a, ci, cj, hb, x, out, lv, st, p1_tile, p2_tile);
+    float* p1_tile = SAVE >= 1 ? a.p1_out + tile * (2 * kP1TileFloats) + tl_save * 4 : nullptr;
+    float* p2_tile = SAVE >= 2 ? a.p2_out + tile * (2 * kP1TileFloats) + tl_save * 4 : nullptr;
+    mlp_forward_mfma<ST, 2, PREC, SAVE, PAIR>(lds, L.mlp[0], 0, a, ci, cj, hb, x, out, lv, st, p1_tile, p2_tile);
     static_for<4>([&]<int blk>() {
       x[blk] += out[blk];
       if constexpr (STORE_E) *(f32x4*)(e_otile + blk * 256) = x[blk];
     });
     st.template mark<6>();
-    mlp_forward_mfma<ST, 7, PREC, SAVE>(lds, L.mlp[1], 1, a, ci, cj, hb, x, out, lv, st, SAVE >= 1 ? p1_tile + kP1TileFloats : nullptr,
+    mlp_forward_mfma<ST, 7, PREC, SAVE, PAIR>(lds, L.mlp[1], 1, a, ci, cj, hb, x, out, lv, st, SAVE >= 1 ? p1_tile + kP1TileFloats : nullptr,
                                         SAVE >= 2 ? p2_tile + kP1TileFloats : nullptr);
     {
       if (edge >= a.E) static_for<4>([&]<int blk>() { out[blk] = zero4(); });
@@ -157,7 +160,8 @@
     chain_p<PREC, 4, 2, 0, 0>(lds + L.w2d, hid, d2, lane, a.w_inv);
     chain_p<PREC, 4, 2, 4, 4>(lds + L.w2g, hid, d2, lane, a.w_inv);
   } else {
-    gather_tables(a.TA, a.TB, mlp, ci, cj, qd, p1);
+    if (a.pair_tab) gather_pair_row(a.pair_tab, mlp, cj, qd, p1);
+    else gather_tables(a.TA, a.TB, mlp, ci, cj, qd, p1);
     st.template mark<2>();
     mlp_preacts<true, PREC>(lds, L.w1c, L.w2d, L.w2g, L.b2, x, p1, d2, lane, nullptr, nullptr, a.w_inv);
   }
@@ -202,13 +206,14 @@
   int ticket = queue.fetch(lane);
   if (ticket >= queue.count) return;
   int ci_i, cj_i;
-  load_ends(a.src, a.dst, queue.base + ticket, a.E, lane, ci_i, cj_i);
+  const int32_t* __restrict__ ends_j = a.pair_tab ? a.pair_row : a.dst;
+  load_ends(a.src, ends_j, queue.base + ticket, a.E, lane, ci_i, cj_i);
   for (;;) {
     const int64_t tile = queue.base + ticket;
     ticket = queue.fetch(lane);
     const bool has_next = ticket < queue.count;
     int nci = 0, ncj = 0;
-    if (has_next) load_ends(a.src, a.dst, queue.base + ticket, a.E, lane, nci, ncj);
+    if (has_next) load_ends(a.src, ends_j, queue.base + ticket, a.E, lane, nci, ncj);
     int lv = lane;
     asm volatile("" : "+v"(lv));
     const int64_t edge = tile * kTileEdges + (lane & 15);
@@ -245,13 +250,14 @@
   int ticket = queue.fetch(lane);
   if (ticket >= queue.count) return;
   int ci_i, cj_i;
-  load_ends(a.src, a.dst, queue.base + ticket, a.E, lane, ci_i, cj_i);
+  const int32_t* __restrict__ ends_j = a.pair_tab ? a.pair_row : a.dst;
+  load_ends(a.src, ends_j, queue.base + ticket, a.E, lane, ci_i, cj_i);
   for (;;) {
     const int64_t tile = queue.base + ticket;
     ticket = queue.fetch(lane);
     const bool has_next = ticket < queue.count;
     int nci = 0, ncj = 0;
-    if (has_next) load_ends(a.src, a.dst, queue.base + ticket, a.E, lane, nci, ncj);
+    if (has_next) load_ends(a.src, ends_j, queue.base + ticket, a.E, lane, nci, ncj);
     int lv = lane;
     asm volatile("" : "+v"(lv));
     st.start();
@@ -341,7 +347,7 @@
 }
 
 
-template <bool NEED_DP1, int MLP, int PREC, bool ST = false, int S0 = 0>
+template <bool NEED_DP1, int MLP, int PREC, bool ST = false, int S0 = 0, bool PAIR = false>
 __device__ __forceinline__ void mlp_reverse_dual(const float* lds, const MfmaMlpFused& L, const RevArgs& a, int64_t edge, int64_t tile,
                                                  int64_t ci, int64_t cj, const SegMasks& sk, const f32x4& hv, const f32x4 (&x)[4],
                                                  const f32x4 (&d_upd)[4], f32x4 (&contrib)[4], f32x4& dhv, int lane, Stamps<ST>& st,
@@ -349,7 +355,7 @@
   constexpr int mlp = MLP;
   const int qd = lane >> 4;
   f32x4 p1[8], d2[8];
-  gather_tables(a.TA, a.TB, mlp, ci, cj, qd, p1);
+  start_rows<PAIR>(a, mlp, ci, cj, qd, p1);
   cdual<PREC, 8, 2, 128>(lds + L.w1c, x, p1, lane, a.w_inv);
   sched_fence();
   st.template mark<S0>();
@@ -412,8 +418,10 @@
   });
 }
 
-template <int TBS, bool NEED_DP1, int WAVES, int PREC = kPrecBf16x3, bool ST = false>
+template <int TBS, bool NEED_DP1, int WAVES, int PREC = kPrecBf16x3, bool ST = false, bool PAIR = false>
 __global__ void __launch_bounds__(64 * WAVES) k_edge_rev_fused(RevArgs a, MfmaRevFusedLayout L) {
+  static_assert(!PAIR || !NEED_DP1, "pair rows are block 0's");
+  const int32_t* __restrict__ ends_j = PAIR ? a.pair_row : a.dst;
   Stamps<ST> st;
   __shared__ __attribute__((aligned(16))) float lds[kRevFusedFloats + 4];
   int* q_head = reinterpret_cast<int*>(lds + kRevFusedFloats);
@@ -423,7 +431,7 @@
   int ticket = queue.fetch(lane);
   if (ticket >= queue.count) return;
   int ci_i, cj_i;
-  load_ends(a.src, a.dst, queue.base + ticket, a.E, lane, ci_i, cj_i);
+  load_ends(a.src, ends_j, queue.base + ticket, a.E, lane, ci_i, cj_i);
   int arow_i = load_arow(a.act_id, queue.base + ticket, a.E, lane);
   for (;;) {
     const int64_t tile = queue.base + ticket;
@@ -431,7 +439,7 @@
     const bool has_next = ticket < queue.count;
     int nci = 0, ncj = 0, narow = -1;
     if (has_next) {
-      load_ends(a.src, a.dst, queue.base + ticket, a.E, lane, nci, ncj);
+      load_ends(a.src, ends_j, queue.base + ticket, a.E, lane, nci, ncj);
       narow = load_arow(a.act_id, queue.base + ticket, a.E, lane);
     }
     int lv = lane;
@@ -455,7 +463,7 @@
       static_for<4>([&]<int blk>() { x2[blk] = load_tile4(e2_tile + blk * 256); });
       f32x4 dmsg[4];
       load_dmsg(a.dx_new, ci, qd, dmsg);
-      mlp_reverse_dual<NEED_DP1, 1, PREC, ST, 0>(lds, L.mlp[1], a, edge, tile, ci, cj, sk, hv, x2, dmsg, contrib, dhv, lv, st, dp1_inv);
+      mlp_reverse_dual<NEED_DP1, 1, PREC, ST, 0, PAIR>(lds, L.mlp[1], a, edge, tile, ci, cj, sk, hv, x2, dmsg, contrib, dhv, lv, st, dp1_inv);
     }
     de2_from(a.de_is_zero, de_tile, contrib, de);
     asm volatile("" : "+v"(lv));
@@ -475,7 +483,7 @@
       static_for<4>([&]<int blk>() { add_gated<true>(x[blk], p[blk], p[4 + blk]); });
     }
     st.template mark<5>();
-    mlp_reverse_dual<NEED_DP1, 0, PREC, ST, 6>(lds, L.mlp[0], a, edge, tile, ci, cj, sk, hv, x, de, contrib, dhv, lv, st, dp1_inv);
+    mlp_reverse_dual<NEED_DP1, 0, PREC, ST, 6, PAIR>(lds, L.mlp[0], a, edge, tile, ci, cj, sk, hv, x, de, contrib, dhv, lv, st, dp1_inv);
     if (NEED_DP1 && PREC == kPrecF16x3 && qd == 0 && edge < a.E) *(f32x4*)(a.dp1_scale + edge * 4) = dp1_inv;
     de1_from<!FIRST>(de_tile, contrib, de);
     if (FIRST) {
@@ -607,6 +615,9 @@
     if (prec == kPrecF16x3) a.w_inv = plan->w_scale_inv;
     dim3 grid(grid_for_tiles(tiles));
     const bool first = b == 0 && p.fused_rev;
+    const bool pair = b == 0 && p.pair_rows;
+    if (pair) a.pair_tab = plan->d_pair_tab[prec];
+    const int how = first ? (pair ? kFwdFirstPair : kFwdFirst) : (pair ? kFwdLaterPair : kFwdLater);
     const int save = p.fwd_save;
 #define M3G_FWD_LAUNCH(ST_, FIRST_, PREC_, SAVE_) hipLaunchKernelGGL((k_edge_block_mfma<TBS, ST_, FIRST_, PREC_, SAVE_>), grid, dim3(64 * fwd_waves<PREC_>()), 0, s, a, L)
 #define M3G_FWD_BY_MODE(ST_, FIRST_)                                                               \
@@ -618,11 +629,16 @@
   else { M3G_FWD_LAUNCH(ST_, FIRST_, kPrecF32, 0); }
     if (plan->d_stamps && plan->opt.stamp_target == 1 && tb_steps_for(c.C) == 3) {
       constexpr int TBS = 3;
-      if (first) { M3G_FWD_BY_MODE(true, true); } else { M3G_FWD_BY_MODE(true, false); }
-    } else if (first) {
-      M3G_TBS_SWITCH(c.C, M3G_FWD_BY_MODE(false, true));
+      if (how == kFwdFirstPair) { M3G_FWD_BY_MODE(true, kFwdFirstPair); } else if (how == kFwdFirst) { M3G_FWD_BY_MODE(true, kFwdFirst); }
+      else if (how == kFwdLaterPair) { M3G_FWD_BY_MODE(true, kFwdLaterPair); } else { M3G_FWD_BY_MODE(true, kFwdLater); }
+    } else if (how == kFwdFirstPair) {
+      M3G_TBS_SWITCH(c.C, M3G_FWD_BY_MODE(false, kFwdFirstPair));
+    } else if (how == kFwdFirst) {
+      M3G_TBS_SWITCH(c.C, M3G_FWD_BY_MODE(false, kFwdFirst));
+    } else if (how == kFwdLaterPair) {
+      M3G_TBS_SWITCH(c.C, M3G_FWD_BY_MODE(false, kFwdLaterPair));
     } else {
-      M3G_TBS_SWITCH(c.C, M3G_FWD_BY_MODE(false, false));
+      M3G_TBS_SWITCH(c.C, M3G_FWD_BY_MODE(false, kFwdLater));
     }
 #undef M3G_FWD_BY_MODE
 #undef M3G_FWD_LAUNCH
@@ -641,6 +657,7 @@
   RevArgs an = rev_args(t, w, b, img_n, dx_new, false, 2 * b + 1);
   an.TA = w.TAb[b]; an.TB = w.TBb[b]; an.e_tile = w.e_blk[b + 1]; an.dcn = w.dcn;
   if (saved) an.p1 = w.p1_blk[b];
+  else if (b == 0 && p.pair_rows) an.pair_tab = plan->d_pair_tab[prec];
   if (prec == kPrecF16x3) an.w_inv = plan->w_scale_inv;
   if (saved) { M3G_PREC_SWITCH(prec, hipLaunchKernelGGL((k_edge_rev_node_mlp<PREC, true>), dim3(grid_for_tiles(tiles)), dim3(64 * kWavesRev), 0, s, an, L)); }
   else { M3G_PREC_SWITCH(prec, hipLaunchKernelGGL((k_edge_rev_node_mlp<PREC, false>), dim3(grid_for_tiles(tiles)), dim3(64 * kWavesRev), 0, s, an, L)); }
@@ -657,6 +674,7 @@
   RevArgs ae = rev_args(t, w, b, img_e, dx_new, de_is_zero, 2 * b);
   ae.TA = w.TAb[b]; ae.TB = w.TBb[b]; ae.e_tile = w.e_blk[b]; ae.dcn = w.dcn; ae.stamps = plan->d_stamps;
   if (saved) ae.p1 = w.p1_blk[b];
+  else if (b == 0 && p.pair_rows) ae.pair_tab = plan->d_pair_tab[prec];
   if (prec == kPrecF16x3) ae.w_inv = plan->w_scale_inv;
   dim3 grid(grid_for_tiles(tiles)), block(64 * kWavesRev);
   if (plan->d_stamps && plan->opt.stamp_target == 2 && tb_steps_for(c.C) == 3 && prec == kPrecBf16x3) {
@@ -667,7 +685,7 @@
   else { M3G_PREC_SWITCH(prec, M3G_TBS_SWITCH(c.C, hipLaunchKernelGGL((k_edge_rev_edge_mlp<TBS, false, PREC, false>), grid, block, 0, s, ae, L))); }
 }
 
-void launch_edge_rev_fused(const m3g_plan* plan, const Consts& c, const Topo& t, const Work& w, int b, const float* dx_new,
+void launch_edge_rev_fused(const m3g_plan* plan, const StepPath& p, const Consts& c, const Topo& t, const Work& w, int b, const float* dx_new,
                            bool de_is_zero, hipStream_t s) {
   const int64_t tiles = tiles_for(t.E);
   if (tiles == 0) return;
@@ -678,18 +696,22 @@
   ar.TA = w.TAb[b]; ar.TB = w.TBb[b]; ar.e_tile = w.e_blk[b]; ar.e2_tile = w.e_blk[b + 1]; ar.stamps = plan->d_stamps;
   ar.seg_head = w.seg_head; ar.seg_first = w.seg_first; ar.dp1_scale = dp1_scale_of(w.dp1, t.E);
   if (f16) ar.w_inv = plan->w_scale_inv;
+  const bool pair = b == 0 && p.pair_rows;
+  if (pair) ar.pair_tab = plan->d_pair_tab[plan->opt.precision];
   constexpr int WV = kWavesRevFused;
   dim3 grid(grid_for_tiles(tiles)), block(64 * WV);
   if (plan->d_stamps && plan->opt.stamp_target == 3 && f16 && tb_steps_for(c.C) == 3) {
     if (b > 0) hipLaunchKernelGGL((k_edge_rev_fused<3, true, WV, kPrecF16x3, true>), grid, block, 0, s, ar, L);
+    else if (pair) hipLaunchKernelGGL((k_edge_rev_fused<3, false, WV, kPrecF16x3, true, true>), grid, block, 0, s, ar, L);
     else hipLaunchKernelGGL((k_edge_rev_fused<3, false, WV, kPrecF16x3, true>), grid, block, 0, s, ar, L);
     return;
   }
-#define M3G_REVF_LAUNCH(NEED_) \
-  if (f16) { M3G_TBS_SWITCH(c.C, hipLaunchKernelGGL((k_edge_rev_fused<TBS, NEED_, WV, kPrecF16x3>), grid, block, 0, s, ar, L)); } \
-  else { M3G_TBS_SWITCH(c.C, hipLaunchKernelGGL((k_edge_rev_fused<TBS, NEED_, WV, kPrecBf16x3>), grid, block, 0, s, ar, L)); }
-  if (b > 0) { M3G_REVF_LAUNCH(true); }
-  else { M3G_REVF_LAUNCH(false); }
+#define M3G_REVF_LAUNCH(NEED_, PAIR_) \
+  if (f16) { M3G_TBS_SWITCH(c.C, hipLaunchKernelGGL((k_edge_rev_fused<TBS, NEED_, WV, kPrecF16x3, false, PAIR_>), grid, block, 0, s, ar, L)); } \
+  else { M3G_TBS_SWITCH(c.C, hipLaunchKernelGGL((k_edge_rev_fused<TBS, NEED_, WV, kPrecBf16x3, false, PAIR_>), grid, block, 0, s, ar, L)); }
+  if (b > 0) { M3G_REVF_LAUNCH(true, false); }
+  else if (pair) { M3G_REVF_LAUNCH(false, true); }
+  else { M3G_REVF_LAUNCH(false, false); }
 #undef M3G_REVF_LAUNCH
 }
 
diff --git a/torch-m3gnet_amd/csrc/m3g_edge_small.hip b/torch-m3gnet_amd/csrc/m3g_edge_small.hip
--- a/torch-m3gnet_amd/csrc/m3g_edge_small.hip
+++ b/torch-m3gnet_amd/csrc/m3g_edge_small.hip
@@ -72,8 +72,10 @@
   return out;
 }
 
-template <int TBS, bool FIRST, int SAVE>
+template <int TBS, int FIRST, int SAVE>
 __global__ void __launch_bounds__(64 * kSplitWaves) k_edge_fwd_split(FwdArgs a, MfmaFwdLayout L) {
+  constexpr bool PAIR = fwd_pair(FIRST), E0 = fwd_forms_e0(FIRST);
+  const int32_t* __restrict__ ends_j = PAIR ? a.pair_row : a.dst;
   __shared__ __attribute__((aligned(16))) float xs[4 * 256];
   __shared__ __attribute__((aligned(16))) float hs[8 * 256];
   const int lane = threadIdx.x & 63, qd = lane >> 4;
@@ -85,11 +87,11 @@
   load_fwd_mlp(a.img, L.mlp[0], w, lane, A0);
   load_fwd_mlp(a.img, L.mlp[1], w, lane, A1);
   float a_adj = 0.f;
-  if (FIRST) a_adj = a.img[L.adj + w * 64 + lane];
+  if (E0) a_adj = a.img[L.adj + w * 64 + lane];
   for (int64_t tile = blockIdx.x; tile < a.tiles; tile += gridDim.x) {
     const int64_t edge = tile * kTileEdges + (lane & 15);
     const int64_t ec = edge < a.E ? edge : a.E - 1;
-    const int64_t ci = a.src[ec], cj = a.dst[ec];
+    const int64_t ci = a.src[ec], cj = ends_j[ec];
     const int arow = a.act_id[ec];
     const float hb = a.h[ec * kRP + qd];
     float mb[TBS];
@@ -98,11 +100,12 @@
     static_for<2>([&]<int mlp>() {
       static_for<2>([&]<int hf>() {
         const int off = mlp * (2 * kDP) + 4 * qd + (hf * 4 + w) * 16;
-        t1[mlp][hf] = *(const f32x4*)(a.TA + ci * (4 * kDP) + off) + *(const f32x4*)(a.TB + cj * (4 * kDP) + off);
+        if constexpr (PAIR) t1[mlp][hf] = *(const f32x4*)(a.pair_tab + cj * kPairRowFloats + off);
+        else t1[mlp][hf] = *(const f32x4*)(a.TA + ci * (4 * kDP) + off) + *(const f32x4*)(a.TB + cj * (4 * kDP) + off);
       });
     });
     f32x4 xw;
-    if (FIRST) {
+    if (E0) {
       xw = mfma16(a_adj, hb, zero4());
       static_for<4>([&]<int r>() { xw[r] = fsilu(xw[r]); });
     } else {
@@ -156,11 +159,12 @@
   FwdArgs a = fwd_args(t, w, b, plan->d_mfma_fwd[kPrecF32] + (size_t)b * L.total);
   if (save == 2) { a.p1_out = w.p1_blk[b]; a.p2_out = w.p2_blk[b]; }
   const dim3 grid(grid_for_split(tiles)), block(64 * kSplitWaves);
-  const bool first = b == 0 && p.fused_rev;
+  const bool first = b == 0 && p.fused_rev, pair = b == 0 && p.pair_rows;
+  if (pair) a.pair_tab = plan->d_pair_tab[kPrecF32];
 #define M3G_FWDS(FIRST_) \
   if (save == 2) { M3G_TBS_SWITCH(c.C, hipLaunchKernelGGL((k_edge_fwd_split<TBS, FIRST_, 2>), grid, block, 0, s, a, L)); } \
   else { M3G_TBS_SWITCH(c.C, hipLaunchKernelGGL((k_edge_fwd_split<TBS, FIRST_, 0>), grid, block, 0, s, a, L)); }
-  if (first) { M3G_FWDS(true); } else { M3G_FWDS(false); }
+  if (pair && first) { M3G_FWDS(kFwdFirstPair); } else if (first) { M3G_FWDS(kFwdFirst); } else if (pair) { M3G_FWDS(kFwdLaterPair); } else { M3G_FWDS(kFwdLater); }
 #undef M3G_FWDS
 }
 
diff --git a/torch-m3gnet_amd/csrc/m3g_geometry.hip b/torch-m3gnet_amd/csrc/m3g_geometry.hip
--- a/torch-m3gnet_amd/csrc/m3g_geometry.hip
+++ b/torch-m3gnet_amd/csrc/m3g_geometry.hip
@@ -158,13 +158,13 @@
   for (int m = 0; m < c.R; ++m) out[e * out_stride + m] = h[m];
 }
 
-void launch_geometry(const Consts& c, const Topo& t, const float* pos, const float* lattice, const int32_t* shift,
+void launch_geometry(const Consts& c, const Topo& t, const float* pos, const float* lattice, const int32_t* shift, const int64_t* types,
                      const Work& w, hipStream_t s) {
   if (t.E == 0) {
     if (w.sync) (void)hipMemsetAsync(w.sync, 0, sizeof(int32_t) * kSyncWords, s);
     return;
   }
-  const GeomArgs a = geometry_args(t, pos, lattice, shift, w);
+  const GeomArgs a = geometry_args(c, t, pos, lattice, shift, types, w);
   M3G_DISPATCH_LR(c.L, c.R, hipLaunchKernelGGL((k_geometry<true, L, R>), grid_for(t.E), dim3(256), 0, s, c, a));
 }
 
@@ -173,7 +173,7 @@
   if (t.E == 0) return;
   Consts c{};
   c.length_scale = length_scale;
-  const GeomArgs a{t.E, t.src, t.dst, t.batch, pos, lattice, shift, u, d, nullptr, nullptr, nullptr, nullptr, nullptr, nullptr, nullptr, nullptr};
+  const GeomArgs a{t.E, t.src, t.dst, t.batch, pos, lattice, shift, u, d, nullptr, nullptr, nullptr, nullptr, nullptr, nullptr, nullptr, nullptr, nullptr, 0, nullptr};
   hipLaunchKernelGGL((k_geometry<false, 1, 1>), grid_for(t.E), dim3(256), 0, s, c, a);
 }
 
diff --git a/torch-m3gnet_amd/csrc/m3g_geometry_body.h b/torch-m3gnet_amd/csrc/m3g_geometry_body.h
--- a/torch-m3gnet_amd/csrc/m3g_geometry_body.h
+++ b/torch-m3gnet_amd/csrc/m3g_geometry_body.h
@@ -1,6 +1,7 @@
 #pragma once
 #include "m3g_internal.h"
 #include "m3g_basis.h"
+#include "m3g_device.h"
 
 namespace m3g {
 
@@ -28,6 +29,9 @@
   float *u, *dist, *h, *hp, *q, *qp, *fc3, *fc3p;
   const int32_t* act_id;
   int32_t* sync;
+  const int64_t* types;
+  int num_types;
+  int32_t* pair_row;
 };
 template <bool FULL, int L, int R>
 __device__ __forceinline__ void geometry_body(const Consts& c, const GeomArgs& a, int64_t vblock) {
@@ -67,6 +71,10 @@
   u[e * 3 + 1] = r[1] / d;
   u[e * 3 + 2] = r[2] / d;
   if (!FULL) return;
+  if (a.pair_row) {
+    bool bad;
+    a.pair_row[e] = (int32_t)(species_index(a.types[i], a.num_types, bad) * a.num_types + species_index(a.types[j], a.num_types, bad));
+  }
   float hh[kRCap], hd[kRCap];
   radial_basis(c, d, hh, hd);
   *(float4*)(h + e * kRP) = float4{hh[0], hh[1], hh[2], hh[3]};
@@ -135,8 +143,10 @@
   rz = __builtin_fmaf(g, uz, __builtin_fmaf(-proj, uz, az) * inv);
 }
 
-inline GeomArgs geometry_args(const Topo& t, const float* pos, const float* lattice, const int32_t* shift, const Work& w) {
-  return GeomArgs{t.E, t.src, t.dst, t.batch, pos, lattice, shift, w.u, w.d, w.h, w.hp, w.q, w.qp, w.fc3, w.fc3p, t.act_id, w.sync};
+inline GeomArgs geometry_args(const Consts& c, const Topo& t, const float* pos, const float* lattice, const int32_t* shift, const int64_t* types,
+                              const Work& w) {
+  return GeomArgs{t.E, t.src, t.dst, t.batch, pos, lattice, shift, w.u, w.d, w.h, w.hp, w.q, w.qp, w.fc3, w.fc3p, t.act_id, w.sync,
+                  types, c.num_types, w.pair_row};
 }
 
 }
diff --git a/torch-m3gnet_amd/csrc/m3g_internal.h b/torch-m3gnet_amd/csrc/m3g_internal.h
--- a/torch-m3gnet_amd/csrc/m3g_internal.h
+++ b/torch-m3gnet_amd/csrc/m3g_internal.h
@@ -146,6 +146,7 @@
 constexpr size_t species_tab_v(int num_types) { return (size_t)num_types * kDP; }
 constexpr size_t species_tab_ta(int num_types) { return (size_t)num_types * (kDP + kCP); }
 constexpr size_t species_tab_tb(int num_types) { return (size_t)num_types * (kDP + kCP + 4 * kDP); }
+constexpr int kPairRowFloats = 4 * kDP;
 struct ReadoutImg {
   static constexpr int w1 = 0;
   static constexpr int w2d = w1 + 8 * 2 * 512;
@@ -179,6 +180,7 @@
   float* d_mfma_revf32 = nullptr;
   float* d_node_img[m3g::kNumPrec] = {nullptr, nullptr, nullptr};
   float* d_species_tab[m3g::kNumPrec] = {nullptr, nullptr, nullptr};
+  float* d_pair_tab[m3g::kNumPrec] = {nullptr, nullptr, nullptr};
   m3g::Options opt;
   float w_scale_inv = 1.f;
   int device = -1;
@@ -326,6 +328,7 @@
   float* p1_blk[kMaxBlocks];
   float* TAb[kMaxBlocks];
   float* TBb[kMaxBlocks];
+  int32_t* pair_row;
   float* de_soa;
   float* dcn;
   float* dh_parts;
@@ -337,7 +340,7 @@
 };
 Work work_carve(int B, const StepPath& path , int64_t N, int64_t E, int64_t S, void* base);
 
-void launch_geometry(const Consts& c, const Topo& t, const float* pos, const float* lattice, const int32_t* shift,
+void launch_geometry(const Consts& c, const Topo& t, const float* pos, const float* lattice, const int32_t* shift, const int64_t* types,
                      const Work& w, hipStream_t s);
 void launch_geometry_reverse(const Consts& c, const Topo& t, const Work& w, const float* dh, int dh_parts, float* forces,
                              float* stresses, hipStream_t s, bool gather_virial = false, const float* pos = nullptr, const float* lattice = nullptr,
@@ -370,6 +373,7 @@
 void launch_geometry_species(const m3g_plan* plan, const Consts& c, const Topo& t, const Work& w, const float* pos, const float* lattice,
                              const int32_t* shift, const int64_t* types, hipStream_t s);
 int build_species_tables(m3g_plan* plan);
+int build_pair_tables(m3g_plan* plan);
 void launch_energy_sums(const Consts& c, const Topo& t, const float* scaled_atomic, float* scaled_total, float* total, hipStream_t s);
 void launch_readout_mfma(const m3g_plan* plan, const StepPath& p, const Consts& c, const WeightLayout& wl, const Topo& t, const int64_t* types,
                          const float* x_prev, float* x, const Work& w, float* scaled_atomic, float* scaled_total, float* total,
@@ -403,7 +407,7 @@
                               hipStream_t s);
 void launch_edge_rev_edge_mlp(const m3g_plan* plan, const StepPath& p, const Consts& c, const Topo& t, const Work& w, int b, const float* dx_new,
                               bool de_is_zero, hipStream_t s);
-void launch_edge_rev_fused(const m3g_plan* plan, const Consts& c, const Topo& t, const Work& w, int b, const float* dx_new,
+void launch_edge_rev_fused(const m3g_plan* plan, const StepPath& p, const Consts& c, const Topo& t, const Work& w, int b, const float* dx_new,
                            bool de_is_zero, hipStream_t s);
 void launch_edge_rev_f32(const m3g_plan* plan, const StepPath& p, const Consts& c, const Topo& t, const Work& w, int b, const float* dx_new,
                          bool de_is_zero, hipStream_t s);
diff --git a/torch-m3gnet_amd/csrc/m3g_node_mfma.hip b/torch-m3gnet_amd/csrc/m3g_node_mfma.hip
--- a/torch-m3gnet_amd/csrc/m3g_node_mfma.hip
+++ b/torch-m3gnet_amd/csrc/m3g_node_mfma.hip
@@ -182,9 +182,13 @@
   const float* tab;
   float *x, *v, *TA, *TB;
 };
-constexpr int kSpeciesRowVecs = kSpeciesRowFloats / 4, kSpeciesVecsPerThread = 4;
+constexpr int kSpeciesRowVecs = kSpeciesRowFloats / 4, kSpeciesNodeVecs = (kDP + kCP) / 4, kSpeciesVecsPerThread = 4;
+template <bool TABLES>
+constexpr int species_row_vecs() { return TABLES ? kSpeciesRowVecs : kSpeciesNodeVecs; }
+template <bool TABLES>
 __device__ __forceinline__ void species_expand_body(const SpeciesArgs& a, int64_t vblock) {
-  const int64_t total = a.N * kSpeciesRowVecs;
+  constexpr int kRowVecs = species_row_vecs<TABLES>();
+  const int64_t total = a.N * kRowVecs;
   const int64_t first = vblock * (256 * kSpeciesVecsPerThread) + threadIdx.x;
   const float* __restrict__ tab = a.tab;
   const int64_t* __restrict__ types = a.types;
@@ -195,15 +199,15 @@
     const int64_t i = first + j * 256;
     dst[j] = nullptr;
     if (i >= total) return;
-    const int64_t atom = i / kSpeciesRowVecs;
-    const int piece = (int)(i - atom * kSpeciesRowVecs);
+    const int64_t atom = i / kRowVecs;
+    const int piece = (int)(i - atom * kRowVecs);
     bool bad;
     const int64_t ty = species_index(types[atom], nt, bad);
     const float* src;
     if (piece < 16) {
       src = tab + ty * kDP + 4 * piece;
       dst[j] = a.x + atom * kDP + 4 * piece;
-    } else if (piece < 20) {
+    } else if (!TABLES || piece < 20) {
       src = tab + species_tab_v(nt) + ty * kCP + 4 * (piece - 16);
       dst[j] = a.v + atom * kCP + 4 * (piece - 16);
     } else if (piece < 84) {
@@ -219,13 +223,25 @@
     if (dst[j]) *(f32x4*)dst[j] = t[j];
   });
 }
-static_assert(kSpeciesRowVecs == 16 + 4 + 64 + 64, "species_expand_body: the pieces of a row");
-
-__global__ void __launch_bounds__(256) k_species_expand(SpeciesArgs a) { species_expand_body(a, blockIdx.x); }
-template <int L, int R>
+static_assert(kSpeciesRowVecs == 16 + 4 + 64 + 64 && kSpeciesNodeVecs == 16 + 4, "species_expand_body: the pieces of a row");
+
+template <bool TABLES>
+__global__ void __launch_bounds__(256) k_species_expand(SpeciesArgs a) { species_expand_body<TABLES>(a, blockIdx.x); }
+template <int L, int R, bool TABLES>
 __global__ void __launch_bounds__(256) k_geometry_species(Consts c, GeomArgs ga, int n_geo, SpeciesArgs sa) {
   if ((int)blockIdx.x < n_geo) geometry_body<true, L, R>(c, ga, blockIdx.x);
-  else species_expand_body(sa, (int64_t)blockIdx.x - n_geo);
+  else species_expand_body<TABLES>(sa, (int64_t)blockIdx.x - n_geo);
+}
+
+__global__ void __launch_bounds__(256) k_pair_table(int num_types, const float* __restrict__ ta, const float* __restrict__ tb, float* __restrict__ out) {
+  constexpr int kVecs = kPairRowFloats / 4;
+  const int64_t i = blockIdx.x * (int64_t)blockDim.x + threadIdx.x;
+  if (i >= (int64_t)num_types * num_types * kVecs) return;
+  const int64_t row = i / kVecs;
+  const int piece = (int)(i - row * kVecs);
+  const int64_t zi = row / num_types, zj = row - zi * num_types;
+  *(f32x4*)(out + row * kPairRowFloats + 4 * piece) =
+      *(const f32x4*)(ta + zi * kPairRowFloats + 4 * piece) + *(const f32x4*)(tb + zj * kPairRowFloats + 4 * piece);
 }
 
 struct ReadoutSums {
@@ -508,7 +524,7 @@
                               const int32_t* shift, const int64_t* types, const float* emb, hipStream_t s) {
   const int64_t tiles = (t.N + 15) / 16;
   const int n_geo = (int)((t.E + 255) / 256);
-  const GeomArgs ga = geometry_args(t, pos, lattice, shift, w);
+  const GeomArgs ga = geometry_args(c, t, pos, lattice, shift, types, w);
   const NodePreArgs na{c.C, t.N, plan->d_node_img[kPrecF32], nullptr, w.seg_head, w.seg_first, t.row_ptr, w.x[0], w.v[0], w.TAb[0], w.TBb[0], types, emb,
                        c.num_types};
   M3G_DISPATCH_LR(c.L, c.R, hipLaunchKernelGGL((k_geometry_node_pre<L, R>), dim3((unsigned)(n_geo + 3 * tiles)), dim3(256), 0, s, c, ga, n_geo, na));
@@ -517,19 +533,24 @@
 static SpeciesArgs species_args(const m3g_plan* plan, const Consts& c, const Topo& t, const Work& w, const int64_t* types) {
   return SpeciesArgs{t.N, types, c.num_types, plan->d_species_tab[plan->opt.precision], w.x[0], w.v[0], w.TAb[0], w.TBb[0]};
 }
-static unsigned species_expand_blocks(int64_t N) {
+static unsigned species_expand_blocks(int64_t N, bool tables) {
   constexpr int64_t per = 256 * kSpeciesVecsPerThread;
-  return (unsigned)((N * kSpeciesRowVecs + per - 1) / per);
+  return (unsigned)((N * (tables ? kSpeciesRowVecs : kSpeciesNodeVecs) + per - 1) / per);
 }
 void launch_species_expand(const m3g_plan* plan, const Consts& c, const Topo& t, const Work& w, const int64_t* types, hipStream_t s) {
-  hipLaunchKernelGGL(k_species_expand, dim3(species_expand_blocks(t.N)), dim3(256), 0, s, species_args(plan, c, t, w, types));
+  const bool tables = w.TAb[0] != nullptr;
+  if (tables) hipLaunchKernelGGL(k_species_expand<true>, dim3(species_expand_blocks(t.N, true)), dim3(256), 0, s, species_args(plan, c, t, w, types));
+  else hipLaunchKernelGGL(k_species_expand<false>, dim3(species_expand_blocks(t.N, false)), dim3(256), 0, s, species_args(plan, c, t, w, types));
 }
 void launch_geometry_species(const m3g_plan* plan, const Consts& c, const Topo& t, const Work& w, const float* pos, const float* lattice,
                              const int32_t* shift, const int64_t* types, hipStream_t s) {
   const int n_geo = (int)((t.E + 255) / 256);
-  const GeomArgs ga = geometry_args(t, pos, lattice, shift, w);
+  const GeomArgs ga = geometry_args(c, t, pos, lattice, shift, types, w);
   const SpeciesArgs sa = species_args(plan, c, t, w, types);
-  M3G_DISPATCH_LR(c.L, c.R, hipLaunchKernelGGL((k_geometry_species<L, R>), dim3((unsigned)n_geo + species_expand_blocks(t.N)), dim3(256), 0, s, c, ga, n_geo, sa));
+  const bool tables = w.TAb[0] != nullptr;
+  const dim3 grid((unsigned)n_geo + species_expand_blocks(t.N, tables));
+  if (tables) { M3G_DISPATCH_LR(c.L, c.R, hipLaunchKernelGGL((k_geometry_species<L, R, true>), grid, dim3(256), 0, s, c, ga, n_geo, sa)); }
+  else { M3G_DISPATCH_LR(c.L, c.R, hipLaunchKernelGGL((k_geometry_species<L, R, false>), grid, dim3(256), 0, s, c, ga, n_geo, sa)); }
 }
 
 int build_species_tables(m3g_plan* plan) {
@@ -559,4 +580,19 @@
   return M3G_OK;
 }
 
-}
+int build_pair_tables(m3g_plan* plan) {
+  const int nt = plan->cfg.num_types;
+  if (plan->cfg.num_blocks == 0) return M3G_OK;
+  const size_t vecs = (size_t)nt * nt * (kPairRowFloats / 4);
+  for (int prec = 0; prec < kNumPrec; ++prec) {
+    float*& out = plan->d_pair_tab[prec];
+    const float* tab = plan->d_species_tab[prec];
+    if (!out) M3G_HIP_CHECK(hipMalloc((void**)&out, sizeof(float) * 4 * vecs));
+    hipLaunchKernelGGL(k_pair_table, grid_for((int64_t)vecs), dim3(256), 0, nullptr, nt, tab + species_tab_ta(nt), tab + species_tab_tb(nt), out);
+    M3G_HIP_CHECK(hipGetLastError());
+  }
+  M3G_HIP_CHECK(hipDeviceSynchronize());
+  return M3G_OK;
+}
+
+}
diff --git a/torch-m3gnet_amd/csrc/m3g_pack_mfma.hip b/torch-m3gnet_amd/csrc/m3g_pack_mfma.hip
--- a/torch-m3gnet_amd/csrc/m3g_pack_mfma.hip
+++ b/torch-m3gnet_amd/csrc/m3g_pack_mfma.hip
@@ -159,7 +159,7 @@
 
 void free_mfma_images(m3g_plan* plan) {
   auto drop = [](float*& p) { if (p) { (void)hipFree(p); p = nullptr; } };
-  for (int prec = 0; prec < kNumPrec; ++prec) { drop(plan->d_mfma_fwd[prec]); drop(plan->d_mfma_rev[prec]); drop(plan->d_node_img[prec]); drop(plan->d_species_tab[prec]); }
+  for (int prec = 0; prec < kNumPrec; ++prec) { drop(plan->d_mfma_fwd[prec]); drop(plan->d_mfma_rev[prec]); drop(plan->d_node_img[prec]); drop(plan->d_species_tab[prec]); drop(plan->d_pair_tab[prec]); }
   drop(plan->d_mfma_revf);
   drop(plan->d_mfma_revf_h);
   drop(plan->d_mfma_revf32);
diff --git a/torch-m3gnet_amd/csrc/m3g_step_path.h b/torch-m3gnet_amd/csrc/m3g_step_path.h
--- a/torch-m3gnet_amd/csrc/m3g_step_path.h
+++ b/torch-m3gnet_amd/csrc/m3g_step_path.h
@@ -32,6 +32,7 @@
   int dp1_by_dst = 0;
   int split_node_tiles = 128;
   int species_tables = 1;
+  int pair_rows = 1;
   int fuse_node_tb = 1;
   int debug_node_tb_polls = 0;
   int split_tail = 1;
@@ -46,7 +47,7 @@
   int overlap = 0;
   int graph_replay = 0;
 };
-static_assert(sizeof(Options) == 21 * sizeof(int), "Options: twenty-one ints, no padding (its bytes are compared as a key)");
+static_assert(sizeof(Options) == 22 * sizeof(int), "Options: twenty-two ints, no padding (its bytes are compared as a key)");
 
 enum { kDp1F32 = 0, kDp1Packed = 1, kDp1Fixed = 2, kDp1F32ByDst = 3  };
 
@@ -80,6 +81,7 @@
   bool long_lists = false;
   bool geom_with_node_pre = false;
   int block0 = kBlock0Kernel;
+  bool pair_rows = false;
   bool node_split = false;
   bool fwd_split = false;
   int rev_edge = kRevValu;
@@ -120,6 +122,7 @@
     p.node_split = f32 && small_nodes;
     p.geom_with_node_pre = !profile && p.node_split && m.B != 0 && E != 0 && N != 0;
     if (o.species_tables && m.B != 0 && N != 0) p.block0 = !profile && E != 0 ? kBlock0ExpandBesideGeom : kBlock0ExpandAlone;
+    p.pair_rows = o.pair_rows && o.species_tables && m.B != 0 && N != 0;
     p.fwd_split = etiles > 0 && etiles <= o.small_tiles_fwd && f32 && p.fwd_save != 1 && !stamps;
     p.rev_edge = !p.fused_rev ? kRevPair : !f32 ? kRevFused : (etiles > 0 && etiles <= o.small_tiles && saves_p2 && !stamps) ? kRevSplit : kRevF32;
     p.split_tail = o.split_tail;
```

New measurement: 4.357 million atom-steps/s, median of 6. No clear change (+0.7%).
